# martenlienen/generative-turbulence

Hardware: AMD Instinct MI355X
Metric: U-Net fwd+bwd voxels/sec (DDPM training step, 192x64x48x4) (higher is better)
Workload: dtype bf16

## Files before the change

### generative-turbulence_amd/csrc/tdx_codec.hip

```cpp
#include "tdx_codec_elem.h"
#include "tdx_conv3.h"

#define CD_THREADS 256
#define CD_VOX 512
#define CD_VOX_DEC 2048

template <typename T, int F>
__global__ void __launch_bounds__(CD_THREADS)
encode_fwd_kernel(const float* __restrict__ x, const float* __restrict__ wx, const float* __restrict__ bx,
                  const float* __restrict__ c, const float* __restrict__ wc, const float* __restrict__ bc,
                  T* __restrict__ y, int64_t V, int D, int Dtot) {
    const int b = blockIdx.y;
    const int L = Dtot >> 3, rows = CD_THREADS / L;
    const int lc = threadIdx.x % L, r = threadIdx.x / L;
    if (r >= rows) return;
    const EncLane<F> enc(lc, b, D, V, x, wx, bx, c, wc, bc);
    const int64_t v0 = (int64_t)blockIdx.x * CD_VOX, v1 = min(V, v0 + CD_VOX);
    for (int64_t v = v0 + r; v < v1; v += rows) {
        const auto in = enc.load(V, v);
        Vec8<T> o;
#pragma unroll
        for (int j = 0; j < 8; ++j) o.v[j] = enc.eval(j, in);
        o.store(y + ((int64_t)b * V + v) * Dtot + lc * 8);
    }
}

template <typename T, int F>
__global__ void __launch_bounds__(CD_THREADS)
encode_bwd_kernel(const T* __restrict__ dy, const float* __restrict__ x, const float* __restrict__ c,
                  const float* __restrict__ wc, float* __restrict__ dwx, float* __restrict__ dbx,
                  float* __restrict__ dwc, float* __restrict__ dbc, float* __restrict__ dc, int B, int64_t V, int D,
                  int Dtot, int64_t slab_stride) {
    dwx += blockIdx.x * slab_stride; dbx += blockIdx.x * slab_stride;
    if (dwc) { dwc += blockIdx.x * slab_stride; dbc += blockIdx.x * slab_stride; }
    const int L = Dtot >> 3, rows = CD_THREADS / L;
    const int lc = threadIdx.x % L, r = threadIdx.x / L;
    const bool active = r < rows;
    const bool is_x = lc * 8 < D;
    const int ch0 = is_x ? lc * 8 : lc * 8 - D;
    float s[8 * F + 8];
#pragma unroll
    for (int j = 0; j < 8 * F + 8; ++j) s[j] = 0.f;
    float wr[8][F];
    if (!is_x) {
#pragma unroll
        for (int j = 0; j < 8; ++j)
#pragma unroll
            for (int k = 0; k < F; ++k) wr[j][k] = wc[(ch0 + j) * F + k];
    }
    const int Lc = (Dtot - D) >> 3;
    const int64_t v0 = (int64_t)blockIdx.x * CD_VOX, v1 = min(V, v0 + CD_VOX);
    for (int64_t vb = v0; vb < v1; vb += rows) {
        const int64_t v = vb + r;
        const bool ok = active && v < v1;
        float dcl[F];
#pragma unroll
        for (int k = 0; k < F; ++k) dcl[k] = 0.f;
        for (int b0 = 0; b0 < B; b0 += 3) {
            Raw8<T> graw[3];
            float in[3][F];
#pragma unroll
            for (int u = 0; u < 3; ++u) {
                const int b = min(b0 + u, B - 1);
                const bool okb = ok && b0 + u < B;
                graw[u].load(dy + ((int64_t)b * V + (okb ? v : v0)) * Dtot + lc * 8);
                const float* src = is_x ? x + (int64_t)b * F * V : c;
#pragma unroll
                for (int k = 0; k < F; ++k) in[u][k] = src[(int64_t)k * V + (okb ? v : v0)];
            }
            __builtin_amdgcn_sched_barrier(0);
#pragma unroll
            for (int u = 0; u < 3; ++u) {
                const bool okb = ok && b0 + u < B;
                Vec8<T> g = graw[u].get();
#pragma unroll
                for (int j = 0; j < 8; ++j) g.v[j] = okb ? g.v[j] : 0.f;
#pragma unroll
                for (int j = 0; j < 8; ++j) {
#pragma unroll
                    for (int k = 0; k < F; ++k) s[j * F + k] += g.v[j] * in[u][k];
                    s[8 * F + j] += g.v[j];
                }
                if (!is_x) {
#pragma unroll
                    for (int k = 0; k < F; ++k)
#pragma unroll
                        for (int j = 0; j < 8; ++j) dcl[k] += wr[j][k] * g.v[j];
                }
            }
        }
        if (dc != nullptr && Lc > 0) {
#pragma unroll
            for (int k = 0; k < F; ++k) {
                float t = is_x ? 0.f : dcl[k];
                for (int o = 1; o < L; o <<= 1) t += __shfl_xor(t, o, 64);
                if (ok && lc == 0) dc[(int64_t)k * V + v] = t;
            }
        }
    }
    __shared__ float red[CD_THREADS][8 * F + 8 + 1];
    const int tid = threadIdx.x;
#pragma unroll
    for (int j = 0; j < 8 * F + 8; ++j) red[tid][j] = active ? s[j] : 0.f;
    __syncthreads();
    constexpr int N = 8 * F + 8;
    for (int o = tid; o < L * N; o += CD_THREADS) {
        const int l = o / N, j = o - l * N;
        float t = 0.f;
        for (int q = 0; q < rows; ++q) t += red[q * L + l][j];
        const bool lx = l * 8 < D;
        const int c0 = lx ? l * 8 : l * 8 - D;
        float* dw = lx ? dwx : dwc;
        float* db = lx ? dbx : dbc;
        if (j < 8 * F) atomicAdd(&dw[(c0 + j / F) * F + (j % F)], t);
        else atomicAdd(&db[c0 + (j - 8 * F)], t);
    }
}

static bool pow2(int v) { return v > 0 && (v & (v - 1)) == 0; }
static hipError_t codec_zero(float* p, size_t n, hipStream_t st) {
    return tdx_zero_async(p, n * sizeof(float), st) == TDX_OK ? hipSuccess : hipErrorUnknown;
}
static float* det_slabs(int64_t floats) {
    char* arena = (char*)tdx_scratch_ptr();
    if (!arena || (int64_t)tdx_scratch_bytes() < 256 + floats * (int64_t)sizeof(float)) return nullptr;
    return reinterpret_cast<float*>(arena + 256);
}

extern "C" int tdx_encode_fwd(const float* x, int Fx, const float* wx, const float* bx, const float* c, int Fc,
                              const float* wc, const float* bc, void* y, int B, int64_t V, int D, int dtype,
                              void* stream) {
    TDX_CHECK_ARG(x && wx && bx && y && B > 0 && V > 0 && D > 0);
    TDX_CHECK_ARG(c == nullptr || (wc && bc));
    const int Dtot = c ? 2 * D : D;
    if ((D % 8) || !pow2(Dtot / 8) || Dtot / 8 > 64 || Fx != 4 || (c && Fc != 4)) return TDX_ESHAPE;
    dim3 grid(ceil_div(V, CD_VOX), B);
    TDX_DISPATCH_DTYPE(dtype, hipLaunchKernelGGL((encode_fwd_kernel<T, 4>), grid, dim3(CD_THREADS), 0, as_stream(stream),
                                                 x, wx, bx, c, wc, bc, (T*)y, V, D, Dtot));
    return tdx_launch_status();
}

extern "C" int tdx_encode_bwd(const void* dy, const float* x, int Fx, const float* c, int Fc, const float* wc,
                              float* dwx, float* dbx, float* dwc, float* dbc, float* dc, int B, int64_t V, int D,
                              int dtype, void* stream) {
    TDX_CHECK_ARG(dy && x && dwx && dbx && B > 0 && V > 0 && D > 0);
    TDX_CHECK_ARG(c == nullptr || (wc && dwc && dbc));
    const int Dtot = c ? 2 * D : D;
    if ((D % 8) || !pow2(Dtot / 8) || Dtot / 8 > 64 || Fx != 4 || (c && Fc != 4)) return TDX_ESHAPE;
    hipStream_t st = as_stream(stream);
    dim3 grid(ceil_div(V, CD_VOX));
    if (tdx_deterministic()) {
        const int64_t slab = 10 * (int64_t)D;
        float* slabs = det_slabs((int64_t)grid.x * slab);
        if (!slabs) return TDX_EINVAL;
        int e0 = tdx_zero_async(slabs, (size_t)grid.x * slab * sizeof(float), st);
        if (e0 != TDX_OK) return e0;
        TDX_DISPATCH_DTYPE(dtype, hipLaunchKernelGGL((encode_bwd_kernel<T, 4>), grid, dim3(CD_THREADS), 0, st, (const T*)dy, x, c, wc,
                                                     slabs, slabs + 4 * D, c ? slabs + 5 * D : nullptr,
                                                     c ? slabs + 9 * D : nullptr, dc, B, V, D, Dtot, slab));
        int rc = tdx_launch_status();
        if (rc == TDX_OK) rc = ordered_sum_launch(slabs, (int)grid.x, slab, dwx, 1, 4 * D, 4 * D, false, st);
        if (rc == TDX_OK) rc = ordered_sum_launch(slabs + 4 * D, (int)grid.x, slab, dbx, 1, D, D, false, st);
        if (rc == TDX_OK && c) rc = ordered_sum_launch(slabs + 5 * D, (int)grid.x, slab, dwc, 1, 4 * D, 4 * D, false, st);
        if (rc == TDX_OK && c) rc = ordered_sum_launch(slabs + 9 * D, (int)grid.x, slab, dbc, 1, D, D, false, st);
        return rc;
    }
    hipError_t e = codec_zero(dwx, (size_t)D * 4, st);
    if (e == hipSuccess) e = codec_zero(dbx, (size_t)D, st);
    if (e == hipSuccess && c) e = codec_zero(dwc, (size_t)D * 4, st);
    if (e == hipSuccess && c) e = codec_zero(dbc, (size_t)D, st);
    if (e != hipSuccess) return (int)e;
    TDX_DISPATCH_DTYPE(dtype, hipLaunchKernelGGL((encode_bwd_kernel<T, 4>), grid, dim3(CD_THREADS), 0, st, (const T*)dy,
                                                 x, c, wc, dwx, dbx, dwc, dbc, dc, B, V, D, Dtot, (int64_t)0));
    return tdx_launch_status();
}

template <typename T, int F>
__global__ void __launch_bounds__(CD_THREADS)
decode_fwd_kernel(const T* __restrict__ h, const float* __restrict__ w, const float* __restrict__ bias,
                  float* __restrict__ y, int64_t V, int D) {
    const int b = blockIdx.y;
    const int L = D >> 3, rows = CD_THREADS / L;
    const int lc = threadIdx.x % L, r = threadIdx.x / L;
    const DecLane<F> dec(lc, D, w, bias);
    const int64_t v0 = (int64_t)blockIdx.x * CD_VOX_DEC, v1 = min(V, v0 + CD_VOX_DEC);
    for (int64_t vb = v0; vb < v1; vb += rows) {
        const int64_t v = vb + r;
        const bool ok = r < rows && v < v1;
        Vec8<T> a;
#pragma unroll
        for (int j = 0; j < 8; ++j) a.v[j] = 0.f;
        if (ok) a.load(h + ((int64_t)b * V + v) * D + lc * 8);
#pragma unroll
        for (int f = 0; f < F; ++f) {
            const float t = dec.dot(f, a.v, L);
            if (ok && lc == 0) y[((int64_t)b * F + f) * V + v] = t;
        }
    }
}

template <typename T, int F>
__global__ void __launch_bounds__(CD_THREADS)
decode_bwd_kernel(const float* __restrict__ dy, const T* __restrict__ h, const float* __restrict__ w,
                  T* __restrict__ dh, float* __restrict__ dw, float* __restrict__ db, int64_t V, int D, int64_t slab_stride) {
    const int b = blockIdx.y;
    dw += ((int64_t)blockIdx.y * gridDim.x + blockIdx.x) * slab_stride;
    db += ((int64_t)blockIdx.y * gridDim.x + blockIdx.x) * slab_stride;
    const int L = D >> 3, rows = CD_THREADS / L;
    const int lc = threadIdx.x % L, r = threadIdx.x / L;
    const bool active = r < rows;
    float wr[F][8], s[F * 8 + F];
#pragma unroll
    for (int f = 0; f < F; ++f)
#pragma unroll
        for (int j = 0; j < 8; ++j) wr[f][j] = w[f * D + lc * 8 + j];
#pragma unroll
    for (int j = 0; j < F * 8 + F; ++j) s[j] = 0.f;
    const int64_t v0 = (int64_t)blockIdx.x * CD_VOX_DEC, v1 = min(V, v0 + CD_VOX_DEC);
    if (active) {
        for (int64_t v = v0 + r; v < v1; v += rows) {
            float g[F];
#pragma unroll
            for (int f = 0; f < F; ++f) g[f] = dy[((int64_t)b * F + f) * V + v];
            Vec8<T> a, o;
            a.load(h + ((int64_t)b * V + v) * D + lc * 8);
#pragma unroll
            for (int j = 0; j < 8; ++j) {
                float t = 0.f;
#pragma unroll
                for (int f = 0; f < F; ++f) { t += wr[f][j] * g[f]; s[f * 8 + j] += g[f] * a.v[j]; }
                o.v[j] = t;
            }
            if (lc == 0) {
#pragma unroll
                for (int f = 0; f < F; ++f) s[F * 8 + f] += g[f];
            }
            o.store(dh + ((int64_t)b * V + v) * D + lc * 8);
        }
    }
    __shared__ float red[CD_THREADS][F * 8 + F + 1];
    const int tid = threadIdx.x;
    constexpr int N = F * 8 + F;
#pragma unroll
    for (int j = 0; j < N; ++j) red[tid][j] = active ? s[j] : 0.f;
    __syncthreads();
    for (int o = tid; o < L * N; o += CD_THREADS) {
        const int l = o / N, j = o - l * N;
        float t = 0.f;
        for (int q = 0; q < rows; ++q) t += red[q * L + l][j];
        if (j < F * 8) atomicAdd(&dw[(j / 8) * D + l * 8 + (j % 8)], t);
        else if (l == 0) atomicAdd(&db[j - F * 8], t);
    }
}

extern "C" int tdx_decode_fwd(const void* h, const float* w, const float* bias, float* y, int B, int64_t V, int D, int F,
                              int dtype, void* stream) {
    TDX_CHECK_ARG(h && w && bias && y && B > 0 && V > 0 && D > 0);
    if ((D % 8) || !pow2(D / 8) || D / 8 > 64 || F != 4) return TDX_ESHAPE;
    dim3 grid(ceil_div(V, CD_VOX_DEC), B);
    TDX_DISPATCH_DTYPE(dtype, hipLaunchKernelGGL((decode_fwd_kernel<T, 4>), grid, dim3(CD_THREADS), 0, as_stream(stream),
                                                 (const T*)h, w, bias, y, V, D));
    return tdx_launch_status();
}

extern "C" int tdx_decode_bwd(const float* dy, const void* h, const float* w, void* dh, float* dw, float* db, int B,
                              int64_t V, int D, int F, int dtype, void* stream) {
    TDX_CHECK_ARG(dy && h && w && dh && dw && db && B > 0 && V > 0 && D > 0);
    if ((D % 8) || !pow2(D / 8) || D / 8 > 64 || F != 4) return TDX_ESHAPE;
    hipStream_t st = as_stream(stream);
    dim3 grid(ceil_div(V, CD_VOX_DEC), B);
    if (tdx_deterministic()) {
        const int64_t slab = (int64_t)F * D + F, nblk = (int64_t)grid.x * grid.y;
        float* slabs = det_slabs(nblk * slab);
        if (!slabs) return TDX_EINVAL;
        int e0 = tdx_zero_async(slabs, (size_t)nblk * slab * sizeof(float), st);
        if (e0 != TDX_OK) return e0;
        TDX_DISPATCH_DTYPE(dtype, hipLaunchKernelGGL((decode_bwd_kernel<T, 4>), grid, dim3(CD_THREADS), 0, st, dy, (const T*)h, w,
                                                     (T*)dh, slabs, slabs + (int64_t)F * D, V, D, slab));
        int rc = tdx_launch_status();
        if (rc == TDX_OK) rc = ordered_sum_launch(slabs, (int)nblk, slab, dw, 1, F * D, F * D, false, st);
        if (rc == TDX_OK) rc = ordered_sum_launch(slabs + (int64_t)F * D, (int)nblk, slab, db, 1, F, F, false, st);
        return rc;
    }
    hipError_t e = codec_zero(dw, (size_t)F * D, st);
    if (e == hipSuccess) e = codec_zero(db, (size_t)F, st);
    if (e != hipSuccess) return (int)e;
    TDX_DISPATCH_DTYPE(dtype, hipLaunchKernelGGL((decode_bwd_kernel<T, 4>), grid, dim3(CD_THREADS), 0, st, dy,
// ... 4 lines not shown
```

### generative-turbulence_amd/csrc/tdx_codec_elem.h

```cpp
#pragma once
#include "tdx_common.h"

template <typename T> __device__ __forceinline__ float round_as(float a);
template <> __device__ __forceinline__ float round_as<float>(float a) { return a; }
template <> __device__ __forceinline__ float round_as<bf16>(float a) { return __uint_as_float(pack_bf16x2(a, 0.f) << 16); }
template <> __device__ __forceinline__ float round_as<f16>(float a) { return (float)(_Float16)a; }

template <int F>
struct EncLane {
    struct In { float v[F]; };
    const float* src;
    float w[8][F], bias[8];
    __device__ __forceinline__ EncLane(int lc, int b, int D, int64_t V, const float* __restrict__ x, const float* __restrict__ wx,
                                       const float* __restrict__ bx, const float* __restrict__ c, const float* __restrict__ wc,
                                       const float* __restrict__ bc) {
        const bool is_x = lc * 8 < D;
        const int ch0 = is_x ? lc * 8 : lc * 8 - D;
        const float* wp = is_x ? wx : wc;
        const float* bp = is_x ? bx : bc;
        src = is_x ? x + (int64_t)b * F * V : c;
#pragma unroll
        for (int j = 0; j < 8; ++j) {
            bias[j] = bp[ch0 + j];
#pragma unroll
            for (int k = 0; k < F; ++k) w[j][k] = wp[(ch0 + j) * F + k];
        }
    }
    __device__ __forceinline__ In load(int64_t V, int64_t v) const {
        In in;
#pragma unroll
        for (int k = 0; k < F; ++k) in.v[k] = src[(int64_t)k * V + v];
        return in;
    }
    __device__ __forceinline__ float eval(int j, const In& in) const {
        float a = bias[j];
#pragma unroll
        for (int k = 0; k < F; ++k) a = __builtin_fmaf(w[j][k], in.v[k], a);
        return a;
    }
};

template <int F>
struct DecLane {
    float w[F][8], bias[F];
    __device__ __forceinline__ DecLane(int lc, int C, const float* __restrict__ wp, const float* __restrict__ bp) {
#pragma unroll
        for (int f = 0; f < F; ++f) {
            bias[f] = bp[f];
#pragma unroll
            for (int j = 0; j < 8; ++j) w[f][j] = wp[f * C + lc * 8 + j];
        }
    }
    __device__ __forceinline__ float dot(int f, const float (&h)[8], int L) const {
        float t = 0.f;
#pragma unroll
        for (int j = 0; j < 8; ++j) t = __builtin_fmaf(w[f][j], h[j], t);
        for (int q = 1; q < L; q <<= 1) t += __shfl_xor(t, q, 64);
        return t + bias[f];
    }
};
```

### generative-turbulence_amd/csrc/tdx_conv3.h

```cpp
#pragma once
#include "tdx_common.h"

struct Conv3Geom {
    int B;
    int Xi, Yi, Zi;
    int Xo, Yo, Zo;
    int off;
};

bool conv3_mfma_supported(int C1, int C2, int Cout);
bool conv3_mfma_f32_supported(int C1, int C2, int Cout);
static inline int conv3_layout_kc(int dtype, int K, int N) {
    if (dtype == 1 || dtype == 3) return conv3_mfma_supported(K, 0, N) ? 16 : 0;
    return conv3_mfma_f32_supported(K, 0, N) ? 8 : 0;
}
static inline bool conv3_uses_mfma_layout(int dtype, int K, int N) { return (dtype == 1 || dtype == 3) && conv3_mfma_supported(K, 0, N); }
bool conv3_mfma_split_supported(int C1, int C2, int Cout);

struct Conv3Ext {
    int ld1, ld2;
    const void* init;
    bool init_shared;
};

struct Conv3Call {
    const void* x1; int C1;
    const void* x2; int C2;
    const void* wp;
    const float* bias;
    void* y;
    int B, X, Y, Z, N;
    bool zero_pad;
    double* gn_acc;
    void* d1; int D1; void* d2;
    const void* a1; const void* a2;
    hipStream_t st;
    int fmt;
    const Conv3Ext* ext;
    const int* slabs_beyond;
    bool hf() const { return fmt == TDX_F16; }
    Conv3Geom geom() const { return Conv3Geom{B, X, Y, Z, X, Y, Z, 0}; }
};

struct SmallGeom {
    int B;
    int Ev[3];
    int Es[3];
    int off;
    int clamp;
    int nbg;
    int xs;
    int gx;
    int Ix, Iy, Iz;
    int K, N;
    int per_split;
    int nsplit;
};
struct Conv3SmallPlan {
    SmallGeom g;
    size_t lds;
    int mtw;
};

struct Conv3Route {
    int fmt, family, status;
    int ring_depth;
    Conv3SmallPlan small;
};
Conv3Route conv3_route(int dtype, int impl, int C1, int C2, int N, int B, int X, int Y, int Z, bool data_gradient);

int conv3_mfma_launch(const Conv3Call& c);
int conv3_mfma_split_launch(const Conv3Call& c);
int conv3_mfma_f32_launch(const Conv3Call& c);
int conv3_direct_launch(const Conv3Call& c);
int conv3_fold_launch(const Conv3Call& c);

int conv3_ring_depth(int C1, int C2, int N, int B, int X, int Y, int Z, bool data_gradient);
int conv3_ring_launch(const Conv3Call& c, int depth);

bool conv3_small_plan(Conv3SmallPlan& p, int C1, int C2, int N, int B, int X, int Y, int Z, bool data_gradient, bool split);
int conv3_small_launch(const Conv3Call& c, const Conv3SmallPlan& p);

struct Conv3WgradCall {
    const void* x1; int C1;
    const void* x2; int C2;
    const void* dy;
    float* dwp;
    float* dbias;
    int B, X, Y, Z, Cout;
    hipStream_t st;
    float* slabs; int max_slabs; int* nslab;
    bool hf;
};
bool tdx_deterministic();
static inline float* conv3_wgrad_merge(const Conv3WgradCall& c, int& nsplit, int64_t& slab_stride) {
    if (tdx_deterministic() && c.slabs != nullptr && nsplit > c.max_slabs) nsplit = c.max_slabs > 0 ? c.max_slabs : 1;
    const bool use_slabs = c.slabs != nullptr && nsplit <= c.max_slabs;
    slab_stride = use_slabs ? (int64_t)27 * (c.C1 + c.C2) * c.Cout : 0;
    if (c.nslab) *c.nslab = use_slabs ? nsplit : 0;
    return use_slabs ? c.slabs : c.dwp;
}
bool conv3_wgrad_mfma_supported(int C1, int C2, int Cout);
bool conv3_wgrad_mfma_split_supported(int C1, int C2, int Cout);
bool conv3_wgrad_mfma_f32_supported(int C1, int C2, int Cout);
int conv3_wgrad_mfma_launch(const Conv3WgradCall& c);
int conv3_wgrad_small_launch(const Conv3WgradCall& c);
int conv3_wgrad_ring_launch(const Conv3WgradCall& c);
int conv3_wgrad_mfma_split_launch(const Conv3WgradCall& c);
int conv3_wgrad_split_ring_launch(const Conv3WgradCall& c);
int conv3_wgrad_mfma_f32_launch(const Conv3WgradCall& c);
int conv3_wgrad_direct_launch(const Conv3WgradCall& c, int dtype);
int conv3_unpack_wgrad_launch(const Conv3WgradCall& c, float* dw, float* dbw, float* dbias, bool many);
int tdx_persistent_cus();
int ordered_sum_launch(const float* slabs, int nslab, int64_t stride, float* dst, int rows, int cols, int64_t ld, bool add,
                       hipStream_t st);
size_t bias_grad_ordered_scratch_floats(int C);
int bias_grad_ordered_launch(const void* dy, int64_t nvox, int C, int dtype, float* dbias, float* part, size_t part_floats,
                             hipStream_t st);
void* tdx_scratch_ptr();
size_t tdx_scratch_bytes();

size_t conv3_shell_buffer_bytes(int B, int X, int Y, int Z, int N);
int conv3_shell_launch(const void* dy, const void* wb, void* d1, int D1, void* d2, int B, int X, int Y, int Z, int K, int N,
                       int mode, hipStream_t st, void* sbuf = nullptr);

#define TDX_GN_REPLICAS 32
int gn_finalize_launch(double* acc, float* stats, int B, int C, int G, int64_t V, float eps, int replicas,
                       hipStream_t st);
int gn_stats_launch(const void* x, float* stats, int B, int64_t V, int C, int G, float eps, int dtype, void* workspace,
                    bool clean, hipStream_t stream);
```

### generative-turbulence_amd/csrc/tdx_conv3_entry.hip

```cpp
#include "tdx_common.h"
#include "tdx_conv3.h"
#include <stdlib.h>
#include <algorithm>

int tdx_persistent_cus() {
    const char* env = getenv("TDX_PERSISTENT_CUS");
    int n = env ? atoi(env) : 256;
    n = n < 8 ? 8 : (n > 256 ? 256 : n);
    return n & ~7;
}
static void* g_scratch = nullptr;
static size_t g_scratch_bytes = 0;
void* tdx_scratch_ptr() { return g_scratch; }
size_t tdx_scratch_bytes() { return g_scratch_bytes; }
extern "C" int tdx_set_scratch(void* ptr, size_t bytes) {
    if (ptr != nullptr && bytes < 64) return TDX_EINVAL;
    g_scratch = ptr;
    g_scratch_bytes = ptr ? bytes : 0;
    return TDX_OK;
}

Conv3Route conv3_route(int dtype, int impl, int C1, int C2, int N, int B, int X, int Y, int Z, bool data_gradient) {
    Conv3Route r;
    r.fmt = dtype; r.family = TDX_KERNEL_DIRECT; r.status = TDX_OK; r.ring_depth = 0;
    impl &= 0xff;
    auto small_or_brick = [&](bool split) {
        r.family = conv3_small_plan(r.small, C1, C2, N, B, X, Y, Z, data_gradient, split) ? TDX_KERNEL_SMALL : TDX_KERNEL_BRICK;
    };
    if (dtype == TDX_F32 && impl == TDX_CONV_SPLIT && conv3_mfma_split_supported(C1 + C2, 0, N)) {
        r.fmt = TDX_F32_SPLIT;
        if (!conv3_mfma_split_supported(C1, C2, N)) { r.family = TDX_KERNEL_BRICK; r.status = TDX_ESHAPE; return r; }
        small_or_brick(true);
    } else if (dtype == TDX_F32 && impl != TDX_CONV_DIRECT && conv3_mfma_f32_supported(C1, C2, N)) {
        r.family = TDX_KERNEL_BRICK;
    } else {
        const bool ok = tdx_is_h16(dtype) && conv3_mfma_supported(C1, C2, N);
        const bool asked = impl == TDX_CONV_MFMA && (tdx_is_h16(dtype) || !data_gradient);
        if (!ok) { r.status = asked ? TDX_ESHAPE : TDX_OK; return r; }
        if (!asked && impl != TDX_CONV_AUTO) return r;
        small_or_brick(false);
        if (r.family == TDX_KERNEL_BRICK && (r.ring_depth = conv3_ring_depth(C1, C2, N, B, X, Y, Z, data_gradient)) != 0)
            r.family = TDX_KERNEL_RING;
    }
    return r;
}

static int conv3_launch(const Conv3Call& c, const Conv3Route& r) {
    switch (r.family) {
        case TDX_KERNEL_SMALL: return conv3_small_launch(c, r.small);
        case TDX_KERNEL_RING: return conv3_ring_launch(c, r.ring_depth);
        case TDX_KERNEL_BRICK:
            if (c.fmt == TDX_F32_SPLIT) return conv3_mfma_split_launch(c);
            return c.fmt == TDX_F32 ? conv3_mfma_f32_launch(c) : conv3_mfma_launch(c);
        default: return conv3_direct_launch(c);
    }
}

static Conv3Call conv3_fwd_call(const void* x1, int C1, const void* x2, int C2, const void* wf, const float* bias, void* y, int B,
                                int X, int Y, int Z, int Cout, int fmt, void* stream) {
    Conv3Call c = {};
    c.x1 = x1; c.C1 = C1; c.x2 = x2; c.C2 = C2; c.wp = wf; c.bias = bias; c.y = y;
    c.B = B; c.X = X; c.Y = Y; c.Z = Z; c.N = Cout;
    c.st = as_stream(stream); c.fmt = fmt;
    return c;
}

extern "C" int tdx_conv3_fwd(const void* x1, int C1, const void* x2, int C2, const void* wf, const float* bias,
                             void* y, int B, int X, int Y, int Z, int Cout, int dtype, int impl, void* stream) {
    TDX_CHECK_ARG(x1 && wf && y && B > 0 && X > 0 && Y > 0 && Z > 0 && C1 > 0 && C2 >= 0 && Cout > 0);
    TDX_CHECK_ARG(C2 == 0 || x2);
    const Conv3Route r = conv3_route(dtype, impl, C1, C2, Cout, B, X, Y, Z, false);
    if (r.status != TDX_OK) return r.status;
    return conv3_launch(conv3_fwd_call(x1, C1, x2, C2, wf, bias, y, B, X, Y, Z, Cout, r.fmt, stream), r);
}

extern "C" int tdx_conv3_fwd_kernel(int C1, int C2, int Cout, int B, int X, int Y, int Z, int dtype, int impl) {
    return conv3_route(dtype, impl, C1, C2, Cout, B, X, Y, Z, false).family;
}

extern "C" int tdx_conv3_fwd_gn(const void* x1, int C1, const void* x2, int C2, const void* wf, const float* bias,
                                void* y, float* stats, int G, float eps, void* gn_workspace, int B, int X, int Y, int Z,
                                int Cout, int dtype, int impl, void* stream) {
    TDX_CHECK_ARG(x1 && wf && y && stats && gn_workspace && B > 0 && X > 0 && Y > 0 && Z > 0 && C1 > 0 && C2 >= 0);
    TDX_CHECK_ARG(Cout > 0 && G > 0 && (Cout % G) == 0 && (C2 == 0 || x2));
    const bool clean = (impl & TDX_WS_CLEAN) != 0;
    const Conv3Route r = conv3_route(dtype, impl, C1, C2, Cout, B, X, Y, Z, false);
    if (r.status != TDX_OK) return r.status;
    Conv3Call c = conv3_fwd_call(x1, C1, x2, C2, wf, bias, y, B, X, Y, Z, Cout, r.fmt, stream);
    const int64_t V = (int64_t)X * Y * Z;
    if (r.family == TDX_KERNEL_DIRECT || r.family == TDX_KERNEL_SMALL || tdx_deterministic()) {
        int rc = conv3_launch(c, r);
        if (rc != TDX_OK) return rc;
        if (r.family == TDX_KERNEL_DIRECT && !tdx_deterministic())
            return tdx_gn_stats(y, stats, B, V, Cout, G, eps, dtype, gn_workspace, stream);
        return gn_stats_launch(y, stats, B, V, Cout, G, eps, dtype, gn_workspace, clean, c.st);
    }
    c.gn_acc = (double*)gn_workspace;
    if (!clean) {
        int e = tdx_zero_async(c.gn_acc, (size_t)TDX_GN_REPLICAS * B * Cout * 2 * sizeof(double), c.st);
        if (e != TDX_OK) return e;
    }
    int rc = conv3_launch(c, r);
    if (rc != TDX_OK) return rc;
    return gn_finalize_launch(c.gn_acc, stats, B, Cout, G, V, eps, TDX_GN_REPLICAS, c.st);
}

extern "C" int tdx_conv3_fwd_partial(const void* x1, int C1, int ld1, const void* wf, const float* bias,
                                     const void* init, int init_shared, void* y, float* stats, int G, float eps,
                                     void* gn_workspace, int B, int X, int Y, int Z, int Cout, int dtype, int impl,
                                     void* stream) {
    TDX_CHECK_ARG(x1 && wf && y && B > 0 && X > 0 && Y > 0 && Z > 0 && C1 > 0 && Cout > 0 && ld1 >= C1 && (ld1 % 8) == 0);
    TDX_CHECK_ARG(stats == nullptr || (gn_workspace && G > 0 && (Cout % G) == 0));
    const bool clean = (impl & TDX_WS_CLEAN) != 0;
    if (!tdx_is_h16(dtype)) return TDX_EDTYPE;
    if (!conv3_mfma_supported(C1, 0, Cout)) return TDX_ESHAPE;
    const bool det = tdx_deterministic();
    const Conv3Ext ext = {ld1, 0, init, init_shared != 0};
    Conv3Call c = conv3_fwd_call(x1, C1, nullptr, 0, wf, bias, y, B, X, Y, Z, Cout, dtype, stream);
    c.ext = &ext;
    c.gn_acc = (stats && !det) ? (double*)gn_workspace : nullptr;
    if (c.gn_acc && !clean) {
        int e = tdx_zero_async(c.gn_acc, (size_t)TDX_GN_REPLICAS * B * Cout * 2 * sizeof(double), c.st);
        if (e != TDX_OK) return e;
    }
    int rc = conv3_mfma_launch(c);
    if (rc != TDX_OK || !stats) return rc;
    if (det) return gn_stats_launch(y, stats, B, (int64_t)X * Y * Z, Cout, G, eps, dtype, gn_workspace, clean, c.st);
    return gn_finalize_launch(c.gn_acc, stats, B, Cout, G, (int64_t)X * Y * Z, eps, TDX_GN_REPLICAS, c.st);
}

extern "C" size_t tdx_conv3_bwd_data_workspace_bytes(int B, int X, int Y, int Z, int Cin, int dtype, int impl) {
    (void)impl;
    const size_t padded = (size_t)B * (X + 2) * (Y + 2) * (Z + 2) * Cin * (tdx_is_h16(dtype) ? 2 : 4);
    const size_t shell = conv3_shell_buffer_bytes(B, X, Y, Z, Cin);
    return (padded > shell ? padded : shell) + 256;
}

static int conv3_bwd_data_impl(const void* dy, const void* wb, void* dx1, int C1, void* dx2, int C2, const void* add1,
                               const void* add2, int B, int X, int Y, int Z, int Cout, int dtype, int impl,
                               void* workspace, void* stream) {
    TDX_CHECK_ARG(dy && wb && dx1 && workspace && B > 0 && X > 0 && Y > 0 && Z > 0 && C1 > 0 && C2 >= 0 && Cout > 0);
    TDX_CHECK_ARG(C2 == 0 || dx2);
    const int Cin = C1 + C2;
    if ((C1 % 8) || (C2 % 8) || (Cout % 8)) return TDX_ESHAPE;
    const Conv3Route r = conv3_route(dtype, impl, Cout, 0, Cin, B, X, Y, Z, true);
    if (r.status != TDX_OK) return r.status;
    Conv3Call c = {};
    c.x1 = dy; c.C1 = Cout; c.wp = wb;
    c.B = B; c.X = X; c.Y = Y; c.Z = Z; c.N = Cin;
    c.zero_pad = true;
    c.d1 = dx1; c.D1 = C1; c.d2 = dx2; c.a1 = add1; c.a2 = add2;
    c.st = as_stream(stream); c.fmt = r.fmt;
    if (r.family == TDX_KERNEL_DIRECT) c.y = workspace;
    int rc = conv3_launch(c, r);
    if (rc != TDX_OK || r.family == TDX_KERNEL_SMALL) return rc;
    if (r.family == TDX_KERNEL_DIRECT) return conv3_fold_launch(c);
    const int shell_mode = r.fmt == TDX_F16 ? 3 : (r.fmt == TDX_F32_SPLIT ? 2 : (r.fmt == TDX_F32 ? 1 : 0));
    return conv3_shell_launch(dy, wb, dx1, C1, dx2, B, X, Y, Z, Cout, Cin, shell_mode, c.st, workspace);
}

extern "C" int tdx_conv3_bwd_data(const void* dy, const void* wb, void* dx1, int C1, void* dx2, int C2,
                                  int accumulate, int B, int X, int Y, int Z, int Cout, int dtype, int impl,
                                  void* workspace, void* stream) {
    return conv3_bwd_data_impl(dy, wb, dx1, C1, dx2, C2, accumulate ? dx1 : nullptr, accumulate ? dx2 : nullptr, B, X, Y, Z,
                               Cout, dtype, impl, workspace, stream);
}

extern "C" int tdx_conv3_bwd_data_add(const void* dy, const void* wb, void* dx1, int C1, void* dx2, int C2,
                                      const void* add1, const void* add2, int B, int X, int Y, int Z, int Cout, int dtype,
                                      int impl, void* workspace, void* stream) {
    return conv3_bwd_data_impl(dy, wb, dx1, C1, dx2, C2, add1, add2, B, X, Y, Z, Cout, dtype, impl, workspace, stream);
}

#define W3_MAX_SLABS 8
static int w3_slab_capacity(int Cin, int Cout) {
    const int64_t c = ((int64_t)1 << 19) / ((int64_t)Cin * Cout);
    return (int)(c < W3_MAX_SLABS ? W3_MAX_SLABS : (c > 512 ? 512 : c));
}
extern "C" size_t tdx_conv3_bwd_weight_workspace_bytes(int Cin, int Cout, int impl) {
    (void)impl;
    return (size_t)(1 + w3_slab_capacity(Cin, Cout)) * 27 * Cin * Cout * sizeof(float) + (size_t)Cout * sizeof(float) + 512;
}

struct Conv3WgradRoute {
    int (*launch)(const Conv3WgradCall&);
    bool f32;
    int status;
};
static Conv3WgradRoute conv3_wgrad_route(int dtype, int impl, int C1, int C2, int Cout) {
    if (dtype == TDX_F32 && impl == TDX_CONV_SPLIT && conv3_wgrad_mfma_split_supported(C1, C2, Cout))
        return {conv3_wgrad_mfma_split_launch, true, TDX_OK};
    if (dtype == TDX_F32 && impl != TDX_CONV_DIRECT && conv3_wgrad_mfma_f32_supported(C1, C2, Cout))
        return {conv3_wgrad_mfma_f32_launch, true, TDX_OK};
    if (impl == TDX_CONV_MFMA || (impl == TDX_CONV_AUTO && tdx_is_h16(dtype) && conv3_wgrad_mfma_supported(C1, C2, Cout))) {
        if (!tdx_is_h16(dtype)) return {nullptr, false, TDX_EDTYPE};
        if (!conv3_wgrad_mfma_supported(C1, C2, Cout)) return {nullptr, false, TDX_ESHAPE};
        return {conv3_wgrad_mfma_launch, false, TDX_OK};
    }
    return {nullptr, false, TDX_OK};
}

extern "C" int tdx_conv3_bwd_weight(const void* x1, int C1, const void* x2, int C2, const void* dy, float* dw,
                                    float* dbias, int B, int X, int Y, int Z, int Cout, int dtype, int impl,
                                    void* workspace, void* stream) {
    TDX_CHECK_ARG(x1 && dy && dw && workspace && B > 0 && X > 0 && Y > 0 && Z > 0 && C1 > 0 && C2 >= 0 && Cout > 0);
    TDX_CHECK_ARG(C2 == 0 || x2);
    const int Cin = C1 + C2;
    if ((C1 % 8) || (C2 % 8) || (Cout % 8)) return TDX_ESHAPE;
    hipStream_t st = as_stream(stream);
    const bool clean = (impl & TDX_WS_CLEAN) != 0;
    float* dwp = (float*)workspace;
    float* dbw = dwp + (size_t)27 * Cin * Cout;
    if (!clean) {
        int e = tdx_zero_async(dwp, ((size_t)27 * Cin * Cout + Cout) * sizeof(float), st);
        if (e != TDX_OK) return e;
    }
    const Conv3WgradRoute r = conv3_wgrad_route(dtype, impl & 0xff, C1, C2, Cout);
    if (r.status != TDX_OK) return r.status;
    int nslab = 0;
    const bool det = tdx_deterministic();
    float* slab_base = dbw + ((Cout + 63) / 64) * 64;
    auto ordered_bias = [&]() -> int {
        if (!det || !dbias) return TDX_OK;
        return bias_grad_ordered_launch(dy, (int64_t)B * X * Y * Z, Cout, dtype, dbias, slab_base,
                                        (size_t)W3_MAX_SLABS * 27 * Cin * Cout, st);
    };
    Conv3WgradCall c = {x1, C1, x2, C2, dy, dwp, (dbias && !det) ? dbw : nullptr, B, X, Y, Z, Cout, st, slab_base, 0, &nslab,
                        dtype == TDX_F16};
    if (r.launch != nullptr) {
        c.max_slabs = (r.f32 && !det) ? W3_MAX_SLABS : w3_slab_capacity(Cin, Cout);
    } else if (det) {
        c.max_slabs = std::min(w3_slab_capacity(Cin, Cout), 64);
    }
    const int rc = r.launch != nullptr ? r.launch(c) : conv3_wgrad_direct_launch(c, dtype);
    if (rc != TDX_OK) return rc;
    const int rc_unpack = conv3_unpack_wgrad_launch(c, dw, dbw, dbias, r.launch != nullptr && nslab > W3_MAX_SLABS);
    return rc_unpack != TDX_OK ? rc_unpack : ordered_bias();
}
```

### generative-turbulence_amd/csrc/tdx_conv3_mfma.hip

```cpp
#include "tdx_common.h"
#include "tdx_conv3.h"
#include "tdx_mfma.h"
#include <stdlib.h>

#define M3_KC 16

bool conv3_mfma_supported(int C1, int C2, int Cout) {
    return C1 > 0 && (C1 % M3_KC) == 0 && (C2 % M3_KC) == 0 && (Cout % 32) == 0;
}

struct ConvView {
    int B;
    int Ei[3];
    int si[3];
    int so[3];
    int r0[3];
    int r1[3];
    int nb[3];
    int off;
    int ws[3];
    int in_batch, out_batch;
    int ld1, ld2;
    int init_batch;
};

struct ConvViews {
    ConvView v[3];
    int start[4];
};

template <int BN>
__device__ __forceinline__ int out_addr(int v, int c) {
    if (BN == 64) return v * 128 + ((c ^ (v & 7)) << 4);
    return v * 64 + ((c ^ ((v >> 1) & 3)) << 4);
}

template <int NT, bool XT, bool ZERO_PAD, bool PERM, bool EXT, bool HF>
__global__ void __launch_bounds__(256, 2)
conv3_mfma_kernel(const bf16* __restrict__ x1, int C1, const bf16* __restrict__ x2, int C2,
                  const bf16* __restrict__ wp, const float* __restrict__ bias, bf16* __restrict__ y, ConvViews gs,
                  int Cout, double* __restrict__ gn_acc, bf16* __restrict__ d1, int D1, bf16* __restrict__ d2,
                  const bf16* __restrict__ a1, const bf16* __restrict__ a2, const bf16* __restrict__ init) {
    typedef H16<HF> H;
    typedef typename H::T HT;
    constexpr int BN = NT * 32;
    constexpr int BX = XT ? 2 : 4, BY = XT ? 16 : 8, BZ = 8;
    constexpr int HX = BX + 2, HY = BY + 2, HZ = BZ + 2;
    constexpr int SZ = XT ? 10 : 12;
    constexpr int NHALO = HX * HY * HZ;
    constexpr int APLANE = HX * HY * SZ * 16 + 64;
    constexpr int BRICK_BYTES = 2 * APLANE;
    constexpr int B_PLANE = 27 * BN * 16 + 64;
    extern __shared__ __attribute__((aligned(16))) unsigned char smem[];
    unsigned char* sA = smem;
    unsigned char* sB = smem + BRICK_BYTES;

    const int tid = threadIdx.x;
    const int lane = tid & 63, wave = tid >> 6;
    const int r = lane & 31, hh = lane >> 5;

    int bid = blockIdx.x;
    bid = xcd_contiguous(bid, (int)gridDim.x);
    const int region = bid >= gs.start[1] ? (bid >= gs.start[2] ? 2 : 1) : 0;
    const ConvView& g = gs.v[region];
    bid -= gs.start[region];
    const int b2 = bid % g.nb[2]; bid /= g.nb[2];
    const int b1 = bid % g.nb[1]; bid /= g.nb[1];
    const int b0 = bid % g.nb[0]; bid /= g.nb[0];
    const int b = bid;
    const int n0 = blockIdx.y * BN;
    const int o0 = g.r0[0] + b0 * BX, o1 = g.r0[1] + b1 * BY, o2 = g.r0[2] + b2 * BZ;
    const int Cin = C1 + C2;

    constexpr int A_PIECES = NHALO * 2;
    constexpr int A_PER_THREAD = (A_PIECES + 255) / 256;
    constexpr int B_PIECES = 27 * BN * 2;
    constexpr int B_PER_THREAD = (B_PIECES + 255) / 256;
    int a_src[A_PER_THREAD];
    int a_dst[A_PER_THREAD];
#pragma unroll
    for (int i = 0; i < A_PER_THREAD; ++i) {
        const int p = tid + i * 256;
        a_dst[i] = -1;
        a_src[i] = -1;
        if (p < A_PIECES) {
            const int hv = ((p >> 3) << 2) + (p & 3), half = (p >> 2) & 1;
            const int hx = hv / (HY * HZ), rem = hv - hx * (HY * HZ);
            const int hy = rem / HZ, hz = rem - hy * HZ;
            a_dst[i] = half * APLANE + ((hx * HY + hy) * SZ + hz) * 16;
            int s0 = o0 + hx - 1 + g.off, s1 = o1 + hy - 1 + g.off, s2 = o2 + hz - 1 + g.off;
            bool ok = true;
            if (ZERO_PAD) {
                ok = s0 >= 0 && s0 < g.Ei[0] && s1 >= 0 && s1 < g.Ei[1] && s2 >= 0 && s2 < g.Ei[2];
            } else {
                s0 = min(max(s0, 0), g.Ei[0] - 1); s1 = min(max(s1, 0), g.Ei[1] - 1); s2 = min(max(s2, 0), g.Ei[2] - 1);
            }
            if (ok) a_src[i] = (s0 * g.si[0] + s1 * g.si[1] + s2 * g.si[2]) * 2 + half;
        }
    }
    const int64_t batch_vox = (int64_t)b * g.in_batch;

    const int b_half = (tid >> 2) & 1;
    const int b_row0 = ((tid >> 3) << 2) + (tid & 3);
    const int b_goff = ((b_row0 / BN) * Cout + (b_row0 % BN)) * 16 + b_half * 8;
    const int b_dst = b_half * B_PLANE + b_row0 * 16;

    uint4 areg[A_PER_THREAD], breg[B_PER_THREAD];
    auto load_slice = [&](int c) {
        const int k0 = c * M3_KC;
        const bf16* xs;
        int Cs, kk;
        if (k0 < C1) { xs = x1; Cs = EXT ? g.ld1 : C1; kk = k0; } else { xs = x2; Cs = EXT ? g.ld2 : C2; kk = k0 - C1; }
        xs += batch_vox * Cs + kk;
#pragma unroll
        for (int i = 0; i < A_PER_THREAD; ++i) {
            areg[i] = make_uint4(0, 0, 0, 0);
            if (a_src[i] >= 0)
                areg[i] = *reinterpret_cast<const uint4*>(xs + (int64_t)(a_src[i] >> 1) * Cs + (a_src[i] & 1) * 8);
        }
        const bf16* wc = wp + (int64_t)c * 27 * Cout * 16 + (int64_t)n0 * 16 + b_goff;
#pragma unroll
        for (int i = 0; i < B_PER_THREAD; ++i) {
            breg[i] = make_uint4(0, 0, 0, 0);
            if (b_row0 + 128 * i < 27 * BN)
                breg[i] = *reinterpret_cast<const uint4*>(wc + (int64_t)i * (128 / BN) * Cout * 16);
        }
    };
    auto store_slice = [&]() {
#pragma unroll
        for (int i = 0; i < A_PER_THREAD; ++i)
            if (a_dst[i] >= 0) *reinterpret_cast<uint4*>(sA + a_dst[i]) = areg[i];
#pragma unroll
        for (int i = 0; i < B_PER_THREAD; ++i)
            if (b_row0 + 128 * i < 27 * BN) *reinterpret_cast<uint4*>(sB + b_dst + i * 2048) = breg[i];
    };

    const int wx = XT ? (wave >> 1) : wave, wy0 = XT ? 8 * (wave & 1) : 0;
    int a_h[2];
#pragma unroll
    for (int mt = 0; mt < 2; ++mt)
        a_h[mt] = ((wx + 1) * HY + (wy0 + 4 * mt + (r & 3) + 1)) * SZ + ((r >> 2) + 1);
    int b_off[NT];
#pragma unroll
    for (int nt = 0; nt < NT; ++nt) b_off[nt] = hh * B_PLANE + (nt * 32 + r) * 16;

    f32x16 acc[NT][2];
#pragma unroll
    for (int nt = 0; nt < NT; ++nt)
#pragma unroll
        for (int mt = 0; mt < 2; ++mt)
#pragma unroll
            for (int i = 0; i < 16; ++i) acc[nt][mt][i] = 0.f;

    const int nchunks = Cin / M3_KC;
    load_slice(0);
    for (int c = 0; c < nchunks; ++c) {
        __syncthreads();
        store_slice();
        __syncthreads();
        if (c + 1 < nchunks) load_slice(c + 1);

        bf16x8 xf[2][2], wf[2][NT];
        auto read_frags = [&](int tap, int buf) {
            const int ex = tap / 9 - 1, ey = (tap / 3) % 3 - 1, ez = tap % 3 - 1;
            const int toff = (ex * HY + ey) * SZ + ez;
            const int wtap = (XT || PERM) ? (ex + 1) * g.ws[0] + (ey + 1) * g.ws[1] + (ez + 1) * g.ws[2] : tap;
#pragma unroll
            for (int mt = 0; mt < 2; ++mt)
                xf[buf][mt] = *reinterpret_cast<const bf16x8*>(sA + hh * APLANE + (a_h[mt] + toff) * 16);
#pragma unroll
            for (int nt = 0; nt < NT; ++nt)
                wf[buf][nt] = *reinterpret_cast<const bf16x8*>(sB + wtap * (BN * 16) + b_off[nt]);
        };
        read_frags(0, 0);
        __builtin_amdgcn_sched_group_barrier(0x100, 2 + NT, 0);
#pragma unroll
        for (int tap = 0; tap < 27; ++tap) {
            if (tap + 1 < 27) read_frags(tap + 1, (tap + 1) & 1);
#pragma unroll
            for (int nt = 0; nt < NT; ++nt)
#pragma unroll
                for (int mt = 0; mt < 2; ++mt)
                    acc[nt][mt] = H::mfma(wf[tap & 1][nt], xf[tap & 1][mt], acc[nt][mt]);
            if (tap + 1 < 27) {
#pragma unroll
                for (int k = 0; k < 2 * NT; ++k) {
                    __builtin_amdgcn_sched_group_barrier(0x008, 1, 0);
                    if (k < 2 + NT) __builtin_amdgcn_sched_group_barrier(0x100, 1, 0);
                }
            } else {
                __builtin_amdgcn_sched_group_barrier(0x008, 2 * NT, 0);
            }
        }
    }

    __syncthreads();
    unsigned char* sO = smem;
#pragma unroll
    for (int nt = 0; nt < NT; ++nt)
#pragma unroll
        for (int j = 0; j < 4; ++j) {
            const int ch = nt * 32 + 8 * j + 4 * hh;
            float bv[4] = {0.f, 0.f, 0.f, 0.f};
            if (bias) {
#pragma unroll
                for (int e = 0; e < 4; ++e) bv[e] = bias[n0 + ch + e];
            }
#pragma unroll
            for (int mt = 0; mt < 2; ++mt) {
                const int v = (wx * BY + wy0 + 4 * mt + (r & 3)) * 8 + (r >> 2);
                const unsigned lo = H::pack2(acc[nt][mt][4 * j] + bv[0], acc[nt][mt][4 * j + 1] + bv[1]);
                const unsigned hi = H::pack2(acc[nt][mt][4 * j + 2] + bv[2], acc[nt][mt][4 * j + 3] + bv[3]);
                *reinterpret_cast<uint2*>(sO + out_addr<BN>(v, ch >> 3) + (ch & 7) * 2) = make_uint2(lo, hi);
            }
        }
    __syncthreads();
    constexpr int CHUNKS = BN / 8;
    float s1[8], s2[8];
#pragma unroll
    for (int e = 0; e < 8; ++e) s1[e] = s2[e] = 0.f;
#pragma unroll
    for (int i = 0; i < CHUNKS; ++i) {
        const int p = tid + i * 256;
        const int v = p / CHUNKS, cidx = p % CHUNKS;
        const int c0 = o0 + (v >> 3) / BY, c1 = o1 + (v >> 3) % BY, c2 = o2 + (v & 7);
        if (c0 < g.r1[0] && c1 < g.r1[1] && c2 < g.r1[2]) {
            uint4 val = *reinterpret_cast<const uint4*>(sO + out_addr<BN>(v, cidx));
            bool direct = false;
            if (ZERO_PAD && d1 != nullptr) {
                const int u0 = c0 + g.off, u1 = c1 + g.off, u2 = c2 + g.off;
                if (u0 >= 0 && u0 < g.Ei[0] && u1 >= 0 && u1 < g.Ei[1] && u2 >= 0 && u2 < g.Ei[2]) {
                    const int64_t u = (int64_t)b * g.in_batch + u0 * g.si[0] + u1 * g.si[1] + u2 * g.si[2];
                    const int n = n0 + cidx * 8;
                    const bool lo = n < D1;
                    bf16* dst = lo ? d1 + u * D1 + n : d2 + u * (Cout - D1) + (n - D1);
                    const bf16* asrc = lo ? (a1 ? a1 + u * D1 + n : nullptr) : (a2 ? a2 + u * (Cout - D1) + (n - D1) : nullptr);
                    if (asrc) {
                        Vec8<HT> va, vb;
                        va.load(reinterpret_cast<const HT*>(&val));
                        vb.load(reinterpret_cast<const HT*>(asrc));
#pragma unroll
                        for (int e = 0; e < 8; ++e) va.v[e] += vb.v[e];
                        va.store(reinterpret_cast<HT*>(dst));
                    } else {
                        *reinterpret_cast<uint4*>(dst) = val;
                    }
                    direct = true;
                }
            }
            if (!direct) {
                const int64_t ov = (int64_t)b * g.out_batch + c0 * g.so[0] + c1 * g.so[1] + c2 * g.so[2];
                if (EXT && init != nullptr) {
                    const int64_t iv = (int64_t)b * g.init_batch + c0 * g.so[0] + c1 * g.so[1] + c2 * g.so[2];
                    Vec8<HT> va, vb;
                    va.load(reinterpret_cast<const HT*>(&val));
                    vb.load(reinterpret_cast<const HT*>(init + iv * Cout + n0 + cidx * 8));
#pragma unroll
                    for (int e = 0; e < 8; ++e) va.v[e] += vb.v[e];
                    va.store(reinterpret_cast<HT*>(&val));
                }
                *reinterpret_cast<uint4*>(y + ov * Cout + n0 + cidx * 8) = val;
            }
            if (gn_acc != nullptr) {
                const unsigned wds[4] = {val.x, val.y, val.z, val.w};
#pragma unroll
                for (int e = 0; e < 4; ++e) {
                    const float lo = H::lo(wds[e]), hi = H::hi(wds[e]);
                    s1[2 * e] += lo; s2[2 * e] += lo * lo;
                    s1[2 * e + 1] += hi; s2[2 * e + 1] += hi * hi;
                }
            }
        }
    }
    if (gn_acc != nullptr) {
        constexpr int NP = 256 / CHUNKS;
        float* red = reinterpret_cast<float*>(smem + 256 * BN * 2);
        const int cidx = tid % CHUNKS, part = tid / CHUNKS;
#pragma unroll
        for (int e = 0; e < 8; ++e) {
            red[(part * BN + cidx * 8 + e) * 2] = s1[e];
            red[(part * BN + cidx * 8 + e) * 2 + 1] = s2[e];
        }
        __syncthreads();
        if (tid < BN * 2) {
            float t = 0.f;
#pragma unroll 8
            for (int pp = 0; pp < NP; ++pp) t += red[pp * BN * 2 + tid];
            const int rep = blockIdx.x & (TDX_GN_REPLICAS - 1);
            atomicAdd(&gn_acc[(((size_t)rep * g.B + b) * Cout + n0) * 2 + tid], (double)t);
        }
    }
}

template <int NT, bool XT, bool ZP, bool PERM, bool EXT, bool HF>
static int launch_view_h(const Conv3Call& c, const ConvViews& v) {
    constexpr int BN = NT * 32;
    constexpr int HXv = (XT ? 2 : 4) + 2, HYv = (XT ? 16 : 8) + 2, SZv = XT ? 10 : 12;
    const size_t lds = (size_t)2 * (HXv * HYv * SZv * 16 + 64) + (size_t)27 * BN * 32 + 128;
    auto kern = conv3_mfma_kernel<NT, XT, ZP, PERM, EXT, HF>;
    static bool attr_set = false;
    if (!attr_set) {
        hipError_t e = hipFuncSetAttribute((const void*)kern, hipFuncAttributeMaxDynamicSharedMemorySize, (int)lds);
        if (e != hipSuccess) return (int)e;
        attr_set = true;
    }
    dim3 grid((unsigned)v.start[3], c.N / BN);
    hipLaunchKernelGGL(kern, grid, dim3(256), lds, c.st, (const bf16*)c.x1, c.C1, (const bf16*)c.x2, c.C2, (const bf16*)c.wp, c.bias,
                       (bf16*)c.y, v, c.N, c.gn_acc, (bf16*)c.d1, c.D1, (bf16*)c.d2, (const bf16*)c.a1, (const bf16*)c.a2,
                       (const bf16*)(EXT ? c.ext->init : nullptr));
    return tdx_launch_status();
}
template <int NT, bool XT, bool ZP, bool PERM, bool EXT = false>
static int launch_view(const Conv3Call& c, const ConvViews& v) {
    return c.hf() ? launch_view_h<NT, XT, ZP, PERM, EXT, true>(c, v) : launch_view_h<NT, XT, ZP, PERM, EXT, false>(c, v);
}

int conv3_mfma_launch(const Conv3Call& c) {
    if (!tdx_is_h16(c.fmt)) return TDX_EINVAL;
    const Conv3Geom g = c.geom();
    const int C1 = c.C1, C2 = c.C2;
    const bool zero_pad = c.zero_pad;
    const Conv3Ext* ext = c.ext;
    const int* slabs_beyond = c.slabs_beyond;
    const int NT = (c.N % 64 == 0) ? 2 : 1;
    if ((int64_t)g.Xi * g.Yi * g.Zi * 2 >= (1ll << 31) || (int64_t)g.Xo * g.Yo * g.Zo >= (1ll << 31)) return TDX_ESHAPE;
    static const bool no_thin = getenv("TDX_CONV3_THIN") && atoi(getenv("TDX_CONV3_THIN")) == 0;

    const int Ei[3] = {g.Xi, g.Yi, g.Zi}, Eo[3] = {g.Xo, g.Yo, g.Zo};
    const int si[3] = {g.Yi * g.Zi, g.Zi, 1}, so[3] = {g.Yo * g.Zo, g.Zo, 1};
    const int bdim[3] = {4, 8, 8};
    static const bool force_thin = getenv("TDX_CONV3_THIN") && atoi(getenv("TDX_CONV3_THIN")) == 2;
    const bool big = force_thin || (int64_t)g.Xo * g.Yo * g.Zo >= 60000;
    int main_end[3];
    bool thin[3];
    for (int a = 0; a < 3; ++a) {
        const int rem = Eo[a] % bdim[a];
        thin[a] = !no_thin && rem >= 1 && rem <= 2 && Eo[a] > bdim[a] && big && ext == nullptr;
        main_end[a] = thin[a] ? Eo[a] - rem : Eo[a];
        if (slabs_beyond != nullptr) {
            if (ext != nullptr || slabs_beyond[a] <= 0 || Eo[a] - slabs_beyond[a] > 2 || Eo[a] < slabs_beyond[a]) return TDX_ESHAPE;
            main_end[a] = slabs_beyond[a];
            thin[a] = main_end[a] < Eo[a];
        }
    }
    auto make_view = [&](const int perm[3], const int lo[3], const int hi[3], bool xt, ConvView& v) -> int {
        v.B = g.B; v.off = g.off;
        v.in_batch = g.Xi * g.Yi * g.Zi; v.out_batch = g.Xo * g.Yo * g.Zo;
        v.ld1 = ext && ext->ld1 ? ext->ld1 : C1;
        v.ld2 = ext && ext->ld2 ? ext->ld2 : C2;
        v.init_batch = ext && ext->init && !ext->init_shared ? v.out_batch : 0;
        const int bl[3] = {xt ? 2 : 4, xt ? 16 : 8, 8};
        int64_t n = g.B;
        for (int k = 0; k < 3; ++k) {
            const int a = perm[k];
            v.Ei[k] = Ei[a]; v.si[k] = si[a]; v.so[k] = so[a];
            v.ws[k] = (a == 0) ? 9 : (a == 1 ? 3 : 1);
            v.r0[k] = lo[a]; v.r1[k] = hi[a];
            v.nb[k] = hi[a] > lo[a] ? ceil_div(hi[a] - lo[a], bl[k]) : 0;
            n *= v.nb[k];
        }
        return (int)n;
    };
    auto launch = [&](const ConvViews& vs, bool xt, bool permuted) -> int {
        if (vs.start[3] == 0) return TDX_OK;
#define M3_GO(NTV, XTV, PV) (zero_pad ? launch_view<NTV, XTV, true, PV>(c, vs) : launch_view<NTV, XTV, false, PV>(c, vs))
        if (ext != nullptr) {
            if (zero_pad || xt || permuted) return TDX_ESHAPE;
            return NT == 2 ? launch_view<2, false, false, false, true>(c, vs) : launch_view<1, false, false, false, true>(c, vs);
        }
        if (NT == 2) return xt ? M3_GO(2, true, false) : (permuted ? M3_GO(2, false, true) : M3_GO(2, false, false));
        return xt ? M3_GO(1, true, false) : (permuted ? M3_GO(1, false, true) : M3_GO(1, false, false));
#undef M3_GO
    };
    const int lo[3] = {0, 0, 0}, hi[3] = {main_end[0], main_end[1], main_end[2]};
    static const bool no_perm = getenv("TDX_CONV3_PERM") && atoi(getenv("TDX_CONV3_PERM")) == 0;
    int best[3] = {0, 1, 2};
    if (!no_perm && ext == nullptr) {
        const int cand[3][3] = {{0, 1, 2}, {1, 0, 2}, {2, 0, 1}};
        int64_t best_n = -1;
        for (int c = 0; c < 3; ++c) {
            const int64_t n = (int64_t)ceil_div(hi[cand[c][0]], 4) * ceil_div(hi[cand[c][1]], 8) * ceil_div(hi[cand[c][2]], 8);
            if (best_n < 0 || n < best_n) {
                best_n = n;
                for (int k = 0; k < 3; ++k) best[k] = cand[c][k];
            }
        }
    }
    ConvViews mainv;
    const int nmain = make_view(best, lo, hi, false, mainv.v[0]);
    mainv.v[1] = mainv.v[2] = mainv.v[0];
    mainv.start[0] = 0; mainv.start[1] = mainv.start[2] = mainv.start[3] = nmain;
    int rc = slabs_beyond ? TDX_OK : launch(mainv, false, !(best[0] == 0 && best[1] == 1 && best[2] == 2));
    if (rc != TDX_OK) return rc;
    if (thin[0] || thin[1] || thin[2]) {
        const int pm[3][3] = {{0, 1, 2}, {1, 0, 2}, {2, 0, 1}};
        const int l[3][3] = {{main_end[0], 0, 0}, {0, main_end[1], 0}, {0, 0, main_end[2]}};
        const int h[3][3] = {{Eo[0], Eo[1], Eo[2]}, {main_end[0], Eo[1], Eo[2]}, {main_end[0], main_end[1], Eo[2]}};
        ConvViews tv;
        int total = 0;
        for (int r = 0; r < 3; ++r) {
            tv.start[r] = total;
            const int n = make_view(pm[r], l[r], h[r], true, tv.v[r]);
            if (thin[r]) total += n;
        }
        tv.start[3] = total;
        for (int r = 2; r >= 0; --r)
            if (!thin[r]) tv.start[r] = tv.start[r + 1];
        if ((rc = launch(tv, true, false)) != TDX_OK) return rc;
    }
    return TDX_OK;
}
```

### generative-turbulence_amd/csrc/tdx_conv3_ring.hip

```cpp
#include "tdx_common.h"
#include "tdx_conv3.h"
#include "tdx_mfma.h"
#include <stdlib.h>
#include <algorithm>

#define RG_HY 10
#define RG_SZ 12
#define RG_SZ4 6
#define RG_WSLOTS 3
#define RG_WAVES 8
#define RG_STEPS 14
#ifndef RG_DEFAULT_LOADERS
#define RG_DEFAULT_LOADERS 1
#endif

struct RingArgs {
    const bf16* x1; const bf16* x2; int C1, C2;
    const bf16* wp; const float* bias; bf16* y;
    int B, X, Y, Z, Cout;
    int nbx, nby, nbz, ntn;
    double* gn_acc;
    bf16* d1; bf16* d2; int D1; const bf16* a1; const bf16* a2;
    const void* zeros;
    unsigned long long* stamps;
};

__device__ __forceinline__ void rg_dma_off(const void* sbase, unsigned voff, unsigned lds) {
    lds = __builtin_amdgcn_readfirstlane(lds);
    unsigned keep;
    asm volatile("s_mov_b32 %0, m0\n\ts_mov_b32 m0, %3\n\ts_nop 0\n\tglobal_load_lds_dwordx4 %1, %2\n\ts_mov_b32 m0, %0"
                 : "=&s"(keep) : "v"(voff), "s"(sbase), "s"(lds) : "memory");
}
#define RG_VMCNT(n) asm volatile("s_waitcnt vmcnt(%0)" ::"n"(n) : "memory")

#ifdef RG_STAMPS
#define RG_NSTAMP 64
#define RG_T()                                                                                        \
    do {                                                                                              \
        if (ord >= RG_STAMP_B0 && ord < RG_STAMP_B0 + 2) {                                            \
            const unsigned long long t_ = __builtin_amdgcn_s_memtime();                               \
            if (lane == 0 && nst < RG_NSTAMP) sStamp[wave * RG_NSTAMP + nst] = t_;                    \
            ++nst;                                                                                    \
        }                                                                                             \
    } while (0)
#else
#define RG_T() do { } while (0)
#endif

template <int BN>
__device__ __forceinline__ int rg_tile_addr(int v, int c) {
    if (BN == 64) return v * 128 + ((c ^ (v & 7)) << 4);
    return v * 64 + ((c ^ ((v >> 1) & 3)) << 4);
}

template <int NT, int LW = 0, bool Z4 = false>
struct RingShape {
    static constexpr int IW = LW ? LW : 8;
    static constexpr int BN = NT * 32;
    static constexpr int MT = 4 / NT;
    static constexpr int XP = Z4 ? MT : MT / 2;
    static constexpr int BX = 8 * XP;
    static constexpr int BZ = Z4 ? 4 : 8;
    static constexpr int HZ = BZ + 2;
    static constexpr int SZ = Z4 ? RG_SZ4 : RG_SZ;
    static constexpr int ENT = Z4 ? (BX + 2) / 2 * RG_HY * RG_SZ
                                  : (BX + 2) * RG_HY * SZ;
    static constexpr int APIECES = (ENT + 63) / 64;
    static constexpr int ABUF = APIECES * 1024;
    static constexpr int BPW = (APIECES + IW - 1) / IW;
    static constexpr int WPIECES = 28 * BN * 16 / 1024;
    static constexpr int WSLOT = WPIECES * 1024;
    static constexpr int WPW = (WPIECES + IW - 1) / IW;
    static constexpr int TILE = 32 * BN * 2;
    static constexpr int CH = BN / 8;
    static constexpr int VPI = 64 / CH;
    static constexpr int NST = MT * (32 / VPI);
    static constexpr size_t LDS = (size_t)2 * ABUF + (size_t)RG_WSLOTS * WSLOT + (size_t)RG_WAVES * TILE + 1024  +
                                  64  + BN * 4  + (size_t)RG_WAVES * BN * 2 * 4 ;
};

template <int NT, bool ZP, int LW, bool HF, bool Z4>
__global__ void __launch_bounds__(512 + 64 * LW, LW ? 3 : 2) conv3_ring_kernel(RingArgs A) {
    typedef RingShape<NT, LW, Z4> S;
    typedef H16<HF> H;
    typedef typename H::T HT;
    constexpr int BN = S::BN, MT = S::MT, XP = S::XP, BPW = S::BPW, WPW = S::WPW, CH = S::CH, VPI = S::VPI, NST = S::NST;
    static_assert(LW > 0 || BPW + WPW < RG_STEPS, "one DMA instruction per K step");
    extern __shared__ __attribute__((aligned(1024))) unsigned char smem[];
    unsigned char* sA = smem;
    unsigned char* sW = sA + 2 * S::ABUF;
    unsigned char* sT = sW + RG_WSLOTS * S::WSLOT;
    unsigned char* sD = sT + RG_WAVES * S::TILE;
    unsigned char* sZ = sD + 1024;
    float* sBias = reinterpret_cast<float*>(sZ + 64);
    float* sRed = sBias + BN;
    const unsigned lds0 = (unsigned)(size_t)(__attribute__((address_space(3))) const void*)smem;
    const unsigned ldsA = lds0, ldsW = lds0 + 2 * S::ABUF, ldsD = ldsW + RG_WSLOTS * S::WSLOT + RG_WAVES * S::TILE;

    const int tid = threadIdx.x, lane = tid & 63;
    const int wave = __builtin_amdgcn_readfirstlane(tid >> 6);
    const int r = lane & 31, hh = lane >> 5;
    const bool loader = LW > 0 && wave >= RG_WAVES;
    const int iw = LW ? wave - RG_WAVES : wave;
#ifdef RG_STAMPS
    unsigned long long* sStamp = reinterpret_cast<unsigned long long*>(NT == 2 ? sRed : sRed + RG_WAVES * BN * 2);
    int nst = 0;
#endif

    const int hw = blockIdx.x, xcd = hw & 7, slot = hw >> 3;
    const int ntile = slot % A.ntn, kx = slot / A.ntn, KX = (int)(gridDim.x >> 3) / A.ntn;
    const int nbricks = A.B * A.nbx * A.nby * A.nbz;
    const int lo = xcd * (nbricks >> 3) + min(xcd, nbricks & 7), hi = lo + (nbricks >> 3) + (xcd < (nbricks & 7) ? 1 : 0);
    const int nmine = hi - lo > kx ? (hi - lo - kx + KX - 1) / KX : 0;
    if (nmine == 0) return;
    const int n0 = ntile * BN;
    const int Cin = A.C1 + A.C2, nun = Cin >> 3;
    const int YZ = A.Y * A.Z, V = A.X * YZ;

    if (tid < BN) sBias[tid] = A.bias ? A.bias[n0 + tid] : 0.f;
    if (tid < 16) reinterpret_cast<unsigned*>(sZ)[tid] = 0u;
    lds_barrier();

    int hxyz[BPW];
#pragma unroll
    for (int i = 0; i < BPW; ++i) {
        const int pi = min(max(iw, 0) * BPW + i, S::APIECES - 1);
        const int e = min(pi * 64 + lane, S::ENT - 1);
        int hx, hy, hz;
        if (Z4) {
            const int xp = e / (RG_HY * RG_SZ), rem = e - xp * (RG_HY * RG_SZ), q = rem % RG_SZ;
            hy = rem / RG_SZ; hx = 2 * xp + q / RG_SZ4; hz = q % RG_SZ4;
        } else {
            hx = e / (RG_HY * S::SZ);
            const int rem = e - hx * (RG_HY * S::SZ);
            hy = rem / S::SZ; hz = min(rem - hy * S::SZ, S::HZ - 1);
        }
        hxyz[i] = hx | (hy << 8) | (hz << 16);
    }
    unsigned wlane[WPW];
#pragma unroll
    for (int j = 0; j < WPW; ++j) {
        const int pj = min(max(iw, 0) * WPW + j, S::WPIECES - 1);
        const int e = pj * 64 + lane;
        wlane[j] = (unsigned)((min(e / BN, 26) * A.Cout + (e % BN)) * 32);
    }

    const int ly = Z4 ? (r & 7) : (r & 3), lz = Z4 ? (r >> 3) : (r >> 2);
    int a_h[MT];
#pragma unroll
    for (int mt = 0; mt < MT; ++mt) {
        const int px = Z4 ? wave * XP + mt : wave * XP + mt / 2, py = Z4 ? ly : 4 * (mt % 2) + ly;
        const int hx = px + 1;
        a_h[mt] = Z4 ? ((hx >> 1) * (RG_HY * RG_SZ) + (py + 1) * RG_SZ + (hx & 1) * RG_SZ4 + (lz + 1)) * 16
                     : ((hx * RG_HY + (py + 1)) * S::SZ + (lz + 1)) * 16;
    }
    int xo[Z4 ? 2 : 1][RG_STEPS];
#pragma unroll
    for (int p = 0; p < RG_STEPS; ++p) {
        const int t = min(2 * p + hh, 26);
        const int dx = t / 9 - 1, dy = (t / 3) % 3 - 1, dz = t % 3 - 1;
        if (Z4) {
            const int step_odd = dx > 0 ? RG_HY * RG_SZ - RG_SZ4 : (dx < 0 ? -RG_SZ4 : 0);
            const int step_even = dx > 0 ? RG_SZ4 : (dx < 0 ? RG_SZ4 - RG_HY * RG_SZ : 0);
            xo[0][p] = (step_odd + dy * RG_SZ + dz) * 16;
            xo[Z4 ? 1 : 0][p] = (step_even + dy * RG_SZ + dz) * 16;
        } else {
            xo[0][p] = ((dx * RG_HY + dy) * S::SZ + dz) * 16;
        }
    }
    int b_off[NT];
#pragma unroll
    for (int nt = 0; nt < NT; ++nt) b_off[nt] = (hh * BN + nt * 32 + r) * 16;

    int vox[BPW];
    int vb_b = 0;
    auto brick_coords = [&](int ord, int& b, int& o0, int& o1, int& o2) {
        int id = lo + kx + KX * ord;
        const int bz = id % A.nbz; id /= A.nbz;
        const int by = id % A.nby; id /= A.nby;
        const int bx = id % A.nbx; id /= A.nbx;
        b = id; o0 = bx * S::BX; o1 = by * 8; o2 = bz * S::BZ;
    };
    auto plan_brick = [&](int ord) {
        int b, o0, o1, o2;
        brick_coords(min(ord, nmine - 1), b, o0, o1, o2);
        vb_b = b;
#pragma unroll
        for (int i = 0; i < BPW; ++i) {
            int s0 = o0 + (hxyz[i] & 0xff) - 1, s1 = o1 + ((hxyz[i] >> 8) & 0xff) - 1, s2 = o2 + ((hxyz[i] >> 16) & 0xff) - 1;
            bool ok = true;
            if (ZP) ok = s0 >= 0 && s0 < A.X && s1 >= 0 && s1 < A.Y && s2 >= 0 && s2 < A.Z;
            else { s0 = min(max(s0, 0), A.X - 1); s1 = min(max(s1, 0), A.Y - 1); s2 = min(max(s2, 0), A.Z - 1); }
            vox[i] = ok ? (s0 * A.Y + s1) * A.Z + s2 : -1;
        }
    };
    auto issue_brick_piece = [&](int c8, int buf, int i) {
        const int k0 = c8 << 3;
        const bf16* xs; int Cs, kk;
        if (k0 < A.C1) { xs = A.x1; Cs = A.C1; kk = k0; } else { xs = A.x2; Cs = A.C2; kk = k0 - A.C1; }
        const bf16* base = xs + ((int64_t)vb_b * V) * Cs + kk;
        const int pi = iw * BPW + i;
        const unsigned dst = pi < S::APIECES ? ldsA + buf * S::ABUF + pi * 1024 : ldsD;
        if (ZP) {
            const bf16* src = vox[i] >= 0 ? base + (int64_t)vox[i] * Cs : reinterpret_cast<const bf16*>(A.zeros);
            lds_dma16(src, dst);
        } else {
            rg_dma_off(base, (unsigned)(vox[i] * Cs) * 2u, dst);
        }
    };
    auto issue_weight_piece = [&](int c8, int wslot, int j) {
        const bf16* base = A.wp + ((int64_t)((c8 >> 1) * 27) * A.Cout + n0) * 16 + (c8 & 1) * 8;
        const int pj = iw * WPW + j;
        const unsigned dst = pj < S::WPIECES ? ldsW + wslot * S::WSLOT + pj * 1024 : ldsD;
        rg_dma_off(base, wlane[j], dst);
    };

    typedef __attribute__((ext_vector_type(2))) float f32x2;
    f32x2 p1[4], p2[4];
#pragma unroll
    for (int e = 0; e < 4; ++e) p1[e] = p2[e] = f32x2{0.f, 0.f};
    auto flush_stats = [&](int b) {
        float s1[8], s2[8];
#pragma unroll
        for (int e = 0; e < 4; ++e) { s1[2 * e] = p1[e].x; s1[2 * e + 1] = p1[e].y; s2[2 * e] = p2[e].x; s2[2 * e + 1] = p2[e].y; }
#pragma unroll
        for (int e = 0; e < 8; ++e) {
#pragma unroll
            for (int o = CH; o < 64; o <<= 1) { s1[e] += __shfl_xor(s1[e], o, 64); s2[e] += __shfl_xor(s2[e], o, 64); }
        }
        if (lane < CH) {
#pragma unroll
            for (int e = 0; e < 8; ++e) {
                sRed[(wave * BN + lane * 8 + e) * 2] = s1[e];
                sRed[(wave * BN + lane * 8 + e) * 2 + 1] = s2[e];
            }
        }
        lds_barrier();
        if (tid < BN * 2) {
            float t = 0.f;
#pragma unroll
            for (int w = 0; w < RG_WAVES; ++w) t += sRed[w * BN * 2 + tid];
            const int rep = blockIdx.x & (TDX_GN_REPLICAS - 1);
            atomicAdd(&A.gn_acc[(((size_t)rep * A.B + b) * A.Cout + n0) * 2 + tid], (double)t);
        }
        lds_barrier();
#pragma unroll
        for (int e = 0; e < 4; ++e) p1[e] = p2[e] = f32x2{0.f, 0.f};
    };

    int qs = 1, qb = 0, ws = 2 % nun, uw = 2;
    int u = 0;
    if (LW == 0 || loader) {
        plan_brick(0);
#pragma unroll
        for (int i = 0; i < BPW; ++i) issue_brick_piece(0, 0, i);
#pragma unroll
        for (int j = 0; j < WPW; ++j) issue_weight_piece(0, 0, j);
#pragma unroll
        for (int j = 0; j < WPW; ++j) issue_weight_piece(1 % nun, 1, j);
        if (qs == nun) { qs = 0; qb = 1; plan_brick(1); }
    }
    if (LW > 0 && loader) {
        for (int ord = 0; ord < nmine; ++ord) {
            for (int c8 = 0; c8 < nun; ++c8, ++u) {
                RG_VMCNT(WPW);
                lds_barrier();
#pragma unroll
                for (int i = 0; i < BPW; ++i) issue_brick_piece(qs, (u + 1) & 1, i);
#pragma unroll
                for (int j = 0; j < WPW; ++j) issue_weight_piece(ws, uw % RG_WSLOTS, j);
                ++uw;
                if (++ws == nun) ws = 0;
                if (++qs == nun) { qs = 0; ++qb; plan_brick(qb); }
            }
#ifndef RG_STAMPS
            if (!ZP && A.gn_acc != nullptr) {
                int b, nb = -1, t0, t1, t2;
                brick_coords(ord, b, t0, t1, t2);
                if (ord + 1 < nmine) brick_coords(ord + 1, nb, t0, t1, t2);
                if (nb != b) { lds_barrier(); lds_barrier(); }
            }
#endif
        }
        RG_VMCNT(0);
        return;
    }
    bool stores_behind = false;

    f32x16 acc[NT][MT];

    for (int ord = 0; ord < nmine; ++ord) {
        int b, o0, o1, o2;
        brick_coords(ord, b, o0, o1, o2);
#pragma unroll
        for (int nt = 0; nt < NT; ++nt)
#pragma unroll
            for (int j = 0; j < 4; ++j) {
                const float4 bv = *reinterpret_cast<const float4*>(sBias + nt * 32 + 8 * j + 4 * hh);
#pragma unroll
                for (int mt = 0; mt < MT; ++mt) {
                    acc[nt][mt][4 * j] = bv.x; acc[nt][mt][4 * j + 1] = bv.y; acc[nt][mt][4 * j + 2] = bv.z; acc[nt][mt][4 * j + 3] = bv.w;
                }
            }

        for (int c8 = 0; c8 < nun; ++c8, ++u) {
            RG_T();
            if (LW == 0) { if (stores_behind) RG_VMCNT(WPW + NST); else RG_VMCNT(WPW); }
            stores_behind = false;
            RG_T();
            lds_barrier();
            RG_T();

            const unsigned char* bufA = sA + (u & 1) * S::ABUF;
            const unsigned char* slotW = sW + (u % RG_WSLOTS) * S::WSLOT;
            const unsigned char* xa[MT];
#pragma unroll
            for (int mt = 0; mt < MT; ++mt) xa[mt] = bufA + a_h[mt];

            bf16x8 xf[3][MT], wf[3][NT];
            auto read_frags = [&](int p, int fb) {
#pragma unroll
                for (int mt = 0; mt < MT; ++mt) {
                    const unsigned char* src = xa[mt] + xo[Z4 ? (mt & 1) : 0][p];
                    if (p == RG_STEPS - 1) src = hh ? sZ : src;
                    xf[fb][mt] = *reinterpret_cast<const bf16x8*>(src);
                }
#pragma unroll
                for (int nt = 0; nt < NT; ++nt) wf[fb][nt] = *reinterpret_cast<const bf16x8*>(slotW + p * (2 * BN * 16) + b_off[nt]);
            };
            read_frags(0, 0);
            read_frags(1, 1);
            __builtin_amdgcn_sched_group_barrier(0x100, 2 * (MT + NT), 0);
#pragma unroll
            for (int p = 0; p < RG_STEPS; ++p) {
#if defined(RG_ABL) && (RG_ABL & 2)
                if (false)
#endif
                if (p + 2 < RG_STEPS) read_frags(p + 2, (p + 2) % 3);
#pragma unroll
                for (int nt = 0; nt < NT; ++nt)
#pragma unroll
                    for (int mt = 0; mt < MT; ++mt)
                        acc[nt][mt] = H::mfma(wf[p % 3][nt], xf[p % 3][mt], acc[nt][mt]);
                if (p + 2 < RG_STEPS) {
#pragma unroll
                    for (int k = 0; k < 4; ++k) {
                        __builtin_amdgcn_sched_group_barrier(0x008, 1, 0);
                        if (k < MT + NT) __builtin_amdgcn_sched_group_barrier(0x100, 1, 0);
                    }
                } else {
                    __builtin_amdgcn_sched_group_barrier(0x008, 4, 0);
                }
#if !defined(RG_ABL) || !(RG_ABL & 1)
                if (LW == 0 && p < BPW) issue_brick_piece(qs, (u + 1) & 1, p);
                if (LW == 0 && p >= BPW && p < BPW + WPW) issue_weight_piece(ws, uw % RG_WSLOTS, p - BPW);
#endif
                if (LW == 0 && p == BPW + WPW) {
                    ++uw;
                    if (++ws == nun) ws = 0;
                    if (++qs == nun) { qs = 0; ++qb; plan_brick(qb); }
                }
            }
        }

        RG_T();
        unsigned char* tile = sT + wave * S::TILE;
        const int last_b = b;
#pragma unroll
        for (int mt = 0; mt < MT; ++mt) {
            const int vw = ly * S::BZ + lz;
#pragma unroll
            for (int nt = 0; nt < NT; ++nt)
#pragma unroll
                for (int j = 0; j < 4; ++j) {
                    const int ch = nt * 32 + 8 * j + 4 * hh;
                    const unsigned lo2 = H::pack2(acc[nt][mt][4 * j], acc[nt][mt][4 * j + 1]);
                    const unsigned hi2 = H::pack2(acc[nt][mt][4 * j + 2], acc[nt][mt][4 * j + 3]);
                    *reinterpret_cast<uint2*>(tile + rg_tile_addr<BN>(vw, ch >> 3) + (ch & 7) * 2) = make_uint2(lo2, hi2);
                }
#pragma unroll
            for (int i = 0; i < 32 / VPI; ++i) {
                const int v = lane / CH + VPI * i, cidx = lane % CH;
                const int c0 = o0 + (Z4 ? wave * XP + mt : wave * XP + mt / 2);
                const int c1 = o1 + (Z4 ? (v >> 2) : 4 * (mt % 2) + (v >> 3)), c2 = o2 + (Z4 ? (v & 3) : (v & 7));
                uint4 val = *reinterpret_cast<const uint4*>(tile + rg_tile_addr<BN>(v, cidx));
                const int64_t ov = (int64_t)b * V + c0 * YZ + c1 * A.Z + c2;
                const int n = n0 + cidx * 8;
                if (ZP) {
                    const bool lo1 = n < A.D1;
                    bf16* dst = lo1 ? A.d1 + ov * A.D1 + n : A.d2 + ov * (A.Cout - A.D1) + (n - A.D1);
                    const bf16* asrc = lo1 ? (A.a1 ? A.a1 + ov * A.D1 + n : nullptr)
                                           : (A.a2 ? A.a2 + ov * (A.Cout - A.D1) + (n - A.D1) : nullptr);
                    if (asrc) {
                        Vec8<HT> va, vb;
                        va.load(reinterpret_cast<const HT*>(&val));
                        vb.load(reinterpret_cast<const HT*>(asrc));
#pragma unroll
                        for (int e = 0; e < 8; ++e) va.v[e] += vb.v[e];
                        va.store(reinterpret_cast<HT*>(dst));
                    } else {
                        *reinterpret_cast<uint4*>(dst) = val;
                    }
                } else {
                    *reinterpret_cast<uint4*>(A.y + ov * A.Cout + n) = val;
                    if (A.gn_acc != nullptr) {
                        const unsigned wds[4] = {val.x, val.y, val.z, val.w};
#pragma unroll
                        for (int e = 0; e < 4; ++e) {
                            const f32x2 lh = {H::lo(wds[e]), H::hi(wds[e])};
                            p1[e] += lh;
                            p2[e] = __builtin_elementwise_fma(lh, lh, p2[e]);
                        }
                    }
                }
            }
        }
        stores_behind = true;
        RG_T();
#ifndef RG_STAMPS
        if (!ZP && A.gn_acc != nullptr) {
            int nb = -1;
            if (ord + 1 < nmine) { int t0, t1, t2; brick_coords(ord + 1, nb, t0, t1, t2); }
            if (nb != last_b) flush_stats(last_b);
        }
#endif
    }
    if (LW == 0) RG_VMCNT(0);
#ifdef RG_STAMPS
    if (lane == 0 && A.stamps != nullptr) {
        unsigned long long* rec = A.stamps + ((size_t)blockIdx.x * RG_WAVES + wave) * (RG_NSTAMP + 1);
        rec[0] = nst;
        for (int i = 0; i < RG_NSTAMP; ++i) rec[1 + i] = sStamp[wave * RG_NSTAMP + i];
    }
#endif
}

static bool ring_z8_supported(int C1, int C2, int Cout, int B, int X, int Y, int Z, int mode);
static bool ring_z4_supported(int C1, int C2, int Cout, int B, int X, int Y, int Z, int mode) {
    const char* env = getenv("TDX_RING_Z4");
    if (env && atoi(env) == 0) return false;
    const int NT = Cout % 64 == 0 ? 2 : 1, bx = NT == 2 ? 16 : 32;
    if (X < bx || Y < 8 || Z < 4 || (X % bx) > 2 || (Y % 8) > 2 || (Z % 4) > 2) return false;
    const int ntn = Cout / (32 * NT);
    if (ntn > tdx_persistent_cus() / 8) return false;
    if ((int64_t)X * Y * Z * 1024 >= (1ll << 31)) return false;
    if (mode == 2) return true;
    if (NT == 1 && std::max(C1, C2) > 32) return false;
    const int64_t nb = (int64_t)B * (X / bx) * (Y / 8) * (Z / 4);
    return nb * ntn >= 192 && (C1 + C2) >= 64;
}
static int ring_brick_depth(int C1, int C2, int Cout, int B, int X, int Y, int Z) {
    const char* env = getenv("TDX_CONV3_RING");
    const int mode = env ? atoi(env) : 1;
    if (mode == 0 || !conv3_mfma_supported(C1, C2, Cout)) return 0;
    const char* z4 = getenv("TDX_RING_Z4");
    if (z4 && atoi(z4) == 2 && ring_z4_supported(C1, C2, Cout, B, X, Y, Z, 2)) return 4;
    if (ring_z8_supported(C1, C2, Cout, B, X, Y, Z, mode)) return 8;
    return ring_z4_supported(C1, C2, Cout, B, X, Y, Z, mode) ? 4 : 0;
}
int conv3_ring_depth(int C1, int C2, int N, int B, int X, int Y, int Z, bool data_gradient) {
    if (data_gradient && (tdx_scratch_ptr() == nullptr || tdx_scratch_bytes() < 16)) return 0;
    return ring_brick_depth(C1, C2, N, B, X, Y, Z);
}
static bool ring_z8_supported(int C1, int C2, int Cout, int B, int X, int Y, int Z, int mode) {
    const int NT = Cout % 64 == 0 ? 2 : 1, bx = NT == 2 ? 8 : 16;
    if (X < bx || Y < 8 || Z < 8 || (X % bx) > 2 || (Y % 8) > 2 || (Z % 8) > 2) return false;
    const char* rag = getenv("TDX_RING_RAGGED");
    if (rag && atoi(rag) == 0 && ((X % bx) || (Y % 8) || (Z % 8))) return false;
    const int ntn = Cout / (32 * NT);
    if (ntn > tdx_persistent_cus() / 8) return false;
    if ((int64_t)X * Y * Z * 1024 >= (1ll << 31)) return false;
    if (mode == 2) return true;
    if (NT == 1 && std::max(C1, C2) > 32) return false;
    const int64_t nb = (int64_t)B * (X / bx) * (Y / 8) * (Z / 8);
    const char* mi = getenv("TDX_RING_MIN_ITEMS");
    return nb * ntn >= (mi ? atoi(mi) : 3 * 256);
}

#ifdef RG_STAMPS
static unsigned long long* rg_stamp_buffer = nullptr;
#endif

template <int NT, bool ZP, int LW, bool HF, bool Z4 = false>
static int ring_go(const RingArgs& a, hipStream_t st) {
    size_t lds = RingShape<NT, LW, Z4>::LDS;
#ifdef RG_STAMPS
    if (NT == 1) lds += (size_t)RG_WAVES * RG_NSTAMP * 8;
#endif
    auto kern = conv3_ring_kernel<NT, ZP, LW, HF, Z4>;
    static bool attr_set = false;
    if (!attr_set) {
        hipError_t e = hipFuncSetAttribute((const void*)kern, hipFuncAttributeMaxDynamicSharedMemorySize, (int)lds);
        if (e != hipSuccess) return (int)e;
        attr_set = true;
    }
    const int px = tdx_persistent_cus() / 8, grid = 8 * (px - px % a.ntn);
    hipLaunchKernelGGL(kern, dim3(grid), dim3(512 + 64 * LW), lds, st, a);
    return tdx_launch_status();
}

int conv3_ring_launch(const Conv3Call& c, int depth) {
    if ((depth != 4 && depth != 8) || !tdx_is_h16(c.fmt)) return TDX_EINVAL;
    if (c.zero_pad && (tdx_scratch_ptr() == nullptr || tdx_scratch_bytes() < 16)) return TDX_EINVAL;
    const int X = c.X, Y = c.Y, Z = c.Z;
    const bool zero_pad = c.zero_pad, hf = c.hf();
    hipStream_t st = c.st;
    const int NT = c.N % 64 == 0 ? 2 : 1;
    const int bxr = (NT == 2 ? 8 : 16) * (depth == 4 ? 2 : 1);
    RingArgs a;
    a.x1 = (const bf16*)c.x1; a.x2 = (const bf16*)c.x2; a.C1 = c.C1; a.C2 = c.C2;
    a.wp = (const bf16*)c.wp; a.bias = c.bias; a.y = (bf16*)c.y;
    a.B = c.B; a.X = X; a.Y = Y; a.Z = Z; a.Cout = c.N;
    a.nbx = X / bxr; a.nby = Y / 8; a.nbz = Z / depth; a.ntn = c.N / (32 * NT);
    a.gn_acc = c.gn_acc;
    a.d1 = (bf16*)c.d1; a.d2 = (bf16*)c.d2; a.D1 = c.D1; a.a1 = (const bf16*)c.a1; a.a2 = (const bf16*)c.a2;
    a.zeros = tdx_scratch_ptr();
    a.stamps = nullptr;
#ifdef RG_STAMPS
    a.stamps = rg_stamp_buffer;
#endif
    const char* env = getenv("TDX_RING_LOADERS");
    const bool lw = env ? atoi(env) != 0 : RG_DEFAULT_LOADERS;
    int rc;
    if (depth == 4) {
#define RG_Z4(NTV) (hf ? (zero_pad ? ring_go<NTV, true, 4, true, true>(a, st) : ring_go<NTV, false, 4, true, true>(a, st)) \
                       : (zero_pad ? ring_go<NTV, true, 4, false, true>(a, st) : ring_go<NTV, false, 4, false, true>(a, st)))
        rc = NT == 2 ? RG_Z4(2) : RG_Z4(1);
#undef RG_Z4
    } else if (hf) {
        if (NT == 2) rc = zero_pad ? ring_go<2, true, 4, true>(a, st) : ring_go<2, false, 4, true>(a, st);
        else rc = zero_pad ? ring_go<1, true, 4, true>(a, st) : ring_go<1, false, 4, true>(a, st);
    } else if (NT == 2) {
        if (lw) rc = zero_pad ? ring_go<2, true, 4, false>(a, st) : ring_go<2, false, 4, false>(a, st);
        else rc = zero_pad ? ring_go<2, true, 0, false>(a, st) : ring_go<2, false, 0, false>(a, st);
    } else {
        if (lw) rc = zero_pad ? ring_go<1, true, 4, false>(a, st) : ring_go<1, false, 4, false>(a, st);
        else rc = zero_pad ? ring_go<1, true, 0, false>(a, st) : ring_go<1, false, 0, false>(a, st);
    }
    if (rc != TDX_OK || ((X % bxr) == 0 && (Y % 8) == 0 && (Z % depth) == 0)) return rc;
    const int beyond[3] = {X - X % bxr, Y - Y % 8, Z - Z % depth};
    Conv3Call rest = c;
    rest.slabs_beyond = beyond;
    return conv3_mfma_launch(rest);
}

extern "C" int tdx_conv3_uses_ring(int C1, int C2, int Cout, int B, int X, int Y, int Z) {
    return ring_brick_depth(C1, C2, Cout, B, X, Y, Z) != 0 ? 1 : 0;
}
extern "C" int tdx_conv3_ring_brick_depth(int C1, int C2, int Cout, int B, int X, int Y, int Z) {
    return ring_brick_depth(C1, C2, Cout, B, X, Y, Z);
}
```

### generative-turbulence_amd/csrc/tdx_conv3_wgrad_ring.hip

```cpp
#include "tdx_conv3_wgrad.h"
#include <stdlib.h>
#include <algorithm>
#include <type_traits>

typedef WgradBrick<4> WR;
#define WR_NSTEPS (WR::NVOX / 16)
#define WR_XPIECES ((WR::NHALO * 4 + 63) / 64)
#define WR_XBUF (WR_XPIECES * 1024)
#define WR_XPW ((WR_XPIECES + 3) / 4)
#define WR_CW 8
#define WR_GBUF(NTN) ((NTN) * WR::GPLANE)
#define WR_GPW(NTN) (4 * (NTN))
#define WR_SLOTS(NTN) ((NTN) == 2 ? 7 : 4)

template <int NTN, bool HF>
__global__ void __launch_bounds__(768, 3)
conv3_wgrad_ring_kernel(const bf16* __restrict__ x1, int C1, const bf16* __restrict__ x2, int C2, const bf16* __restrict__ dy,
                        float* __restrict__ dwp, float* __restrict__ dbias, WgradView gv, int Cout, int nsplit, int n_ci_tiles,
                        int64_t slab_stride, const void* __restrict__ zeros) {
    extern __shared__ __attribute__((aligned(1024))) unsigned char smem[];
    unsigned char* sX = smem;
    unsigned char* sG = smem + 2 * WR_XBUF;
    constexpr int GBUF = WR_GBUF(NTN), GPW = WR_GPW(NTN), SLOTS = WR_SLOTS(NTN);
    const unsigned lds0 = lds_addr(smem);
// ... 78 lines not shown

    auto run = [&](auto odd_c) {
        constexpr bool ODD = decltype(odd_c)::value;
        int it = 0;
        for (int brick = split; brick < nbricks; brick += nsplit, ++it) {
            lds_barrier();
            const unsigned char* bX = sX + (it & 1) * WR_XBUF;
            const unsigned char* bG = sG + (it & 1) * GBUF + b_row;
            auto step_off = [&](int s) { return wgrad_x_step_offset<WR>(s); };
            auto read_a = [&](int s, int t) {
                const unsigned char* ap = bX + a_off[t] + step_off(s);
                return tr_frag(ap, ap + 4 * 64);
            };
            auto read_b = [&](int s, int nt) {
                const unsigned char* bp = bG + nt * WR::GPLANE + s * (16 * 64);
                return tr_frag(bp, bp + 4 * 64);
            };
            bf16x8 A[4], Bq[2][NTN];
#pragma unroll
            for (int t = 0; t < 4; ++t) A[t] = read_a(0, t);
#pragma unroll
            for (int nt = 0; nt < NTN; ++nt) Bq[0][nt] = read_b(0, nt);

            auto step = [&](int s, int cur) {
                const int sn = min(s + 1, WR_NSTEPS - 1), nx = cur ^ 1;
#pragma unroll
                for (int nt = 0; nt < NTN; ++nt) Bq[nx][nt] = read_b(sn, nt);
                __builtin_amdgcn_sched_group_barrier(0x100, 2 * NTN, 0);
                if constexpr (NTN == 2) {
                    const bf16x8 a6 = bias_slot ? ones : A[3];
                    const bf16x8 b6 = bias_slot ? (wave == 7 ? Bq[cur][1] : Bq[cur][0]) : (ODD ? Bq[cur][1] : Bq[cur][0]);
                    if (!ODD) {
                        acc[0] = H16<HF>::mfma(A[0], Bq[cur][0], acc[0]);
                        acc[1] = H16<HF>::mfma(A[0], Bq[cur][1], acc[1]);
                        A[0] = read_a(sn, 0);
                        __builtin_amdgcn_sched_group_barrier(0x008, 2, 0); __builtin_amdgcn_sched_group_barrier(0x100, 2, 0);
                        acc[2] = H16<HF>::mfma(A[1], Bq[cur][0], acc[2]);
                        acc[3] = H16<HF>::mfma(A[1], Bq[cur][1], acc[3]);
                        A[1] = read_a(sn, 1);
                        __builtin_amdgcn_sched_group_barrier(0x008, 2, 0); __builtin_amdgcn_sched_group_barrier(0x100, 2, 0);
                        acc[4] = H16<HF>::mfma(A[2], Bq[cur][0], acc[4]);
                        acc[5] = H16<HF>::mfma(A[2], Bq[cur][1], acc[5]);
                        A[2] = read_a(sn, 2);
                        __builtin_amdgcn_sched_group_barrier(0x008, 2, 0); __builtin_amdgcn_sched_group_barrier(0x100, 2, 0);
                        acc[6] = H16<HF>::mfma(a6, b6, acc[6]);
                        A[3] = read_a(sn, 3);
                        __builtin_amdgcn_sched_group_barrier(0x008, 1, 0); __builtin_amdgcn_sched_group_barrier(0x100, 2, 0);
                    } else {
                        acc[0] = H16<HF>::mfma(A[0], Bq[cur][1], acc[0]);
                        A[0] = read_a(sn, 0);
                        __builtin_amdgcn_sched_group_barrier(0x008, 1, 0); __builtin_amdgcn_sched_group_barrier(0x100, 2, 0);
                        acc[1] = H16<HF>::mfma(A[1], Bq[cur][0], acc[1]);
                        acc[2] = H16<HF>::mfma(A[1], Bq[cur][1], acc[2]);
                        A[1] = read_a(sn, 1);
                        __builtin_amdgcn_sched_group_barrier(0x008, 2, 0); __builtin_amdgcn_sched_group_barrier(0x100, 2, 0);
                        acc[3] = H16<HF>::mfma(A[2], Bq[cur][0], acc[3]);
                        acc[4] = H16<HF>::mfma(A[2], Bq[cur][1], acc[4]);
                        A[2] = read_a(sn, 2);
                        __builtin_amdgcn_sched_group_barrier(0x008, 2, 0); __builtin_amdgcn_sched_group_barrier(0x100, 2, 0);
                        acc[5] = H16<HF>::mfma(A[3], Bq[cur][0], acc[5]);
                        acc[6] = H16<HF>::mfma(a6, b6, acc[6]);
                        A[3] = read_a(sn, 3);
                        __builtin_amdgcn_sched_group_barrier(0x008, 2, 0); __builtin_amdgcn_sched_group_barrier(0x100, 2, 0);
                    }
                } else {
#pragma unroll
                    for (int t = 0; t < 3; ++t) {
                        acc[t] = H16<HF>::mfma(A[t], Bq[cur][0], acc[t]);
                        A[t] = read_a(sn, t);
                        __builtin_amdgcn_sched_group_barrier(0x008, 1, 0); __builtin_amdgcn_sched_group_barrier(0x100, 2, 0);
                    }
                    if (ODD) {
                        acc[3] = H16<HF>::mfma(bias_slot ? ones : A[3], Bq[cur][0], acc[3]);
                        A[3] = read_a(sn, 3);
                        __builtin_amdgcn_sched_group_barrier(0x008, 1, 0); __builtin_amdgcn_sched_group_barrier(0x100, 2, 0);
                    }
                }
            };
#pragma unroll 1
            for (int s2 = 0; s2 < WR_NSTEPS / 2; ++s2) {
                step(2 * s2, 0);
                step(2 * s2 + 1, 1);
            }
        }
    };
    if (NTN == 2 ? odd : (cnt == 4 || bias_slot)) run(std::true_type{}); else run(std::false_type{});

    const int r = lane & 31, hh = lane >> 5;
#pragma unroll
    for (int i = 0; i < SLOTS; ++i) {
        const int T = first + i;
        if (i < cnt) {
            const int ltap = T / NTN, nt = T % NTN;
            const int tap = wgrad_global_tap(gv, ltap);
#pragma unroll
            for (int e = 0; e < 16; ++e) {
                const int ci = ci0 + (e & 3) + 8 * (e >> 2) + 4 * hh;
                if (ci >= Cin) continue;
                float* dst = &dwp[((int64_t)tap * Cin + ci) * Cout + co0 + nt * 32 + r];
                if (slab_stride) dst[(int64_t)split * slab_stride] = acc[i][e];
                else atomicAdd(dst, acc[i][e]);
            }
        } else if (bias_slot && i == SLOTS - 1 && dbias != nullptr && ci0 == 0 && hh == 0) {
            atomicAdd(&dbias[co0 + (NTN == 2 ? (wave - 6) * 32 : 0) + r], acc[i][0]);
        }
    }
}

bool conv3_wgrad_ring_supported(int C1, int C2, int Cout) {
    const char* env = getenv("TDX_WGRAD_RING");
    if (env && atoi(env) == 0) return false;
    return conv3_wgrad_mfma_supported(C1, C2, Cout) && (Cout % 32) == 0 && tdx_scratch_ptr() != nullptr && tdx_scratch_bytes() >= 16;
}

int conv3_wgrad_ring_launch(const Conv3WgradCall& c) {
    const int Cout = c.Cout;
    if (!conv3_wgrad_ring_supported(c.C1, c.C2, Cout)) return TDX_ESHAPE;
    const int Cin = c.C1 + c.C2;
    WgradView g;
    const int nbricks = conv3_wgrad_view(g, c, WR::BX, WR::BY, WR::BZ);
    const int NTN = (Cout % 64) == 0 ? 2 : 1;
    {
        const char* env = getenv("TDX_WGRAD_RING");
        if (NTN == 1 && env && atoi(env) == 2) return TDX_ESHAPE;
    }
    const int n_ci = (Cin + 31) / 32, n_co = Cout / (32 * NTN);
    const int ntiles = n_ci * n_co;
    const int cus = tdx_persistent_cus();
    int nsplit = cus >= 256 ? (256 + ntiles - 1) / ntiles : std::max(cus / ntiles, 1);
    if (nsplit > nbricks) nsplit = nbricks;
    if (nsplit < 1) nsplit = 1;
    if (nbricks < 4 * nsplit) return TDX_ESHAPE;
    const size_t lds = (size_t)2 * WR_XBUF + (size_t)2 * WR_GBUF(NTN);
    int64_t slab_stride;
    float* out = conv3_wgrad_merge(c, nsplit, slab_stride);
    static bool attr_set[2][2] = {{false, false}, {false, false}};
#define WR_GO(NTNV, HFV)                                                                                                          \
    do {                                                                                                                          \
        auto kern = conv3_wgrad_ring_kernel<NTNV, HFV>;                                                                           \
        if (!attr_set[NTNV - 1][HFV]) {                                                                                           \
            hipError_t e = hipFuncSetAttribute((const void*)kern, hipFuncAttributeMaxDynamicSharedMemorySize, (int)lds);          \
            if (e != hipSuccess) return (int)e;                                                                                   \
            attr_set[NTNV - 1][HFV] = true;                                                                                       \
        }                                                                                                                         \
        hipLaunchKernelGGL(kern, dim3((unsigned)(ntiles * nsplit)), dim3(768), lds, c.st, (const bf16*)c.x1, c.C1,                \
                           (const bf16*)c.x2, c.C2, (const bf16*)c.dy, out, c.dbias, g, Cout, nsplit, n_ci, slab_stride,          \
                           tdx_scratch_ptr());                                                                                    \
    } while (0)
    if (NTN == 2) { if (c.hf) WR_GO(2, true); else WR_GO(2, false); }
    else { if (c.hf) WR_GO(1, true); else WR_GO(1, false); }
#undef WR_GO
    return tdx_launch_status();
}
```

### generative-turbulence_amd/turbdiff_amd/_lib.py

```python

from __future__ import annotations

import ctypes as C
import os
import threading
from pathlib import Path

import torch

_HERE = Path(__file__).resolve().parent
LIB_PATH = Path(os.environ.get("TDX_LIB", _HERE / "libtdx_hip.so"))

F32, BF16 = 0, 1
F16 = 3
CONV_AUTO, CONV_DIRECT, CONV_MFMA, CONV_SPLIT = 0, 1, 2, 3
F32_SPLIT = 2
WS_CLEAN = 0x100

_vp, _i, _i64, _u64, _f, _sz = C.c_void_p, C.c_int, C.c_int64, C.c_uint64, C.c_float, C.c_size_t

SIGNATURES = {
    "tdx_version": (_i, []),
    "tdx_arch": (C.c_char_p, []),
    "tdx_set_scratch": (_i, [_vp, _sz]),
    "tdx_ncv_to_nvc": (_i, [_vp, _vp, _i, _i, _i64, _i, _i, _vp]),
    "tdx_nvc_to_ncv": (_i, [_vp, _vp, _i, _i, _i64, _i, _i, _vp]),
    "tdx_cast": (_i, [_vp, _vp, _i64, _i, _i, _vp]),
    "tdx_conv3_pack_weight": (_i, [_vp, _vp, _vp, _i, _i, _i, _vp]),
    "tdx_conv3_pack_weights": (_i, [_vp, _i, _i, _vp]),
    "tdx_transpose_many": (_i, [_vp, _i, _vp]),
    "tdx_conv3_fwd": (_i, [_vp, _i, _vp, _i, _vp, _vp, _vp, _i, _i, _i, _i, _i, _i, _i, _vp]),
    "tdx_conv3_uses_ring": (_i, [_i] * 7),
    "tdx_conv3_ring_brick_depth": (_i, [_i] * 7),
    "tdx_conv3_fwd_kernel": (_i, [_i] * 9),
    "tdx_conv3_fwd_gn": (_i, [_vp, _i, _vp, _i, _vp, _vp, _vp, _vp, _i, _f, _vp, _i, _i, _i, _i, _i, _i, _i, _vp]),
    "tdx_conv3_fwd_partial": (_i, [_vp, _i, _i, _vp, _vp, _vp, _i, _vp, _vp, _i, _f, _vp, _i, _i, _i, _i, _i, _i, _i, _vp]),
    "tdx_conv3_bwd_data_workspace_bytes": (_sz, [_i, _i, _i, _i, _i, _i, _i]),
    "tdx_conv3_bwd_data": (_i, [_vp, _vp, _vp, _i, _vp, _i, _i, _i, _i, _i, _i, _i, _i, _i, _vp, _vp]),
    "tdx_conv3_bwd_data_add": (_i, [_vp, _vp, _vp, _i, _vp, _i, _vp, _vp, _i, _i, _i, _i, _i, _i, _i, _vp, _vp]),
    "tdx_conv3_bwd_weight_workspace_bytes": (_sz, [_i, _i, _i]),
    "tdx_conv3_bwd_weight": (_i, [_vp, _i, _vp, _i, _vp, _vp, _vp, _i, _i, _i, _i, _i, _i, _i, _vp, _vp]),
    "tdx_conv1_fwd": (_i, [_vp, _i, _vp, _i, _vp, _i, _vp, _vp, _vp, _i64, _i, _i, _vp]),
    "tdx_conv1_fwd_gn": (_i, [_vp, _i, _vp, _i, _vp, _i, _vp, _vp, _vp, _vp, _vp, _i, _vp, _i, _i64, _i, _i, _vp]),
    "tdx_conv1_bwd_weight": (_i, [_vp, _i, _vp, _i, _vp, _i, _vp, _i64, _i, _vp]),
    "tdx_conv1_bwd_weight_oc": (_i, [_vp, _i, _vp, _i, _vp, _i, _vp, _i, _i64, _i, _vp]),
    "tdx_encode_fwd": (_i, [_vp, _i, _vp, _vp, _vp, _i, _vp, _vp, _vp, _i, _i64, _i, _i, _vp]),
    "tdx_encode_bwd": (_i, [_vp, _vp, _i, _vp, _i, _vp, _vp, _vp, _vp, _vp, _vp, _i, _i64, _i, _i, _vp]),
    "tdx_decode_fwd": (_i, [_vp, _vp, _vp, _vp, _i, _i64, _i, _i, _i, _vp]),
    "tdx_decode_bwd": (_i, [_vp, _vp, _vp, _vp, _vp, _vp, _i, _i64, _i, _i, _i, _vp]),
    "tdx_gn_workspace_bytes": (_sz, [_i, _i]),
    "tdx_gn_stats": (_i, [_vp, _vp, _i, _i64, _i, _i, _f, _i, _vp, _vp]),
    "tdx_gn_apply": (_i, [_vp, _vp, _vp, _vp, _vp, _vp, _vp, _vp, _i, _i64, _i, _i, _i, _i, _vp]),
    "tdx_gn_apply_decode": (_i, [_vp, _vp, _vp, _vp, _vp, _vp, _vp, _vp, _i, _i64, _i, _i, _i, _i, _vp]),
    "tdx_gn_apply_encoded": (_i, [_vp, _vp, _vp, _vp, _vp, _i, _vp, _vp, _vp, _i, _vp, _vp, _vp, _i, _i64, _i, _i, _i, _vp]),
    "tdx_gn_bwd": (_i, [_vp] * 12 + [_i, _i64, _i, _i, _i, _i, _vp, _vp]),
    "tdx_resize_fwd": (_i, [_vp, _vp] + [_i] * 9 + [_vp]),
    "tdx_resize_bwd": (_i, [_vp, _vp, _vp] + [_i] * 9 + [_vp]),
    "tdx_attn_fwd": (_i, [_vp, _vp, _vp, _i, _i, _i, _i, _i, _vp]),
    "tdx_attn_bwd": (_i, [_vp, _vp, _vp, _vp, _vp, _i, _i, _i, _i, _i, _vp, _vp]),
    "tdx_attn_bwd_workspace_bytes": (_sz, [_i, _i, _i, _i]),
    "tdx_cell_mask": (_i, [_vp, _i64, _vp, _i64, _vp]),
    "tdx_q_sample": (_i, [_vp, _vp, _vp, _vp, _vp, _i, _vp, _i, _vp, _i, _i, _i64, _vp]),
    "tdx_p_sample_step": (_i, [_vp] * 7 + [_i, _vp, _i, _i, _vp, _i, _i, _i64, _vp]),
    "tdx_p_sample_step_rng": (_i, [_vp] * 5 + [_i, _vp, _i, _i, _vp, _i, _i, _i64, _u64, _vp, _vp, _vp]),
    "tdx_p_sample_step_lv": (_i, [_vp] * 8 + [_i, _vp, _i, _i, _vp, _i, _i, _i64, _vp]),
    "tdx_p_sample_step_lv_rng": (_i, [_vp] * 6 + [_i, _vp, _i, _i, _vp, _i, _i, _i64, _u64, _vp, _vp, _vp]),
    "tdx_ddim_step": (_i, [_vp] * 7 + [_i, _vp, _vp, _vp, _i, _i, _vp, _i, _i, _i64, _vp]),
    "tdx_ddim_step_rng": (_i, [_vp] * 5 + [_i, _vp, _vp, _vp, _i, _i, _vp, _i, _i, _i64, _u64, _vp, _vp, _vp]),
    "tdx_masked_loss": (_i, [_vp, _vp, _vp, _i64, _i, _vp, _vp, _i, _i, _i64, _vp, _vp]),
    "tdx_masked_loss_dyn": (_i, [_vp, _vp, _vp, _vp, _i, _vp, _vp, _i, _i, _i64, _vp, _vp]),
    "tdx_masked_loss_workspace_bytes": (_sz, []),
    "tdx_elbo_loss": (_i, [_vp] * 5 + [_i64, _vp, _vp, _vp, _i, _i, _i, _i, C.c_double, _vp, _vp, _i, _i, _i64, _vp, _vp]),
    "tdx_elbo_loss_dyn": (_i, [_vp] * 5 + [_vp, _vp, _vp, _vp, _i, _i, _i, _i, C.c_double, _vp, _vp, _i, _i, _i64, _vp, _vp]),
    "tdx_elbo_loss_workspace_bytes": (_sz, []),
    "tdx_grid_embed": (_i, [_vp, _i, _vp, _i, _vp, _i, _vp, _i, _vp, _vp, _vp, _vp, _vp, _vp, _vp, _i, _i64, _i64, _vp]),
    "tdx_grid_select": (_i, [_vp, _vp, _vp, _vp, _vp, _i, _vp, _i, _vp, _i, _vp, _i, _i, _i64, _i64, _vp]),
    "tdx_cell_embed_fwd": (_i, [_vp, _vp, _vp, _i, _i, _i64, _vp]),
    "tdx_cell_embed_bwd_workspace_bytes": (_sz, [_i, _i]),
    "tdx_cell_embed_bwd": (_i, [_vp, _vp, _vp, _i, _i, _i, _i64, _vp, _vp]),
    "tdx_tke_energy": (_i, [_vp, _vp, _i, _i64, _vp]),
    "tdx_tke_sphere": (_i, [_vp, _vp, _vp, _vp, _vp, _i, _i, _i, _i, _i, _i, _vp]),
    "tdx_fd": (_i, [_vp, _vp, _i, _i, _i, _i, _f, _f, _f, _f, _i, _vp]),
    "tdx_ot_features": (_i, [_vp, _vp, _vp, _vp, _vp, _vp, _i, _i64, _i, _i, _i, _f, _f, _f, _vp]),
    "tdx_ot_workspace_bytes": (_sz, [_i, _i]),
    "tdx_ot_auction": (_i, [_vp, _vp, _i64, _vp, _vp, _i, _vp, _i, _i, _i, C.c_double, _i, _i64, _vp, _i, _i, _vp, _vp, _vp]),
    "tdx_randn": (_i, [_vp, _i64, _u64, _u64, _vp, _vp]),
    "tdx_randn_batched": (_i, [_vp, _i, _i64, _u64, _vp, _vp, _vp]),
    "tdx_convg_apply": (_i, [_vp, _vp, _vp, _vp] + [_i] * 16 + [_vp]),
    "tdx_convg_fold_clamp": (_i, [_vp, _vp, _i, _i, _i, _i, _i, _i, _i, _vp]),
    "tdx_convg_bwd_weight": (_i, [_vp, _vp, _vp, _vp] + [_i] * 15 + [_vp]),
    "tdx_convg_apply_fused": (_i, [_vp, _vp, _vp, _vp] + [_i] * 13 + [_vp, _i, _vp]),
    "tdx_convg_fold_fused": (_i, [_vp] * 6 + [_i] * 7 + [_vp]),
    "tdx_film_supported": (_i, [_i, _i]),
    "tdx_film_fwd": (_i, [_vp, _i, _i, _vp, _i, _vp]),
    "tdx_film_bwd_workspace_bytes": (_sz, [_i, _i, _vp, _i]),
    "tdx_film_bwd": (_i, [_vp, _i, _i, _vp, _i, _vp, _vp, _vp]),
    "tdx_opt_chunk_elems": (_i64, []),
    "tdx_grad_norm": (_i, [_vp, _vp, _vp, _i, _f, _vp, _vp, _vp]),
    "tdx_radam_step": (_i, [_vp, _vp, _vp, _i, _vp, _i64, _f, _f, _f, _f, _i, _vp]),
    "tdx_signal_host": (_i, [_vp, _vp, C.c_uint32, _vp]),
    "tdx_stage_scaled": (_i, [_vp, _i, _f, _vp]),
    "tdx_grad_norm_scaled": (_i, [_vp, _vp, _vp, _i, _f, _f, _vp, _vp, _vp]),
    "tdx_radam_step_scaled": (_i, [_vp, _vp, _vp, _i, _vp, _i64, _f, _f, _f, _f, _i, _vp]),
}

FILM_MAX_LAYERS = 32


class FilmLayer(C.Structure):
    _fields_ = [("weight", _vp), ("bias", _vp), ("out", _vp), ("channels", _i)]


class PackJob(C.Structure):
    _fields_ = [("w", _vp), ("wf", _vp), ("wb", _vp), ("Cin", _i), ("Cout", _i)]


class TransposeJob(C.Structure):
    _fields_ = [("src", _vp), ("dst", _vp), ("rows", _i), ("cols", _i)]


class StageItem(C.Structure):
    _fields_ = [("src", _vp), ("dst", _vp), ("n", _i64)]


class FilmGrad(C.Structure):
    _fields_ = [("weight", _vp), ("grad_out", _vp), ("grad_weight", _vp), ("grad_bias", _vp), ("channels", _i)]


_lib = None


def load() -> C.CDLL:
    global _lib
    if _lib is None:
        if not LIB_PATH.exists():
            raise RuntimeError(
                f"{LIB_PATH} not found: the HIP kernels have not been built. "
                "Run `python -c 'import __graft_entry__ as g; g.build()'` (or `make -C generative-turbulence_amd/csrc`)."
            )
        lib = C.CDLL(str(LIB_PATH))
        lax = "TDX_LIB" in os.environ and os.environ.get("TDX_LIB_LAX") == "1"
        for name, (res, args) in SIGNATURES.items():
            if lax and not hasattr(lib, name):
                continue
            fn = getattr(lib, name)
            fn.restype = res
            fn.argtypes = args
        _lib = lib
    return _lib


_SCRATCH: "OrderedDict" = None
_ACTIVE = None
SCRATCH_BYTES = int(os.environ.get("TDX_SCRATCH_MB", "96")) << 20
SCRATCH_SMALL_BYTES = 4096
SCRATCH_MAX_ARENAS = int(os.environ.get("TDX_SCRATCH_MAX_ARENAS", "6"))
ARENA_USERS = {"tdx_conv3_fwd", "tdx_conv3_fwd_gn", "tdx_conv3_fwd_partial", "tdx_conv3_bwd_data", "tdx_conv3_bwd_data_add",
               "tdx_conv3_bwd_weight", "tdx_attn_fwd"}
DET_ARENA_USERS = {"tdx_conv1_bwd_weight", "tdx_conv1_bwd_weight_oc", "tdx_encode_bwd", "tdx_decode_bwd", "tdx_gn_stats"}


def deterministic() -> bool:
    return os.environ.get("TDX_DETERMINISTIC", "0") not in ("", "0")


_LAUNCH_LOCK = threading.RLock()
_SMALL_STREAMS = set()


def declare_zero_block_only(stream) -> None:
    _SMALL_STREAMS.add((stream.device.index, stream.cuda_stream))


def ensure_scratch(device=None) -> None:
    global _SCRATCH, _ACTIVE
    if _SCRATCH is None:
        from collections import OrderedDict

        _SCRATCH = OrderedDict()
    idx = torch.cuda.current_device() if device is None else torch.device(device).index
    idx = torch.cuda.current_device() if idx is None else idx
    key = (idx, stream(idx))
    if _ACTIVE == key:
        return
    if SCRATCH_BYTES <= 0:
        load().tdx_set_scratch(None, 0)
        _ACTIVE = key
# ... 175 lines not shown
```

### generative-turbulence_amd/turbdiff_amd/models/ddpm.py

```python

from __future__ import annotations

import math
import os
from dataclasses import dataclass
from functools import partial

import torch
import torch.nn.functional as F
from torch import nn

from .. import _lib, ops, schedules
from ..sequential import KwargsSequential
from .conditioning import global_conditioning, local_conditioning
from .utils import broadcast_right


@dataclass
class ModelPrediction:
    noise: torch.Tensor
    x_start: torch.Tensor
    mean: torch.Tensor
    log_var: torch.Tensor

# ... 183 lines not shown
        self.extract_features = nn.Sequential(
            nn.Conv3d(in_features, out_features, kernel_size=5, stride=5),
            actfn(),
            nn.Conv3d(out_features, out_features, kernel_size=5, stride=1),
            actfn(),
            nn.Conv3d(out_features, out_features, kernel_size=5, stride=5),
        )

    def forward(self, c_local):
        front = torch.narrow(c_local, dim=-3, start=0, length=50)
        return self.extract_features(front).mean(dim=(-3, -2, -1))




class DenoisingModel(nn.Module):

    def __init__(self, *, in_features: int, out_features: int, c_local_features: int, c_global_features: int,
                 timesteps: int, dim: int, u_net_levels: int, actfn=nn.SiLU, norm_type: str = "instance",
                 with_geometry_embedding: bool = False):
        super().__init__()
        self.in_features = in_features
        self.out_features = out_features
        self.c_local_features = c_local_features
        self.c_global_features = c_global_features
        self.dim = dim
        self.timesteps = timesteps
        self.u_net_levels = u_net_levels
        self.with_geometry_embedding = with_geometry_embedding
        self.compute_dtype = torch.float32
        self.conv_impl = None

        groups_of = {"instance": lambda ch: ch, "layer": lambda ch: 1, "group": lambda ch: 8}
        if norm_type not in groups_of:
            raise RuntimeError(f"Unknown norm type {norm_type}")
        norm_klass = lambda ch: nn.GroupNorm(groups_of[norm_type](ch), ch)

        self.encode_x = nn.Conv3d(in_features, dim, 1)
        c_local_dim = 0
        if c_local_features > 0:
            self.encode_c_local = nn.Conv3d(c_local_features, dim, 1)
            c_local_dim = dim
        c_dim = dim
        self.encode_t = NyquistFrequencyEmbedding(dim, timesteps)
        if c_global_features > 0:
            self.encode_c_global = nn.Linear(c_global_features, dim)
            c_dim += dim
        if with_geometry_embedding and c_local_features > 0:
            self.geometry_embedding = GeometryEmbedding(c_local_features, dim, actfn)
            c_dim += dim
        self.process_c = nn.Sequential(nn.Linear(c_dim, 4 * c_dim), actfn(), nn.Linear(4 * c_dim, c_dim), actfn())

        rb = partial(ResnetBlock, c_dim=c_dim, actfn=actfn, norm_klass=norm_klass)
        self.decode = KwargsSequential(rb(dim, dim), nn.Conv3d(dim, out_features, 1))
        down = [rb(dim + c_local_dim, dim * 2)] + [rb(dim * 2**i, dim * 2 ** (i + 1)) for i in range(1, u_net_levels)]
        up = [rb(2 * dim * 2 ** (i + 1), dim * 2**i) for i in reversed(range(u_net_levels))]
        mid = dim * 2**u_net_levels
        center = KwargsSequential(rb(mid, mid), Residual(PreNorm(norm_klass(mid), Attention(mid))), rb(mid, mid))
        self.u_net = UNet(down, up, center)

    def grad_ready_order(self):
        mods = [self.decode[1], self.decode[0]]
        mods += list(reversed(self.u_net.upsampling_blocks))
        mods += list(reversed(list(self.u_net.center_block)))
        mods += list(reversed(self.u_net.downsampling_blocks))
        mods += [getattr(self, n) for n in ("encode_c_local", "encode_x") if hasattr(self, n)]
        film = {id(p) for m in self.modules() if isinstance(m, ResnetBlock) for p in m.project_onto_scale_shift.parameters()}
        late = []
        for m in mods:
            for p in reversed(list(m.parameters())):
                if id(p) in film:
                    late.append(p)
                else:
                    yield p
        yield from late
        for n in ("geometry_embedding", "encode_c_global", "process_c"):
            if hasattr(self, n):
                yield from reversed(list(getattr(self, n).parameters()))

    def __getstate__(self):
        state = super().__getstate__()
        state.pop("_lists", None)
        return state

    def _static_lists(self):
        hit = self.__dict__.get("_lists")
        if hit is None:
            conv3, conv1, blocks = [], [], []
            for m in self.modules():
                if isinstance(m, Block):
                    conv3.append(m.conv)
                elif isinstance(m, ResnetBlock):
                    blocks.append(m)
                    if not isinstance(m.conv, nn.Identity):
                        conv1.append(m.conv)
                elif isinstance(m, Attention):
                    conv1 += [m.to_qkv, m.to_out]
            hit = self.__dict__["_lists"] = (conv3, conv1, blocks, {})
        return hit

    def prefetch_weights(self, skip_first_conv: bool):
        conv3, conv1, _, plans = self._static_lists()
        first = self.u_net.downsampling_blocks[0].block1.conv if skip_first_conv else None
        key = (bool(skip_first_conv), self.compute_dtype, _lib.pack_code(self.compute_dtype))
        plans[key] = ops.prefetch_weights([m.weight for m in conv3 if m is not first], [m.weight for m in conv1],
                                          self.compute_dtype, plans.get(key))

    def film_table(self, c):
        blocks = self._static_lists()[2]
        films = ops.film_projections(c, [b.project_onto_scale_shift for b in blocks])
        return {id(b): f for b, f in zip(blocks, films)}

    def set_compute_dtype(self, dtype: torch.dtype):
        assert dtype in (torch.float32, torch.bfloat16, torch.float16)
        self.compute_dtype = dtype
        return self

    def conditioning_vector(self, t, C, batch_size):
        parts = [self.encode_t(t)]
        c_global = global_conditioning(C)
        if c_global is not None:
            parts.append(self.encode_c_global(c_global))
        if self.with_geometry_embedding:
            c_local = local_conditioning(C)
            if c_local is not None:
                parts.append(self.geometry_embedding(c_local).expand((batch_size, -1)))
        return self.process_c(parts[0] if len(parts) == 1 else torch.cat(parts, dim=-1))

    def conditioning_table(self, C, timesteps: int):
        if global_conditioning(C) is not None or self.with_geometry_embedding:
            return None
        dev = next(self.parameters()).device
        return self.conditioning_vector(torch.arange(timesteps, device=dev), C, timesteps)

    def encode_local(self, C):
        with _lib.conv_impl_scope(self.conv_impl):
            return self._encode_local(C)

    def _encode_local(self, C):
        c_local = local_conditioning(C)
        if c_local is None:
            return None
        cl = ops.to_nvc(c_local[None].float(), self.compute_dtype)
        enc = ops.conv1(cl, self.encode_c_local.weight, self.encode_c_local.bias)
        first = self.u_net.downsampling_blocks[0]
        n_lead = self.encode_x.out_channels
        if (CACHE_COND_CONV and not torch.is_grad_enabled() and isinstance(first, ResnetBlock) and first.fused()
                and first.block1.conv.in_channels == n_lead + enc.shape[-1]
                and ops.conv3_partial_supported(enc, first.block1.conv.weight, n_lead)):
            enc.first_conv_partial = (n_lead, ops.conv3_shared_tail(enc, first.block1.conv.weight, n_lead))
        return enc


    def compose_first_conv(self, x, c_local):
        first = self.u_net.downsampling_blocks[0]
        D = self.encode_x.out_channels
        if not (COMPOSE_FIRST_CONV and isinstance(first, ResnetBlock) and first.fused() and c_local is not None
                and isinstance(first.conv, nn.Identity) and self.in_features <= 8 and self.c_local_features <= 8
                and first.block1.conv.in_channels == D + self.encode_c_local.out_channels):
            return None
        dev, P = x.device, (16 if c_local.requires_grad else 8)
        eye = getattr(self, "_raw_eye", None)
        if eye is None or eye[0].device != dev or eye[0].shape[0] != P:
            ex = torch.zeros(P, self.in_features, 1, 1, 1, device=dev)
            ec = torch.zeros(P, self.c_local_features, 1, 1, 1, device=dev)
            ex[: self.in_features, :, 0, 0, 0] = torch.eye(self.in_features, device=dev)
            ec[: self.c_local_features, :, 0, 0, 0] = torch.eye(self.c_local_features, device=dev)
            Co_ = first.block1.conv.out_channels
            nx, nc = self.in_features, self.c_local_features
            idx = list(range(nx)) + [nx + nc] * (P - nx) + list(range(nx, nx + nc)) + [nx + nc] * (P - nc)
            eye = self._raw_eye = (ex, ec, torch.zeros(P, device=dev), torch.zeros(Co_, 1, 3, 3, 3, device=dev),
                                   torch.tensor(idx, dtype=torch.long, device=dev))
        if not ops.encode_supported(x, c_local, eye[0]):
            return None
        raw = ops.encode(x, c_local, eye[0], eye[2], eye[1], eye[2], self.compute_dtype)
        W1, b1 = first.block1.conv.weight, first.block1.conv.bias
        frozen = not torch.is_grad_enabled()
        if frozen:
            made_of = (W1, b1, self.encode_x.weight, self.encode_x.bias, self.encode_c_local.weight, self.encode_c_local.bias)
            key = (P,) + tuple((id(p), p._version, p.data_ptr()) for p in made_of)
            hit = getattr(self, "_composed_frozen", None)
            if hit is not None and hit[0] == key:
                return raw, hit[1], hit[2], self.in_features + self.c_local_features
        w_enc = torch.block_diag(self.encode_x.weight.flatten(1), self.encode_c_local.weight.flatten(1))
        b_enc = torch.cat((self.encode_x.bias, self.encode_c_local.bias))
        w8 = torch.einsum("octuv,ck->oktuv", W1, w_enc)
        w_eff = torch.cat((w8, eye[3]), dim=1).index_select(1, eye[4])
        b_eff = b1 + torch.einsum("octuv,c->o", W1, b_enc)
        if frozen:
            self._composed_frozen = (key, w_eff, b_eff)
        return raw, w_eff, b_eff, self.in_features + self.c_local_features

    def forward(self, x: torch.Tensor, t: torch.Tensor, C, encoded_local=None, cond=None):
        with _lib.conv_impl_scope(self.conv_impl):
            return self._forward(x, t, C, encoded_local, cond)

    def _forward(self, x: torch.Tensor, t: torch.Tensor, C, encoded_local=None, cond=None):
        B = x.shape[0]
        c = self.conditioning_vector(t, C, B) if cond is None else cond
        c_local = local_conditioning(C) if self.c_local_features > 0 else None
        first_conv = first_skip = None
        if ops.encode_supported(x, c_local, self.encode_x.weight):
            wc = self.encode_c_local.weight if c_local is not None else None
            bc = self.encode_c_local.bias if c_local is not None else None
            first_conv = self.compose_first_conv(x, c_local)
            if first_conv is not None and DEFER_ENCODE:
                first_skip = ops.encode_deferred(x, c_local, self.encode_x.weight, self.encode_x.bias, wc, bc,
                                                 self.compute_dtype)
                h = first_skip.standin
            else:
                h = ops.encode(x, c_local, self.encode_x.weight, self.encode_x.bias, wc, bc, self.compute_dtype)
        else:
            h = ops.conv1(ops.to_nvc(x, self.compute_dtype), self.encode_x.weight, self.encode_x.bias)
            e = encoded_local if encoded_local is not None else self.encode_local(C)
            if e is not None:
                h = torch.cat((h, e.expand(B, -1, -1, -1, -1)), dim=-1)
        partial = getattr(encoded_local, "first_conv_partial", None) if not torch.is_grad_enabled() else None
        self.prefetch_weights(skip_first_conv=first_conv is not None)
        films = self.film_table(c)
        h = self.u_net(h, c, first_partial=partial, first_conv=first_conv, films=films, first_skip=first_skip)
        last = self.decode[0]
        if (FUSE_DECODE and isinstance(last, ResnetBlock) and last.fused() and isinstance(last.conv, nn.Identity)
                and self.decode[1].bias is not None and ops.decode_fused_supported(last.dim_out, self.decode[1].weight)):
            return last(h, c, films=films, decode_wb=(self.decode[1].weight, self.decode[1].bias))
        h = last(h, c, films=films)
        if ops.decode_supported(h, self.decode[1].weight):
            return ops.decode(h, self.decode[1].weight, self.decode[1].bias)
        y = ops.conv1(h, self.decode[1].weight, self.decode[1].bias)
        return ops.to_ncv(y, torch.float32)




def linear_beta_schedule(timesteps):
    return schedules.betas_for("linear", timesteps)


def log_linear_beta_schedule(timesteps):
    return schedules.betas_for("log-linear", timesteps)


def log_snr_linear_beta_schedule(timesteps, snr_1=1e3, snr_T=1e-5):
    assert (snr_1, snr_T) == (1e3, 1e-5), "only the reference's default SNR end points are tabulated"
    return schedules.betas_for("log-snr-linear", timesteps)


def cosine_beta_schedule(timesteps, s=0.008):
    assert s == 0.008
    return schedules.betas_for("cosine", timesteps)


def sigmoid_beta_schedule(timesteps, start=-3, end=3, tau=1, clamp_min=1e-5):
    assert (start, end, tau) == (-3, 3, 1)
    return schedules.betas_for("sigmoid", timesteps)


def normal_kl(mean1, logvar1, mean2, logvar2):
    return 0.5 * (logvar2 - logvar1 - 1.0 + torch.exp(logvar1 - logvar2) + (mean1 - mean2) ** 2 * torch.exp(-logvar2))


def normal_log_lk(x, mean, log_var):
    return -0.5 * (log_var + math.log(2 * math.pi) + (x - mean) ** 2 * torch.exp(-log_var))


def batch_mean(x: torch.Tensor):
    return x.flatten(1).mean(dim=1)




GRAPH_SAMPLER = os.environ.get("TDX_GRAPH_SAMPLER", "1") != "0"
MAX_GRAPH_SAMPLERS = 3


class GaussianDiffusion(nn.Module):

    def __init__(self, model, *, timesteps: int = 1000, loss_type: str = "l2", beta_schedule: str = "sigmoid",
                 clip_denoised: bool = False, noise_bcs: bool = False, learned_variances: bool = False,
                 elbo_weight: float | None = None, detach_elbo_mean: bool = True):
        super().__init__()
        self.model = model
        self.clip_denoised = clip_denoised
        self.noise_bcs = noise_bcs
        self.learned_variances = learned_variances
        self.elbo_weight = elbo_weight
        self.detach_elbo_mean = detach_elbo_mean
        self.num_timesteps = timesteps
        self.beta_schedule = beta_schedule
        self.loss_type = loss_type
        if loss_type not in ("l1", "l2"):
            raise ValueError(f"invalid loss type {loss_type}")
        tables = schedules.diffusion_tables(beta_schedule, timesteps)
        for name, tab in tables.items():
            self.register_buffer(name, tab, persistent=False)
        self.register_buffer("step_tables", schedules.pack_step_tables(tables), persistent=False)
        self._mask_cache = None
        self._graph_samplers = None

    def graph_samplers(self):
        cache = self.__dict__.get("_graph_samplers")
        if cache is None:
            from collections import OrderedDict

            cache = self.__dict__["_graph_samplers"] = OrderedDict()
        return cache

    def __getstate__(self):
        state = super().__getstate__()
        state["_graph_samplers"] = None
        state["_mask_cache"] = None
        return state

    def domain_mask(self, cell_idx: torch.Tensor, V: int):
        c = self._mask_cache
        if c is None or c[0] is not cell_idx or c[1] != cell_idx._version or c[2] != V:
            c = self._mask_cache = (cell_idx, cell_idx._version, V, ops.cell_mask(cell_idx, V), int(cell_idx.numel()))
        return c[3], c[4]

    @property
    def loss_fn(self):
        return F.l1_loss if self.loss_type == "l1" else F.mse_loss

    def predict_start_from_noise(self, x_t, t, noise):
        return (broadcast_right(self.sqrt_recip_alphas_cumprod[t], x_t) * x_t
                - broadcast_right(self.sqrt_recipm1_alphas_cumprod[t], x_t) * noise)

    def predict_noise_from_start(self, x_t, t, x0):
        return ((broadcast_right(self.sqrt_recip_alphas_cumprod[t], x_t) * x_t - x0)
                / broadcast_right(self.sqrt_recipm1_alphas_cumprod[t], x_t))

    def q_posterior(self, x_start, x_t, t):
        mean = (broadcast_right(self.posterior_mean_coef1[t], x_t) * x_start
                + broadcast_right(self.posterior_mean_coef2[t], x_t) * x_t)
        return mean, broadcast_right(self.posterior_log_var[t], x_t)

    def q_sample(self, x_start, t, noise):
        return ops.q_sample(x_start, noise, self.sqrt_alphas_cumprod, self.sqrt_one_minus_alphas_cumprod, t)

    def _outside_keep(self, mask, inside_vals, outside_vals):
        m = mask.view(inside_vals.shape[-3:]).bool()
        return torch.where(m, inside_vals, outside_vals)
# ... 252 lines not shown
```

### generative-turbulence_amd/turbdiff_amd/ops.py

```python

from __future__ import annotations

import weakref

import os

import torch
from torch.autograd.function import once_differentiable

from . import _lib as L


def _ws(nbytes: int, device) -> torch.Tensor:
    return torch.empty(max(int(nbytes), 16), dtype=torch.uint8, device=device)


_CLEAN = {}
WS_CLEAN = 0 if os.environ.get("TDX_WS_CLEAN", "1") == "0" else L.WS_CLEAN


def _clean_ws(nbytes: int, device, tag=None) -> torch.Tensor:
    if not WS_CLEAN:
        return _ws(nbytes, device)
    key = (device, L.stream(device.index), int(nbytes), tag)
# ... 65 lines not shown
               Cout, code, impl, L.ptr(ws), st, work=work)
    return gx1, gx2


def _conv3_wgrad_out(wshape, has_bias, dev):
    return (torch.empty(wshape, dtype=torch.float32, device=dev),
            torch.empty(wshape[0], dtype=torch.float32, device=dev) if has_bias else None)


def _conv3_wgrad_ws(Cin, Cout, impl, dev):
    return _clean_ws(L.query("tdx_conv3_bwd_weight_workspace_bytes", Cin, Cout, impl), dev, ("w3", Cin, Cout))


def _conv3_wgrad(x1, C1, x2, C2, gy, gw, gb, grid, Cout, code, impl, ws, st, real=None):
    B, X, Y, Z = grid
    L.call("tdx_conv3_bwd_weight", L.ptr(x1), C1, L.ptr(x2), C2, L.ptr(gy), L.ptr(gw), L.ptr(gb), B, X, Y, Z, Cout, code,
           impl | WS_CLEAN, L.ptr(ws), st, work=54.0 * (real or (C1 + C2)) * Cout * B * X * Y * Z)


def _conv1_fwd(x1, C1, x2, C2, w, ldw, col, bias, add, lead, rows, Cout, code, st):
    y = x1.new_empty((*lead, Cout))
    L.call("tdx_conv1_fwd", L.ptr(x1), C1, L.ptr(x2), C2, L.ptr(w) + 4 * col, ldw, L.ptr(bias), L.ptr(add), L.ptr(y), rows, Cout,
           code, st)
    return y


def _gn_apply(x, stats, gamma, beta, scale, shift, res, B, V, Cc, groups, act, code, st):
    y = torch.empty_like(x)
    L.call("tdx_gn_apply", L.ptr(x), L.ptr(stats), L.ptr(gamma), L.ptr(beta), L.ptr(scale), L.ptr(shift), L.ptr(res), L.ptr(y),
           B, V, Cc, groups, act, code, st)
    return y


def _gn_bwd(x, gy, stats, gamma, beta, scale, shift, dscale, dshift, B, V, Cc, groups, act, code, st, ws=None):
    gx, dgamma, dbeta = torch.empty_like(x), stats.new_empty(Cc), stats.new_empty(Cc)
    if ws is None:
        ws = _gn_ws(B, Cc, x.device)
    L.call("tdx_gn_bwd", L.ptr(x), L.ptr(gy), L.ptr(stats), L.ptr(gamma), L.ptr(beta), L.ptr(scale), L.ptr(shift), L.ptr(gx),
           L.ptr(dgamma), L.ptr(dbeta), L.ptr(dscale), L.ptr(dshift), B, V, Cc, groups, act, code, L.ptr(ws), st)
    return gx, dgamma, dbeta


def _resize_fwd(x, size):
    B, Xi, Yi, Zi, Cc = _grid(x)
    Xo, Yo, Zo = (int(s) for s in size)
    y = torch.empty((B, Xo, Yo, Zo, Cc), dtype=x.dtype, device=x.device)
    L.call("tdx_resize_fwd", L.ptr(x), L.ptr(y), B, Xi, Yi, Zi, Xo, Yo, Zo, Cc, L.dtype_code(x.dtype), L.stream())
    return y, (B, Xi, Yi, Zi, Xo, Yo, Zo, Cc)


def _resize_bwd(gy, add, geom):
    B, Xi, Yi, Zi, Xo, Yo, Zo, Cc = geom
    gx = torch.empty((B, Xi, Yi, Zi, Cc), dtype=gy.dtype, device=gy.device)
    L.call("tdx_resize_bwd", L.ptr(gy), L.ptr(add), L.ptr(gx), B, Xi, Yi, Zi, Xo, Yo, Zo, Cc, L.dtype_code(gy.dtype), L.stream())
    return gx




class _ToNVC(torch.autograd.Function):

    @staticmethod
    def forward(ctx, x, dtype):
        ctx.in_dtype = x.dtype
        return _to_nvc(x.contiguous(), dtype)

    @staticmethod
    @once_differentiable
    def backward(ctx, gy):
        return _to_ncv(gy.contiguous(), ctx.in_dtype), None


class _ToNCV(torch.autograd.Function):

    @staticmethod
    def forward(ctx, x, dtype):
        ctx.in_dtype = x.dtype
        return _to_ncv(x.contiguous(), dtype)

    @staticmethod
    @once_differentiable
    def backward(ctx, gy):
        return _to_nvc(gy.contiguous(), ctx.in_dtype), None


def to_nvc(x: torch.Tensor, dtype: torch.dtype) -> torch.Tensor:
    return _ToNVC.apply(x, dtype)


def to_ncv(x: torch.Tensor, dtype: torch.dtype = torch.float32) -> torch.Tensor:
    return _ToNCV.apply(x, dtype)




class _Encode(torch.autograd.Function):

    @staticmethod
    def forward(ctx, x, c_local, wx, bx, wc, bc, dtype, lazy=None):
        B, Fx, X, Y, Z = x.shape
        V, D = X * Y * Z, wx.shape[0]
        x = x.contiguous().float()
        has_c = c_local is not None
        c = c_local.contiguous().float() if has_c else None
        wx2, bx2 = wx.detach().reshape(D, Fx).contiguous(), bx.detach().contiguous()
        wc2 = wc.detach().reshape(D, -1).contiguous() if has_c else None
        bc2 = bc.detach().contiguous() if has_c else None
        if lazy is not None:
            lazy.extend((x, Fx, wx2, bx2, c, c.shape[0] if has_c else 0, wc2, bc2, D))
            y = torch.empty(1, dtype=dtype, device=x.device).expand(B, X, Y, Z, 2 * D if has_c else D)
        else:
            y = torch.empty((B, X, Y, Z, 2 * D if has_c else D), dtype=dtype, device=x.device)
            L.call("tdx_encode_fwd", L.ptr(x), Fx, L.ptr(wx2), L.ptr(bx2), L.ptr(c), c.shape[0] if has_c else 0, L.ptr(wc2),
                   L.ptr(bc2), L.ptr(y), B, V, D, L.dtype_code(dtype), L.stream())
        ctx.save_for_backward(x, c, wc2)
        ctx.shapes = (tuple(wx.shape), tuple(wc.shape) if has_c else None, tuple(c_local.shape) if has_c else None)
        return y

    @staticmethod
    @once_differentiable
    def backward(ctx, gy):
        x, c, wc2 = ctx.saved_tensors
        wx_shape, wc_shape, c_shape = ctx.shapes
        B, Fx = x.shape[:2]
        V = x[0, 0].numel()
        D = wx_shape[0]
        gy = gy.contiguous()
        dev = gy.device
        dwx = torch.empty(wx_shape, dtype=torch.float32, device=dev)
        dbx = torch.empty(D, dtype=torch.float32, device=dev)
        has_c = c is not None
        dwc = torch.empty(wc_shape, dtype=torch.float32, device=dev) if has_c else None
        dbc = torch.empty(D, dtype=torch.float32, device=dev) if has_c else None
        dc = torch.empty(c_shape, dtype=torch.float32, device=dev) if (has_c and ctx.needs_input_grad[1]) else None
        L.call("tdx_encode_bwd", L.ptr(gy), L.ptr(x), Fx, L.ptr(c), c.shape[0] if has_c else 0, L.ptr(wc2), L.ptr(dwx),
               L.ptr(dbx), L.ptr(dwc), L.ptr(dbc), L.ptr(dc), B, V, D, L.dtype_code(gy.dtype), L.stream())
        return None, dc, dwx, dbx, dwc, dbc, None, None


class DeferredEncoding:

    def __init__(self, standin, operands):
        self.standin, self.operands = standin, tuple(operands)


def encode_deferred(x, c_local, wx, bx, wc, bc, dtype) -> DeferredEncoding:
    ops_ = []
    standin = _Encode.apply(x, c_local, wx, bx, wc, bc, dtype, ops_)
    return DeferredEncoding(standin, ops_)


def encode_supported(x, c_local, wx):
    D = wx.shape[0]
    n = (2 * D if c_local is not None else D) // 8
    return (x.shape[1] == 4 and (c_local is None or c_local.shape[0] == 4) and D % 8 == 0 and n & (n - 1) == 0
            and n <= 64 and not x.requires_grad)


def encode(x, c_local, wx, bx, wc, bc, dtype):
    return _Encode.apply(x, c_local, wx, bx, wc, bc, dtype)


class _Decode(torch.autograd.Function):

    @staticmethod
    def forward(ctx, h, w, bias):
        B, X, Y, Z, D = h.shape
        F = w.shape[0]
        h = h.contiguous()
        w2 = w.detach().reshape(F, D).contiguous()
        y = torch.empty((B, F, X, Y, Z), dtype=torch.float32, device=h.device)
        L.call("tdx_decode_fwd", L.ptr(h), L.ptr(w2), L.ptr(bias.detach().contiguous()), L.ptr(y), B, X * Y * Z, D, F,
               L.dtype_code(h.dtype), L.stream())
        ctx.save_for_backward(h, w2)
        ctx.wshape = tuple(w.shape)
        return y

    @staticmethod
    @once_differentiable
    def backward(ctx, gy):
        h, w2 = ctx.saved_tensors
        B, X, Y, Z, D = h.shape
        F = w2.shape[0]
        gy = gy.contiguous().float()
        dh = torch.empty_like(h)
        dw = torch.empty(ctx.wshape, dtype=torch.float32, device=h.device)
        db = torch.empty(F, dtype=torch.float32, device=h.device)
        L.call("tdx_decode_bwd", L.ptr(gy), L.ptr(h), L.ptr(w2), L.ptr(dh), L.ptr(dw), L.ptr(db), B, X * Y * Z, D, F,
               L.dtype_code(h.dtype), L.stream())
        return dh, dw, db


def decode_supported(h, w):
    n = h.shape[-1] // 8
    return w.shape[0] == 4 and h.shape[-1] % 8 == 0 and n & (n - 1) == 0 and n <= 64


def decode(h, w, bias):
    return _Decode.apply(h, w, bias)


def decode_fused_supported(C: int, w) -> bool:
    n = C // 8
    return (not torch.is_grad_enabled() and w.shape[0] == 4 and w.shape[1] == C and C % 8 == 0 and n & (n - 1) == 0
            and n <= 64)



_pack_cache: dict = {}


def _cached(key, weight):
    hit = _pack_cache.get(key)
    if hit is not None and hit[0]() is weight and hit[1] == weight._version and hit[2] == weight.data_ptr():
        return hit[3], hit[4]
    return None


def _cache_store(key, weight, a, b=None):
    _pack_cache[key] = (weakref.ref(weight), weight._version, weight.data_ptr(), a, b)


def _packed_conv3(weight: torch.Tensor, dtype: torch.dtype):
    code = L.pack_code(dtype)
    key = (id(weight), dtype, code)
    hit = _cached(key, weight)
    if hit is not None:
        return hit
    Cout, Cin = weight.shape[0], weight.shape[1]
    w = weight.detach().contiguous()
    wf = torch.empty(27 * Cin * Cout, dtype=dtype, device=w.device)
    wb = torch.empty(27 * Cin * Cout, dtype=dtype, device=w.device)
    L.call("tdx_conv3_pack_weight", L.ptr(w), L.ptr(wf), L.ptr(wb), Cin, Cout, code, L.stream())
    if len(_pack_cache) > 4096:
        _pack_cache.clear()
    _cache_store(key, weight, wf, wb)
    return wf, wb


def _packed_conv3_cin_slice(weight: torch.Tensor, lo: int, hi: int, dtype: torch.dtype):
    code = L.pack_code(dtype)
    key = (id(weight), dtype, lo, hi, code)
    hit = _cached(key, weight)
    if hit is not None:
        return hit[0]
    Cout, Cin = weight.shape[0], hi - lo
    w = weight.detach()[:, lo:hi].contiguous()
    wf = torch.empty(27 * Cin * Cout, dtype=dtype, device=w.device)
    L.call("tdx_conv3_pack_weight", L.ptr(w), L.ptr(wf), None, Cin, Cout, code, L.stream())
    _cache_store(key, weight, wf)
    return wf


class PackPlan:

    def __init__(self, conv3_weights, conv1_weights, dtype: torch.dtype):
        self.dtype, self.code = dtype, L.pack_code(dtype)
        self.w3, self.w1 = list(conv3_weights), list(conv1_weights)
        for w in self.w3 + self.w1:
            assert w.is_cuda and w.dtype == torch.float32 and w.is_contiguous(), "fp32 contiguous device parameters"
        self.ops3 = [(torch.empty(27 * w.shape[1] * w.shape[0], dtype=dtype, device=w.device),
                      torch.empty(27 * w.shape[1] * w.shape[0], dtype=dtype, device=w.device)) for w in self.w3]
        self.ops1 = [torch.empty((w[0].numel(), w.shape[0]), dtype=torch.float32, device=w.device) for w in self.w1]
        self.tab3 = (L.PackJob * max(len(self.w3), 1))(*[L.PackJob(w.data_ptr(), wf.data_ptr(), wb.data_ptr(), w.shape[1], w.shape[0])
                                                         for w, (wf, wb) in zip(self.w3, self.ops3)])
        self.tab1 = (L.TransposeJob * max(len(self.w1), 1))(*[L.TransposeJob(w.data_ptr(), wt.data_ptr(), w.shape[0], w[0].numel())
                                                              for w, wt in zip(self.w1, self.ops1)])
        self.ptrs = [w.data_ptr() for w in self.w3 + self.w1]
        self.seen3, self.seen1 = [None] * len(self.w3), [None] * len(self.w1)

    def valid_for(self, conv3_weights, conv1_weights, dtype) -> bool:
        ws = list(conv3_weights) + list(conv1_weights)
        return (dtype == self.dtype and L.pack_code(dtype) == self.code and len(ws) == len(self.ptrs)
                and all(a is b for a, b in zip(ws, self.w3 + self.w1)) and all(w.data_ptr() == p for w, p in zip(ws, self.ptrs)))

    def refresh(self) -> None:
        if self.w3 and any(w._version != v for w, v in zip(self.w3, self.seen3)):
            L.call("tdx_conv3_pack_weights", self.tab3, len(self.w3), self.code, L.stream())
            for i, (w, (wf, wb)) in enumerate(zip(self.w3, self.ops3)):
                self.seen3[i] = w._version
                _cache_store((id(w), self.dtype, self.code), w, wf, wb)
        if self.w1 and any(w._version != v for w, v in zip(self.w1, self.seen1)):
            L.call("tdx_transpose_many", self.tab1, len(self.w1), L.stream())
            for i, (w, wt) in enumerate(zip(self.w1, self.ops1)):
                self.seen1[i] = w._version
                _cache_store((id(w), "wt"), w, wt)


def prefetch_weights(conv3_weights, conv1_weights, dtype: torch.dtype, plan: "PackPlan | None" = None) -> "PackPlan | None":
    if plan is None or not plan.valid_for(conv3_weights, conv1_weights, dtype):
        plan = PackPlan(conv3_weights, conv1_weights, dtype)
    plan.refresh()
    if len(_pack_cache) > 4096:
        _pack_cache.clear()
    return plan


def conv3_partial_supported(x, weight, n_lead: int) -> bool:
    return (x.dtype in L.H16_DTYPES and n_lead % 16 == 0 and weight.shape[0] % 32 == 0 and x.shape[-1] % 8 == 0
            and L.conv_impl() != L.CONV_DIRECT)


def conv3_shared_tail(e, weight, n_lead: int):
    Cin = weight.shape[1]
    B, X, Y, Z, Ce = _grid(e)
    assert B == 1 and Ce == Cin - n_lead
    wf = _packed_conv3_cin_slice(weight, n_lead, Cin, e.dtype)
    return _conv3_fwd(e.contiguous(), Ce, None, 0, wf, None, (1, X, Y, Z), weight.shape[0], L.dtype_code(e.dtype), L.conv_impl(),
                      L.stream(), timed=False)


class _Conv3(torch.autograd.Function):
    @staticmethod
    def forward(ctx, x1, x2, weight, bias, gn_groups=0, gn_eps=1e-5):
        B, X, Y, Z, C1 = _grid(x1)
        C2 = 0 if x2 is None else x2.shape[-1]
        Cout = weight.shape[0]
        assert weight.shape[1] == C1 + C2 and tuple(weight.shape[2:]) == (3, 3, 3)
        x1 = x1.contiguous()
        x2 = None if x2 is None else x2.contiguous()
        wf, wb = _packed_conv3(weight, x1.dtype)
        ctx.save_for_backward(x1, x2, wb)
        ctx.has_bias = bias is not None
        ctx.wshape = tuple(weight.shape)
        impl = ctx.impl = L.conv_impl()
        out = _conv3_fwd(x1, C1, x2, C2, wf, bias, (B, X, Y, Z), Cout, L.dtype_code(x1.dtype), impl, L.stream(),
                         gn=(gn_groups, gn_eps) if gn_groups else None)
        if gn_groups:
            ctx.mark_non_differentiable(out[1])
        return out

    @staticmethod
    @once_differentiable
    def backward(ctx, gy, _gstats=None):
        x1, x2, wb = ctx.saved_tensors
        B, X, Y, Z, C1 = _grid(x1)
        C2 = 0 if x2 is None else x2.shape[-1]
        Cout, Cin = ctx.wshape[0], ctx.wshape[1]
        gy = gy.contiguous()
        grid, code, impl, st, dev = (B, X, Y, Z), L.dtype_code(gy.dtype), ctx.impl, L.stream(), gy.device
        gx1 = gx2 = gw = gb = None
        if ctx.needs_input_grad[0] or (x2 is not None and ctx.needs_input_grad[1]):
            gx1, gx2 = _conv3_bwd_data(gy, wb, x1, C1, x2, C2, grid, Cout, code, impl, st)
        if ctx.needs_input_grad[2]:
            gw, gb = _conv3_wgrad_out(ctx.wshape, ctx.has_bias, dev)
            _conv3_wgrad(x1, C1, x2, C2, gy, gw, gb, grid, Cout, code, impl, _conv3_wgrad_ws(Cin, Cout, impl, dev), st)
        return gx1, gx2, gw, gb, None, None


def conv3(x1, weight, bias=None, x2=None):
    return _Conv3.apply(x1, x2, weight, bias)


def conv3_gn_stats(x1, weight, bias, groups, eps=1e-5, x2=None):
    return _Conv3.apply(x1, x2, weight, bias, groups, eps)




def _conv1_wt(weight: torch.Tensor) -> torch.Tensor:
    key = (id(weight), "wt")
    hit = _cached(key, weight)
    if hit is not None:
        return hit[0]
    wt = weight.detach().reshape(weight.shape[0], -1).t().contiguous()
    _cache_store(key, weight, wt)
    return wt


def _conv1_weight_grad(x1, C1, x2, C2, gy, Cout, has_bias, rows, code, st):
    Cin = C1 + C2
    off = (Cout * Cin + 63) // 64 * 64
    buf = torch.zeros(off + (Cout if has_bias else 0), dtype=torch.float32, device=gy.device)
    gw = buf[: Cout * Cin].view(Cout, Cin)
    gb = buf[off:] if has_bias else None
    L.call("tdx_conv1_bwd_weight_oc", L.ptr(x1), C1, L.ptr(gy), Cout, gw.data_ptr(), Cin, L.ptr(gb), 1, rows, code, st)
    if x2 is not None:
        L.call("tdx_conv1_bwd_weight_oc", L.ptr(x2), C2, L.ptr(gy), Cout, gw.data_ptr() + 4 * C1, Cin, None, 1, rows, code, st)
    return gw, gb


class _Conv1(torch.autograd.Function):
    @staticmethod
    def forward(ctx, x1, x2, weight, bias, add):
        C1 = x1.shape[-1]
        C2 = 0 if x2 is None else x2.shape[-1]
        Cout = weight.shape[0]
        w2 = weight.detach().reshape(Cout, -1)
        assert w2.shape[1] == C1 + C2
        x1 = x1.contiguous()
        x2 = None if x2 is None else x2.contiguous()
        add = None if add is None else add.contiguous()
        lead = tuple(x1.shape[:-1])
        y = _conv1_fwd(x1, C1, x2, C2, _conv1_wt(weight), Cout, 0, bias, add, lead, x1.numel() // C1, Cout,
                       L.dtype_code(x1.dtype), L.stream())
        ctx.save_for_backward(x1, x2, w2.contiguous())
        ctx.has_bias = bias is not None
        ctx.has_add = add is not None
        ctx.wshape = tuple(weight.shape)
        return y

    @staticmethod
    @once_differentiable
    def backward(ctx, gy):
        x1, x2, w2 = ctx.saved_tensors
        C1 = x1.shape[-1]
        C2 = 0 if x2 is None else x2.shape[-1]
        Cout, Cin = w2.shape
        gy = gy.contiguous()
        lead, rows = tuple(gy.shape[:-1]), gy.numel() // Cout
        code, st = L.dtype_code(gy.dtype), L.stream()
        gx1 = gx2 = gw = gb = None
        if ctx.needs_input_grad[0]:
            gx1 = _conv1_fwd(gy, Cout, None, 0, w2, Cin, 0, None, None, lead, rows, C1, code, st)
        if x2 is not None and ctx.needs_input_grad[1]:
            gx2 = _conv1_fwd(gy, Cout, None, 0, w2, Cin, C1, None, None, lead, rows, C2, code, st)
        if ctx.needs_input_grad[2]:
            gw, gb = _conv1_weight_grad(x1, C1, x2, C2, gy, Cout, ctx.has_bias, rows, code, st)
            gw = gw.view(ctx.wshape)
        return gx1, gx2, gw, gb, (gy if ctx.has_add else None)


def conv1(x1, weight, bias=None, x2=None, add=None):
    return _Conv1.apply(x1, x2, weight, bias, add)




class _GnFilmSilu(torch.autograd.Function):
    @staticmethod
    def forward(ctx, x, gamma, beta, scale, shift, res, groups, act, eps, stats=None):
        B, X, Y, Z, Cc = _grid(x)
        V = X * Y * Z
        x = x.contiguous()
        res = None if res is None else res.contiguous()
        code, st = L.dtype_code(x.dtype), L.stream()
        gamma, beta = gamma.detach().contiguous(), beta.detach().contiguous()
        if scale is not None:
            scale = scale.detach().reshape(B, Cc).float().contiguous()
            shift = shift.detach().reshape(B, Cc).float().contiguous()
        if stats is None:
            stats = torch.empty((B, groups, 2), dtype=torch.float32, device=x.device)
            L.call("tdx_gn_stats", L.ptr(x), L.ptr(stats), B, V, Cc, groups, float(eps), code, L.ptr(_gn_ws(B, Cc, x.device)), st)
        y = _gn_apply(x, stats, gamma, beta, scale, shift, res, B, V, Cc, groups, int(act), code, st)
        ctx.save_for_backward(x, stats, gamma, beta, scale, shift)
        ctx.cfg = (groups, int(act), res is not None)
        return y

    @staticmethod
    @once_differentiable
    def backward(ctx, gy):
        x, stats, gamma, beta, scale, shift = ctx.saved_tensors
        groups, act, has_res = ctx.cfg
        B, X, Y, Z, Cc = _grid(x)
        gy = gy.contiguous()
        dscale = dshift = None
        if scale is not None:
            dscale, dshift = torch.empty_like(scale), torch.empty_like(shift)
        gx, dgamma, dbeta = _gn_bwd(x, gy, stats, gamma, beta, scale, shift, dscale, dshift, B, X * Y * Z, Cc, groups, act,
                                    L.dtype_code(x.dtype), L.stream())
        return gx, dgamma, dbeta, dscale, dshift, (gy if has_res else None), None, None, None, None


def gn_film_silu(x, gamma, beta, groups, scale=None, shift=None, res=None, act=True, eps=1e-5, stats=None):
    return _GnFilmSilu.apply(x, gamma, beta, scale, shift, res, groups, act, eps, stats)




class _Resize(torch.autograd.Function):
    @staticmethod
    def forward(ctx, x, size):
        y, ctx.geom = _resize_fwd(x.contiguous(), size)
        return y

    @staticmethod
    @once_differentiable
    def backward(ctx, gy):
        return _resize_bwd(gy.contiguous(), None, ctx.geom), None


def resize(x, size):
    return _Resize.apply(x, tuple(size))


class _SkipAndResize(torch.autograd.Function):

    @staticmethod
    def forward(ctx, x, size):
        x = x.contiguous()
        y, ctx.geom = _resize_fwd(x, size)
        ctx.set_materialize_grads(False)
        return x.view_as(x), y

    @staticmethod
    @once_differentiable
    def backward(ctx, g_skip, gy):
        if gy is None:
            return g_skip, None
        return _resize_bwd(gy.contiguous(), None if g_skip is None else g_skip.contiguous(), ctx.geom), None
# ... 585 lines not shown
```

### include/tdx.h

```cpp
#ifndef TDX_H
#define TDX_H

#include <stddef.h>
#include <stdint.h>

#ifdef __cplusplus
extern "C" {
#endif

#define TDX_F32 0
#define TDX_BF16 1

#define TDX_OK 0
#define TDX_EINVAL (-1)
#define TDX_ESHAPE (-2)
#define TDX_EDTYPE (-3)

#define TDX_CONV_AUTO 0
#define TDX_CONV_DIRECT 1
#define TDX_CONV_MFMA 2
#define TDX_CONV_SPLIT 3
#define TDX_F32_SPLIT 2
#define TDX_F16 3
#define TDX_WS_CLEAN 0x100

int tdx_version(void);
int tdx_set_scratch(void* ptr, size_t bytes);
const char* tdx_arch(void);

int tdx_ncv_to_nvc(const void* x, void* y, int B, int C, int64_t V, int dtype_in, int dtype_out, void* stream);
int tdx_nvc_to_ncv(const void* x, void* y, int B, int C, int64_t V, int dtype_in, int dtype_out, void* stream);
int tdx_cast(const void* x, void* y, int64_t n, int dtype_in, int dtype_out, void* stream);

int tdx_conv3_pack_weight(const float* w, void* wf, void* wb, int Cin, int Cout, int dtype, void* stream);
typedef struct {
    const float* w;
    void* wf;
    void* wb;
    int Cin, Cout;
} TdxPackJob;
int tdx_conv3_pack_weights(const TdxPackJob* jobs, int n, int dtype, void* stream);
typedef struct {
    const float* src;
    float* dst;
    int rows, cols;
} TdxTransposeJob;
int tdx_transpose_many(const TdxTransposeJob* jobs, int n, void* stream);

int tdx_conv3_fwd(const void* x1, int C1, const void* x2, int C2, const void* wf, const float* bias, void* y,
                  int B, int X, int Y, int Z, int Cout, int dtype, int impl, void* stream);

int tdx_conv3_uses_ring(int C1, int C2, int Cout, int B, int X, int Y, int Z);
int tdx_conv3_ring_brick_depth(int C1, int C2, int Cout, int B, int X, int Y, int Z);
#define TDX_KERNEL_DIRECT 0
#define TDX_KERNEL_BRICK 1
#define TDX_KERNEL_SMALL 2
#define TDX_KERNEL_RING 3
int tdx_conv3_fwd_kernel(int C1, int C2, int Cout, int B, int X, int Y, int Z, int dtype, int impl);

int tdx_conv3_fwd_gn(const void* x1, int C1, const void* x2, int C2, const void* wf, const float* bias, void* y,
                     float* stats, int G, float eps, void* gn_workspace, int B, int X, int Y, int Z, int Cout,
                     int dtype, int impl, void* stream);

int tdx_conv3_fwd_partial(const void* x1, int C1, int ld1, const void* wf, const float* bias, const void* init,
                          int init_shared, void* y, float* stats, int G, float eps, void* gn_workspace, int B, int X,
                          int Y, int Z, int Cout, int dtype, int impl, void* stream);

size_t tdx_conv3_bwd_data_workspace_bytes(int B, int X, int Y, int Z, int Cin, int dtype, int impl);
int tdx_conv3_bwd_data(const void* dy, const void* wb, void* dx1, int C1, void* dx2, int C2, int accumulate,
                       int B, int X, int Y, int Z, int Cout, int dtype, int impl, void* workspace, void* stream);

int tdx_conv3_bwd_data_add(const void* dy, const void* wb, void* dx1, int C1, void* dx2, int C2, const void* add1,
                           const void* add2, int B, int X, int Y, int Z, int Cout, int dtype, int impl,
                           void* workspace, void* stream);

size_t tdx_conv3_bwd_weight_workspace_bytes(int Cin, int Cout, int impl);
int tdx_conv3_bwd_weight(const void* x1, int C1, const void* x2, int C2, const void* dy, float* dw, float* dbias,
                         int B, int X, int Y, int Z, int Cout, int dtype, int impl, void* workspace, void* stream);

int tdx_conv1_fwd(const void* x1, int C1, const void* x2, int C2, const float* w, int ldw, const float* bias,
                  const void* add, void* y, int64_t rows, int Cout, int dtype, void* stream);
int tdx_conv1_fwd_gn(const void* x1, int C1, const void* x2, int C2, const float* w, int ldw, const float* bias,
                     const void* h, const float* stats, const float* gamma, const float* beta, int groups, void* y,
                     int B, int64_t V, int Cout, int dtype, void* stream);
int tdx_conv1_bwd_weight(const void* x, int Cin, const void* dy, int Cout, float* dw, int ldw, float* dbias,
                         int64_t rows, int dtype, void* stream);
int tdx_conv1_bwd_weight_oc(const void* x, int Cin, const void* dy, int Cout, float* dw, int ldw, float* dbias,
                            int accumulate, int64_t rows, int dtype, void* stream);

int tdx_encode_fwd(const float* x, int Fx, const float* wx, const float* bx, const float* c, int Fc, const float* wc,
                   const float* bc, void* y, int B, int64_t V, int D, int dtype, void* stream);
int tdx_encode_bwd(const void* dy, const float* x, int Fx, const float* c, int Fc, const float* wc, float* dwx,
                   float* dbx, float* dwc, float* dbc, float* dc, int B, int64_t V, int D, int dtype, void* stream);
int tdx_decode_fwd(const void* h, const float* w, const float* bias, float* y, int B, int64_t V, int D, int F, int dtype,
                   void* stream);
int tdx_decode_bwd(const float* dy, const void* h, const float* w, void* dh, float* dw, float* db, int B, int64_t V, int D,
                   int F, int dtype, void* stream);

size_t tdx_gn_workspace_bytes(int B, int C);
int tdx_gn_stats(const void* x, float* stats, int B, int64_t V, int C, int G, float eps, int dtype, void* workspace,
                 void* stream);
int tdx_gn_apply(const void* x, const float* stats, const float* gamma, const float* beta, const float* scale,
                 const float* shift, const void* res, void* y, int B, int64_t V, int C, int G, int act, int dtype,
                 void* stream);
int tdx_gn_apply_encoded(const void* x, const float* stats, const float* gamma, const float* beta, const float* x_raw, int Fx,
                         const float* wx, const float* bx, const float* c_raw, int Fc, const float* wc, const float* bc,
                         void* y, int B, int64_t V, int D, int G, int dtype, void* stream);
int tdx_gn_apply_decode(const void* x, const float* stats, const float* gamma, const float* beta, const void* res,
                        const float* w, const float* bias, float* out, int B, int64_t V, int C, int G, int F, int dtype,
                        void* stream);
int tdx_gn_bwd(const void* x, const void* dy, const float* stats, const float* gamma, const float* beta,
               const float* scale, const float* shift, void* dx, float* dgamma, float* dbeta, float* dscale,
               float* dshift, int B, int64_t V, int C, int G, int act, int dtype, void* workspace, void* stream);

int tdx_resize_fwd(const void* x, void* y, int B, int Xi, int Yi, int Zi, int Xo, int Yo, int Zo, int C, int dtype,
                   void* stream);
int tdx_resize_bwd(const void* dy, const void* add, void* dx, int B, int Xi, int Yi, int Zi, int Xo, int Yo, int Zo, int C,
                   int dtype, void* stream);

int tdx_attn_fwd(const void* qkv, void* out, float* lse, int B, int N, int H, int D, int dtype, void* stream);
int tdx_attn_bwd(const void* qkv, const void* out, const float* lse, const void* dout, void* dqkv, int B, int N, int H,
                 int D, int dtype, void* workspace, void* stream);
size_t tdx_attn_bwd_workspace_bytes(int B, int N, int H, int D);


int tdx_cell_mask(const int64_t* cell_idx, int64_t n_cells, uint8_t* mask, int64_t V, void* stream);

int tdx_q_sample(const float* x0, const float* noise, const float* sqrt_ac, const float* sqrt_1mac, const int64_t* t,
                 int t_stride, const uint8_t* mask, int keep_bcs, float* out, int B, int F, int64_t V, void* stream);

int tdx_p_sample_step(const float* x_t, const float* eps, const float* z, const float* z2, const float* x_bcs,
                      const uint8_t* mask, const float* sched, int T, const int64_t* t, int noise_bcs, int clip,
                      float* out, int B, int F, int64_t V, void* stream);

int tdx_p_sample_step_rng(const float* x_t, const float* eps, const float* x_bcs, const uint8_t* mask, const float* sched,
                          int T, int64_t* t, int noise_bcs, int clip, float* out, int B, int F, int64_t V, uint64_t seed,
                          const uint64_t* stream_ids, uint64_t* offset_dev, void* stream);

int tdx_p_sample_step_lv(const float* x_t, const float* model_out, const float* z, const float* z2, const float* x_bcs,
                         const uint8_t* mask, const float* sched, const float* posterior_log_var, int T, const int64_t* t,
                         int noise_bcs, int clip, float* out, int B, int F, int64_t V, void* stream);

int tdx_p_sample_step_lv_rng(const float* x_t, const float* model_out, const float* x_bcs, const uint8_t* mask,
                             const float* sched, const float* posterior_log_var, int T, int64_t* t, int noise_bcs, int clip,
                             float* out, int B, int F, int64_t V, uint64_t seed, const uint64_t* stream_ids,
                             uint64_t* offset_dev, void* stream);

int tdx_ddim_step(const float* x_t, const float* eps, const float* z, const float* z2, const float* x_bcs,
                  const uint8_t* mask, const float* tab, int S, const int64_t* k, const int64_t* tau, const int64_t* t,
                  int noise_bcs, int clip, float* out, int B, int F, int64_t V, void* stream);

int tdx_ddim_step_rng(const float* x_t, const float* eps, const float* x_bcs, const uint8_t* mask, const float* tab, int S,
                      int64_t* k, const int64_t* tau, int64_t* t, int noise_bcs, int clip, float* out, int B, int F,
                      int64_t V, uint64_t seed, const uint64_t* stream_ids, uint64_t* offset_dev, void* stream);

int tdx_masked_loss(const float* eps_hat, const float* noise, const uint8_t* mask, int64_t n_cells, int l1,
                    float* loss, float* grad, int B, int F, int64_t V, void* workspace, void* stream);
int tdx_masked_loss_dyn(const float* eps_hat, const float* noise, const unsigned char* mask, const int64_t* n_cells_dev,
                        int l1, float* loss, float* grad, int B, int F, int64_t V, void* workspace, void* stream);
size_t tdx_masked_loss_workspace_bytes(void);

int tdx_elbo_loss(const float* out, const float* noise, const float* x_start, const float* x_t, const uint8_t* mask,
                  int64_t n_cells, const int64_t* t, const float* sched, const float* posterior_log_var, int T, int l1,
                  int clip, int detach_mean, double elbo_weight, float* loss, float* grad, int B, int F, int64_t V,
                  void* workspace, void* stream);
int tdx_elbo_loss_dyn(const float* out, const float* noise, const float* x_start, const float* x_t, const uint8_t* mask,
                      const int64_t* n_cells_dev, const int64_t* t, const float* sched, const float* posterior_log_var,
                      int T, int l1, int clip, int detach_mean, double elbo_weight, float* loss, float* grad, int B, int F,
                      int64_t V, void* workspace, void* stream);
size_t tdx_elbo_loss_workspace_bytes(void);

int tdx_grid_embed(const float* s0, int d0, const float* s1, int d1, const float* s2, int d2, const float* s3, int d3,
                   const int32_t* cell_of, const int32_t* ovr_of, const float* ovr_val, const uint32_t* ovr_mask,
                   const float* shift, const float* scale, float* x, int B, int64_t n_cells, int64_t V, void* stream);
int tdx_grid_select(const float* x, const int64_t* cell_idx, const float* mean, const float* std, float* o0, int d0,
                    float* o1, int d1, float* o2, int d2, float* o3, int d3, int B, int64_t n_cells, int64_t V,
                    void* stream);
int tdx_cell_embed_fwd(const uint8_t* types, const float* table, float* out, int n_types, int D, int64_t V, void* stream);
size_t tdx_cell_embed_bwd_workspace_bytes(int n_types, int D);
int tdx_cell_embed_bwd(const uint8_t* types, const float* dC, float* dtable, int accumulate, int n_types, int D, int64_t V,
                       void* workspace, void* stream);

int tdx_tke_energy(const float* u, float* tke, int B, int64_t V, void* stream);
int tdx_tke_sphere(const float* fft, const float* p, const float* w, const float* k, float* E, int B, int X, int Y, int Z,
                   int N, int K, void* stream);

#define TDX_FD_CURL 0
#define TDX_FD_DIVERGENCE 1
#define TDX_FD_ENSTROPHY 2
int tdx_fd(const float* u, float* out, int B, int X, int Y, int Z, float two_hx, float two_hy, float two_hz, float dv,
           int mode, void* stream);
int tdx_ot_features(const float* u_grid, const float* u_cells, const float* p_cells, const int64_t* unpadded_idx,
                    const float* scale, float* out, int S, int64_t n_cells, int X, int Y, int Z, float two_hx, float two_hy,
                    float two_hz, void* stream);

#define TDX_OT_OK 0
#define TDX_OT_ROUND_CAP 1
#define TDX_OT_BID_CAP 2
#define TDX_OT_BAD_JOB 3
#define TDX_OT_NONFINITE 4
size_t tdx_ot_workspace_bytes(int max_n, int slots);
int tdx_ot_auction(const float* fa, const float* fb, int64_t n_cells, const int* idx, const int* offsets, int K,
                   const int* jobs, int J, int Sa, int Sb, double rel_eps, int max_rounds, int64_t max_bids,
                   void* workspace, int max_n, int slots, double* out, int* status, void* stream);

int tdx_randn(float* out, int64_t n, uint64_t seed, uint64_t stream_id, uint64_t* offset_dev, void* stream);
int tdx_randn_batched(float* out, int B, int64_t n, uint64_t seed, const uint64_t* stream_ids, uint64_t* offset_dev,
                      void* stream);

#define TDX_SIGNAL_STRIDE 64
int tdx_signal_host(uint32_t* host_flag, const uint32_t* gen_dev, uint32_t k, void* stream);
// ... 80 lines not shown
```

Baseline: 166.9 million.

## Add 8-channel first-conv path with packed encode, ring conv, and wgrad kernel

When x and c_local both have 4 features, the composed first convolution now packs the raw inputs into 8 channels per voxel instead of padding to 16. A dedicated pair-encode kernel, an 8-wide weight layout in the MFMA/ring forward kernels, and a new c8 weight-gradient kernel serve this shape. This halves the input bytes read by the first conv's forward and wgrad and drops the wasted zero-padded half of each K chunk. In exchange it adds new specialized code paths gated by shape and an environment switch, with some risk of reduced MFMA efficiency at K=8.

```diff
diff --git a/generative-turbulence_amd/csrc/tdx_codec.hip b/generative-turbulence_amd/csrc/tdx_codec.hip
--- a/generative-turbulence_amd/csrc/tdx_codec.hip
+++ b/generative-turbulence_amd/csrc/tdx_codec.hip
@@ -22,6 +22,23 @@
 #pragma unroll
         for (int j = 0; j < 8; ++j) o.v[j] = enc.eval(j, in);
         o.store(y + ((int64_t)b * V + v) * Dtot + lc * 8);
+    }
+}
+
+template <typename T, int F>
+__global__ void __launch_bounds__(CD_THREADS)
+encode_pair_fwd_kernel(const float* __restrict__ x, const float* __restrict__ wx, const float* __restrict__ bx,
+                       const float* __restrict__ c, const float* __restrict__ wc, const float* __restrict__ bc,
+                       T* __restrict__ y, int64_t V) {
+    const int b = blockIdx.y;
+    const EncPairLane<F> enc(b, V, x, wx, bx, c, wc, bc);
+    const int64_t v0 = (int64_t)blockIdx.x * CD_VOX, v1 = min(V, v0 + CD_VOX);
+    for (int64_t v = v0 + threadIdx.x; v < v1; v += CD_THREADS) {
+        const auto in = enc.load(V, v);
+        Vec8<T> o;
+#pragma unroll
+        for (int j = 0; j < 8; ++j) o.v[j] = enc.eval(j, in);
+        o.store(y + ((int64_t)b * V + v) * 8);
     }
 }
 
@@ -133,6 +150,12 @@
     TDX_CHECK_ARG(x && wx && bx && y && B > 0 && V > 0 && D > 0);
     TDX_CHECK_ARG(c == nullptr || (wc && bc));
     const int Dtot = c ? 2 * D : D;
+    if (c && D == 4 && Fx == 4 && Fc == 4) {
+        dim3 grid(ceil_div(V, CD_VOX), B);
+        TDX_DISPATCH_DTYPE(dtype, hipLaunchKernelGGL((encode_pair_fwd_kernel<T, 4>), grid, dim3(CD_THREADS), 0, as_stream(stream),
+                                                     x, wx, bx, c, wc, bc, (T*)y, V));
+        return tdx_launch_status();
+    }
     if ((D % 8) || !pow2(Dtot / 8) || Dtot / 8 > 64 || Fx != 4 || (c && Fc != 4)) return TDX_ESHAPE;
     dim3 grid(ceil_div(V, CD_VOX), B);
     TDX_DISPATCH_DTYPE(dtype, hipLaunchKernelGGL((encode_fwd_kernel<T, 4>), grid, dim3(CD_THREADS), 0, as_stream(stream),
diff --git a/generative-turbulence_amd/csrc/tdx_codec_elem.h b/generative-turbulence_amd/csrc/tdx_codec_elem.h
--- a/generative-turbulence_amd/csrc/tdx_codec_elem.h
+++ b/generative-turbulence_amd/csrc/tdx_codec_elem.h
@@ -41,6 +41,39 @@
 };
 
 template <int F>
+struct EncPairLane {
+    struct In { float v[2][F]; };
+    const float* src[2];
+    float w[8][F], bias[8];
+    __device__ __forceinline__ EncPairLane(int b, int64_t V, const float* __restrict__ x, const float* __restrict__ wx,
+                                           const float* __restrict__ bx, const float* __restrict__ c, const float* __restrict__ wc,
+                                           const float* __restrict__ bc) {
+        src[0] = x + (int64_t)b * F * V;
+        src[1] = c;
+#pragma unroll
+        for (int j = 0; j < 8; ++j) {
+            bias[j] = j < 4 ? bx[j] : bc[j - 4];
+#pragma unroll
+            for (int k = 0; k < F; ++k) w[j][k] = j < 4 ? wx[j * F + k] : wc[(j - 4) * F + k];
+        }
+    }
+    __device__ __forceinline__ In load(int64_t V, int64_t v) const {
+        In in;
+#pragma unroll
+        for (int h = 0; h < 2; ++h)
+#pragma unroll
+            for (int k = 0; k < F; ++k) in.v[h][k] = src[h][(int64_t)k * V + v];
+        return in;
+    }
+    __device__ __forceinline__ float eval(int j, const In& in) const {
+        float a = bias[j];
+#pragma unroll
+        for (int k = 0; k < F; ++k) a = __builtin_fmaf(w[j][k], in.v[j >> 2][k], a);
+        return a;
+    }
+};
+
+template <int F>
 struct DecLane {
     float w[F][8], bias[F];
     __device__ __forceinline__ DecLane(int lc, int C, const float* __restrict__ wp, const float* __restrict__ bp) {
diff --git a/generative-turbulence_amd/csrc/tdx_conv3.h b/generative-turbulence_amd/csrc/tdx_conv3.h
--- a/generative-turbulence_amd/csrc/tdx_conv3.h
+++ b/generative-turbulence_amd/csrc/tdx_conv3.h
@@ -10,8 +10,9 @@
 
 bool conv3_mfma_supported(int C1, int C2, int Cout);
 bool conv3_mfma_f32_supported(int C1, int C2, int Cout);
+static inline bool conv3_c8_shape(int C1, int C2, int N) { return C1 == 8 && C2 == 0 && N > 0 && (N % 32) == 0; }
 static inline int conv3_layout_kc(int dtype, int K, int N) {
-    if (dtype == 1 || dtype == 3) return conv3_mfma_supported(K, 0, N) ? 16 : 0;
+    if (dtype == 1 || dtype == 3) return conv3_mfma_supported(K, 0, N) ? 16 : (conv3_c8_shape(K, 0, N) ? 8 : 0);
     return conv3_mfma_f32_supported(K, 0, N) ? 8 : 0;
 }
 static inline bool conv3_uses_mfma_layout(int dtype, int K, int N) { return (dtype == 1 || dtype == 3) && conv3_mfma_supported(K, 0, N); }
@@ -106,6 +107,9 @@
 int conv3_wgrad_mfma_launch(const Conv3WgradCall& c);
 int conv3_wgrad_small_launch(const Conv3WgradCall& c);
 int conv3_wgrad_ring_launch(const Conv3WgradCall& c);
+bool conv3_wgrad_c8_supported(int Cout, int B, int X, int Y, int Z);
+int conv3_wgrad_c8_launch(const Conv3WgradCall& c);
+bool conv3_c8_route(int dtype, int impl, int Cout, int B, int X, int Y, int Z);
 int conv3_wgrad_mfma_split_launch(const Conv3WgradCall& c);
 int conv3_wgrad_split_ring_launch(const Conv3WgradCall& c);
 int conv3_wgrad_mfma_f32_launch(const Conv3WgradCall& c);
diff --git a/generative-turbulence_amd/csrc/tdx_conv3_entry.hip b/generative-turbulence_amd/csrc/tdx_conv3_entry.hip
--- a/generative-turbulence_amd/csrc/tdx_conv3_entry.hip
+++ b/generative-turbulence_amd/csrc/tdx_conv3_entry.hip
@@ -36,6 +36,11 @@
     } else {
         const bool ok = tdx_is_h16(dtype) && conv3_mfma_supported(C1, C2, N);
         const bool asked = impl == TDX_CONV_MFMA && (tdx_is_h16(dtype) || !data_gradient);
+        if (!ok && !data_gradient && tdx_is_h16(dtype) && conv3_c8_shape(C1, C2, N) && (asked || impl == TDX_CONV_AUTO) &&
+            (r.ring_depth = conv3_ring_depth(C1, C2, N, B, X, Y, Z, false)) != 0) {
+            r.family = TDX_KERNEL_RING;
+            return r;
+        }
         if (!ok) { r.status = asked ? TDX_ESHAPE : TDX_OK; return r; }
         if (!asked && impl != TDX_CONV_AUTO) return r;
         small_or_brick(false);
@@ -187,6 +192,19 @@
     bool f32;
     int status;
 };
+static bool c8_enabled() {
+    const char* env = getenv("TDX_CONV3_C8");
+    return !(env && atoi(env) == 0);
+}
+bool conv3_c8_route(int dtype, int impl, int Cout, int B, int X, int Y, int Z) {
+    if (!c8_enabled() || !tdx_is_h16(dtype) || B <= 0 || X <= 0 || Y <= 0 || Z <= 0 || !conv3_c8_shape(8, 0, Cout)) return false;
+    return conv3_route(dtype, impl, 8, 0, Cout, B, X, Y, Z, false).family == TDX_KERNEL_RING &&
+           conv3_wgrad_c8_supported(Cout, B, X, Y, Z);
+}
+extern "C" int tdx_conv3_c8_route(int Cout, int B, int X, int Y, int Z, int dtype, int impl) {
+    return conv3_c8_route(dtype, impl, Cout, B, X, Y, Z) ? 1 : 0;
+}
+
 static Conv3WgradRoute conv3_wgrad_route(int dtype, int impl, int C1, int C2, int Cout) {
     if (dtype == TDX_F32 && impl == TDX_CONV_SPLIT && conv3_wgrad_mfma_split_supported(C1, C2, Cout))
         return {conv3_wgrad_mfma_split_launch, true, TDX_OK};
@@ -215,7 +233,10 @@
         int e = tdx_zero_async(dwp, ((size_t)27 * Cin * Cout + Cout) * sizeof(float), st);
         if (e != TDX_OK) return e;
     }
-    const Conv3WgradRoute r = conv3_wgrad_route(dtype, impl & 0xff, C1, C2, Cout);
+    Conv3WgradRoute r = conv3_wgrad_route(dtype, impl & 0xff, C1, C2, Cout);
+    const bool c8 = tdx_is_h16(dtype) && conv3_c8_shape(C1, C2, Cout) && ((impl & 0xff) == TDX_CONV_AUTO || (impl & 0xff) == TDX_CONV_MFMA) &&
+                    conv3_wgrad_c8_supported(Cout, B, X, Y, Z);
+    if (c8) r = {conv3_wgrad_c8_launch, false, TDX_OK};
     if (r.status != TDX_OK) return r.status;
     int nslab = 0;
     const bool det = tdx_deterministic();
diff --git a/generative-turbulence_amd/csrc/tdx_conv3_mfma.hip b/generative-turbulence_amd/csrc/tdx_conv3_mfma.hip
--- a/generative-turbulence_amd/csrc/tdx_conv3_mfma.hip
+++ b/generative-turbulence_amd/csrc/tdx_conv3_mfma.hip
@@ -35,7 +35,7 @@
     return v * 64 + ((c ^ ((v >> 1) & 3)) << 4);
 }
 
-template <int NT, bool XT, bool ZERO_PAD, bool PERM, bool EXT, bool HF>
+template <int NT, bool XT, bool ZERO_PAD, bool PERM, bool EXT, bool HF, bool C8 = false>
 __global__ void __launch_bounds__(256, 2)
 conv3_mfma_kernel(const bf16* __restrict__ x1, int C1, const bf16* __restrict__ x2, int C2,
                   const bf16* __restrict__ wp, const float* __restrict__ bias, bf16* __restrict__ y, ConvViews gs,
@@ -95,14 +95,15 @@
             } else {
                 s0 = min(max(s0, 0), g.Ei[0] - 1); s1 = min(max(s1, 0), g.Ei[1] - 1); s2 = min(max(s2, 0), g.Ei[2] - 1);
             }
-            if (ok) a_src[i] = (s0 * g.si[0] + s1 * g.si[1] + s2 * g.si[2]) * 2 + half;
+            if (ok && !(C8 && half)) a_src[i] = (s0 * g.si[0] + s1 * g.si[1] + s2 * g.si[2]) * 2 + half;
         }
     }
     const int64_t batch_vox = (int64_t)b * g.in_batch;
 
     const int b_half = (tid >> 2) & 1;
     const int b_row0 = ((tid >> 3) << 2) + (tid & 3);
-    const int b_goff = ((b_row0 / BN) * Cout + (b_row0 % BN)) * 16 + b_half * 8;
+    const int b_goff = C8 ? ((b_row0 / BN) * Cout + (b_row0 % BN)) * 8
+                          : ((b_row0 / BN) * Cout + (b_row0 % BN)) * 16 + b_half * 8;
     const int b_dst = b_half * B_PLANE + b_row0 * 16;
 
     uint4 areg[A_PER_THREAD], breg[B_PER_THREAD];
@@ -118,12 +119,13 @@
             if (a_src[i] >= 0)
                 areg[i] = *reinterpret_cast<const uint4*>(xs + (int64_t)(a_src[i] >> 1) * Cs + (a_src[i] & 1) * 8);
         }
-        const bf16* wc = wp + (int64_t)c * 27 * Cout * 16 + (int64_t)n0 * 16 + b_goff;
+        constexpr int WK = C8 ? 8 : 16;
+        const bf16* wc = wp + (int64_t)c * 27 * Cout * WK + (int64_t)n0 * WK + b_goff;
 #pragma unroll
         for (int i = 0; i < B_PER_THREAD; ++i) {
             breg[i] = make_uint4(0, 0, 0, 0);
-            if (b_row0 + 128 * i < 27 * BN)
-                breg[i] = *reinterpret_cast<const uint4*>(wc + (int64_t)i * (128 / BN) * Cout * 16);
+            if (b_row0 + 128 * i < 27 * BN && !(C8 && b_half))
+                breg[i] = *reinterpret_cast<const uint4*>(wc + (int64_t)i * (128 / BN) * Cout * WK);
         }
     };
     auto store_slice = [&]() {
@@ -152,7 +154,7 @@
 #pragma unroll
             for (int i = 0; i < 16; ++i) acc[nt][mt][i] = 0.f;
 
-    const int nchunks = Cin / M3_KC;
+    const int nchunks = C8 ? 1 : Cin / M3_KC;
     load_slice(0);
     for (int c = 0; c < nchunks; ++c) {
         __syncthreads();
@@ -292,12 +294,12 @@
     }
 }
 
-template <int NT, bool XT, bool ZP, bool PERM, bool EXT, bool HF>
+template <int NT, bool XT, bool ZP, bool PERM, bool EXT, bool HF, bool C8 = false>
 static int launch_view_h(const Conv3Call& c, const ConvViews& v) {
     constexpr int BN = NT * 32;
     constexpr int HXv = (XT ? 2 : 4) + 2, HYv = (XT ? 16 : 8) + 2, SZv = XT ? 10 : 12;
     const size_t lds = (size_t)2 * (HXv * HYv * SZv * 16 + 64) + (size_t)27 * BN * 32 + 128;
-    auto kern = conv3_mfma_kernel<NT, XT, ZP, PERM, EXT, HF>;
+    auto kern = conv3_mfma_kernel<NT, XT, ZP, PERM, EXT, HF, C8>;
     static bool attr_set = false;
     if (!attr_set) {
         hipError_t e = hipFuncSetAttribute((const void*)kern, hipFuncAttributeMaxDynamicSharedMemorySize, (int)lds);
@@ -324,6 +326,8 @@
     const int* slabs_beyond = c.slabs_beyond;
     const int NT = (c.N % 64 == 0) ? 2 : 1;
     if ((int64_t)g.Xi * g.Yi * g.Zi * 2 >= (1ll << 31) || (int64_t)g.Xo * g.Yo * g.Zo >= (1ll << 31)) return TDX_ESHAPE;
+    const bool c8 = conv3_c8_shape(C1, C2, c.N);
+    if (c8 && (slabs_beyond == nullptr || zero_pad || ext != nullptr)) return TDX_ESHAPE;
     static const bool no_thin = getenv("TDX_CONV3_THIN") && atoi(getenv("TDX_CONV3_THIN")) == 0;
 
     const int Ei[3] = {g.Xi, g.Yi, g.Zi}, Eo[3] = {g.Xo, g.Yo, g.Zo};
@@ -363,6 +367,13 @@
     };
     auto launch = [&](const ConvViews& vs, bool xt, bool permuted) -> int {
         if (vs.start[3] == 0) return TDX_OK;
+        if (c8) {
+            if (!xt) return TDX_ESHAPE;
+            if (NT == 2) return c.hf() ? launch_view_h<2, true, false, false, false, true, true>(c, vs)
+                                       : launch_view_h<2, true, false, false, false, false, true>(c, vs);
+            return c.hf() ? launch_view_h<1, true, false, false, false, true, true>(c, vs)
+                          : launch_view_h<1, true, false, false, false, false, true>(c, vs);
+        }
 #define M3_GO(NTV, XTV, PV) (zero_pad ? launch_view<NTV, XTV, true, PV>(c, vs) : launch_view<NTV, XTV, false, PV>(c, vs))
         if (ext != nullptr) {
             if (zero_pad || xt || permuted) return TDX_ESHAPE;
diff --git a/generative-turbulence_amd/csrc/tdx_conv3_ring.hip b/generative-turbulence_amd/csrc/tdx_conv3_ring.hip
--- a/generative-turbulence_amd/csrc/tdx_conv3_ring.hip
+++ b/generative-turbulence_amd/csrc/tdx_conv3_ring.hip
@@ -22,6 +22,7 @@
     double* gn_acc;
     bf16* d1; bf16* d2; int D1; const bf16* a1; const bf16* a2;
     const void* zeros;
+    int wk;
     unsigned long long* stamps;
 };
 
@@ -142,7 +143,7 @@
     for (int j = 0; j < WPW; ++j) {
         const int pj = min(max(iw, 0) * WPW + j, S::WPIECES - 1);
         const int e = pj * 64 + lane;
-        wlane[j] = (unsigned)((min(e / BN, 26) * A.Cout + (e % BN)) * 32);
+        wlane[j] = (unsigned)((min(e / BN, 26) * A.Cout + (e % BN)) * (2 * A.wk));
     }
 
     const int ly = Z4 ? (r & 7) : (r & 3), lz = Z4 ? (r >> 3) : (r >> 2);
@@ -209,7 +210,7 @@
         }
     };
     auto issue_weight_piece = [&](int c8, int wslot, int j) {
-        const bf16* base = A.wp + ((int64_t)((c8 >> 1) * 27) * A.Cout + n0) * 16 + (c8 & 1) * 8;
+        const bf16* base = A.wp + ((int64_t)((c8 >> 1) * 27) * A.Cout + n0) * A.wk + (c8 & 1) * 8;
         const int pj = iw * WPW + j;
         const unsigned dst = pj < S::WPIECES ? ldsW + wslot * S::WSLOT + pj * 1024 : ldsD;
         rg_dma_off(base, wlane[j], dst);
@@ -452,7 +453,7 @@
 static int ring_brick_depth(int C1, int C2, int Cout, int B, int X, int Y, int Z) {
     const char* env = getenv("TDX_CONV3_RING");
     const int mode = env ? atoi(env) : 1;
-    if (mode == 0 || !conv3_mfma_supported(C1, C2, Cout)) return 0;
+    if (mode == 0 || !(conv3_mfma_supported(C1, C2, Cout) || conv3_c8_shape(C1, C2, Cout))) return 0;
     const char* z4 = getenv("TDX_RING_Z4");
     if (z4 && atoi(z4) == 2 && ring_z4_supported(C1, C2, Cout, B, X, Y, Z, 2)) return 4;
     if (ring_z8_supported(C1, C2, Cout, B, X, Y, Z, mode)) return 8;
@@ -515,6 +516,8 @@
     a.gn_acc = c.gn_acc;
     a.d1 = (bf16*)c.d1; a.d2 = (bf16*)c.d2; a.D1 = c.D1; a.a1 = (const bf16*)c.a1; a.a2 = (const bf16*)c.a2;
     a.zeros = tdx_scratch_ptr();
+    a.wk = conv3_c8_shape(c.C1, c.C2, c.N) ? 8 : 16;
+    if (a.wk == 8 && zero_pad) return TDX_ESHAPE;
     a.stamps = nullptr;
 #ifdef RG_STAMPS
     a.stamps = rg_stamp_buffer;
diff --git a/generative-turbulence_amd/csrc/tdx_conv3_wgrad_ring.hip b/generative-turbulence_amd/csrc/tdx_conv3_wgrad_ring.hip
--- a/generative-turbulence_amd/csrc/tdx_conv3_wgrad_ring.hip
+++ b/generative-turbulence_amd/csrc/tdx_conv3_wgrad_ring.hip
@@ -254,3 +254,182 @@
 #undef WR_GO
     return tdx_launch_status();
 }
+
+#define WC_XPIECES ((WR::NHALO + 63) / 64)
+#define WC_XBUF (WC_XPIECES * 1024)
+#define WC_XPW ((WC_XPIECES + 3) / 4)
+#define WC_GROUPS 7
+
+template <int NTN, bool HF>
+__global__ void __launch_bounds__(768)
+conv3_wgrad_c8_kernel(const bf16* __restrict__ x, const bf16* __restrict__ dy, float* __restrict__ dwp, float* __restrict__ dbias,
+                      WgradView gv, int Cout, int nsplit, int64_t slab_stride, const void* __restrict__ zeros) {
+    extern __shared__ __attribute__((aligned(1024))) unsigned char smem[];
+    unsigned char* sX = smem;
+    unsigned char* sG = smem + 2 * WC_XBUF;
+    constexpr int GBUF = WR_GBUF(NTN), GPW = WR_GPW(NTN);
+    const unsigned lds0 = lds_addr(smem);
+
+    const int tid = threadIdx.x, lane = tid & 63;
+    const int wave = __builtin_amdgcn_readfirstlane(tid >> 6);
+    const int tile = blockIdx.x / nsplit, split = blockIdx.x - tile * nsplit;
+    const int co0 = tile * (32 * NTN);
+    const int nbricks = gv.B * gv.nb[0] * gv.nb[1] * gv.nb[2];
+
+    if (wave >= WR_CW) {
+        const int lw = wave - WR_CW;
+        int xh[WC_XPW];
+#pragma unroll
+        for (int i = 0; i < WC_XPW; ++i) {
+            const int hv = min(min(lw * WC_XPW + i, WC_XPIECES - 1) * 64 + lane, WR::NHALO - 1);
+            int hx, hy, hz;
+            WR::halo_coords(hv, hx, hy, hz);
+            xh[i] = hx | (hy << 8) | (hz << 16);
+        }
+        const int g_plane = (lw * GPW) / 16, g_p0 = (lw * GPW) % 16;
+        const int g_e0 = g_p0 * 64 + lane;
+        auto issue = [&](int brick, int buf) {
+            int bx, by, bz;
+            const int bb = wgrad_brick_coords(gv, brick, bx, by, bz);
+#pragma unroll
+            for (int i = 0; i < WC_XPW; ++i) {
+                const int sx = min(max(bx * WR::BX + (xh[i] & 0xff) - 1, 0), gv.E[0] - 1);
+                const int sy = min(max(by * WR::BY + ((xh[i] >> 8) & 0xff) - 1, 0), gv.E[1] - 1);
+                const int sz = min(max(bz * WR::BZ + ((xh[i] >> 16) & 0xff) - 1, 0), gv.E[2] - 1);
+                const int64_t vox = (int64_t)bb * gv.batch + sx * gv.s[0] + sy * gv.s[1] + sz * gv.s[2];
+                lds_dma16(x + vox * 8, lds0 + buf * WC_XBUF + min(lw * WC_XPW + i, WC_XPIECES - 1) * 1024);
+            }
+#pragma unroll
+            for (int j = 0; j < GPW; ++j) {
+                const int e = g_e0 + 64 * j, v = e >> 2, c4 = e & 3;
+                const int vx = bx * WR::BX + (v >> 6), vy = by * WR::BY + ((v >> 3) & 7), vz = bz * WR::BZ + (v & 7);
+                const bool ok = vx < gv.E[0] && vy < gv.E[1] && vz < gv.E[2];
+                const int64_t vox = wgrad_voxel(gv, bb, vx, vy, vz);
+                const bf16* src = ok ? dy + vox * Cout + co0 + g_plane * 32 + c4 * 8 : reinterpret_cast<const bf16*>(zeros);
+                lds_dma16(src, lds0 + 2 * WC_XBUF + buf * GBUF + g_plane * WR::GPLANE + (g_p0 + j) * 1024);
+            }
+        };
+        int brick = split, it = 0;
+        if (brick < nbricks) issue(brick, 0);
+        for (; brick < nbricks; brick += nsplit, ++it) {
+            asm volatile("s_waitcnt vmcnt(0)" ::: "memory");
+            lds_barrier();
+            if (brick + nsplit < nbricks) issue(brick + nsplit, (it + 1) & 1);
+        }
+        asm volatile("s_waitcnt vmcnt(0)" ::: "memory");
+        return;
+    }
+
+    const WgradLane L = wgrad_lane(lane);
+    const int p = lane & 3, gl = (lane >> 4) & 1;
+    const bool bias_wave = wave == WC_GROUPS;
+    const int ltap_lane = min(4 * min(wave, WC_GROUPS - 1) + 2 * gl + (p >> 1), 26);
+    const int a_off = wgrad_x_frag_row<WR>(L, WR::tap_offset(ltap_lane)) * 16 + 8 * (p & 1);
+    const int b_row = (8 * L.kh + L.q) * 64 + L.col_off;
+
+    f32x16 acc[NTN];
+#pragma unroll
+    for (int i = 0; i < NTN; ++i)
+#pragma unroll
+        for (int e = 0; e < 16; ++e) acc[i][e] = 0.f;
+    const bf16x8 ones = H16<HF>::ones();
+
+    int it = 0;
+    for (int brick = split; brick < nbricks; brick += nsplit, ++it) {
+        lds_barrier();
+        const unsigned char* bX = sX + (it & 1) * WC_XBUF + a_off;
+        const unsigned char* bG = sG + (it & 1) * GBUF + b_row;
+        auto read_a = [&](int s) {
+            const unsigned char* ap = bX + (wgrad_x_step_offset<WR>(s) >> 2);
+            return tr_frag(ap, ap + 4 * 16);
+        };
+        auto read_b = [&](int s, int nt) {
+            const unsigned char* bp = bG + nt * WR::GPLANE + s * (16 * 64);
+            return tr_frag(bp, bp + 4 * 64);
+        };
+        bf16x8 A[2], Bq[2][NTN];
+        A[0] = read_a(0);
+#pragma unroll
+        for (int nt = 0; nt < NTN; ++nt) Bq[0][nt] = read_b(0, nt);
+        auto step = [&](int s, int cur) {
+            const int sn = min(s + 1, WR_NSTEPS - 1), nx = cur ^ 1;
+            A[nx] = read_a(sn);
+#pragma unroll
+            for (int nt = 0; nt < NTN; ++nt) Bq[nx][nt] = read_b(sn, nt);
+            const bf16x8 a = bias_wave ? ones : A[cur];
+#pragma unroll
+            for (int nt = 0; nt < NTN; ++nt) acc[nt] = H16<HF>::mfma(a, Bq[cur][nt], acc[nt]);
+        };
+#pragma unroll 1
+        for (int s2 = 0; s2 < WR_NSTEPS / 2; ++s2) {
+            step(2 * s2, 0);
+            step(2 * s2 + 1, 1);
+        }
+    }
+
+    const int r = lane & 31, hh = lane >> 5;
+#pragma unroll
+    for (int nt = 0; nt < NTN; ++nt) {
+        if (!bias_wave) {
+#pragma unroll
+            for (int e = 0; e < 16; ++e) {
+                const int ltap = 4 * wave + (e >> 2), ci = (e & 3) + 4 * hh;
+                if (ltap > 26) continue;
+                const int tap = wgrad_global_tap(gv, ltap);
+                float* dst = &dwp[((int64_t)tap * 8 + ci) * Cout + co0 + nt * 32 + r];
+                if (slab_stride) dst[(int64_t)split * slab_stride] = acc[nt][e];
+                else atomicAdd(dst, acc[nt][e]);
+            }
+        } else if (dbias != nullptr && hh == 0) {
+            atomicAdd(&dbias[co0 + nt * 32 + r], acc[nt][0]);
+        }
+    }
+}
+
+static int wgrad_c8_nsplit(int Cout, int nbricks) {
+    const int NTN = (Cout % 64) == 0 ? 2 : 1, ntiles = Cout / (32 * NTN);
+    const int cus = tdx_persistent_cus();
+    int nsplit = cus >= 256 ? (256 + ntiles - 1) / ntiles : std::max(cus / ntiles, 1);
+    if (nsplit > nbricks) nsplit = nbricks;
+    return nsplit < 1 ? 1 : nsplit;
+}
+
+bool conv3_wgrad_c8_supported(int Cout, int B, int X, int Y, int Z) {
+    const char* env = getenv("TDX_WGRAD_RING");
+    if (env && atoi(env) == 0) return false;
+    if (Cout <= 0 || (Cout % 32) || B <= 0 || X <= 0 || Y <= 0 || Z <= 0) return false;
+    if (tdx_scratch_ptr() == nullptr || tdx_scratch_bytes() < 16) return false;
+    Conv3WgradCall c = {};
+    c.B = B; c.X = X; c.Y = Y; c.Z = Z;
+    WgradView g;
+    const int nbricks = conv3_wgrad_view(g, c, WR::BX, WR::BY, WR::BZ);
+    return nbricks >= 4 * wgrad_c8_nsplit(Cout, nbricks);
+}
+
+int conv3_wgrad_c8_launch(const Conv3WgradCall& c) {
+    const int Cout = c.Cout;
+    if (!conv3_c8_shape(c.C1, c.C2, Cout) || !conv3_wgrad_c8_supported(Cout, c.B, c.X, c.Y, c.Z)) return TDX_ESHAPE;
+    WgradView g;
+    const int nbricks = conv3_wgrad_view(g, c, WR::BX, WR::BY, WR::BZ);
+    const int NTN = (Cout % 64) == 0 ? 2 : 1, ntiles = Cout / (32 * NTN);
+    int nsplit = wgrad_c8_nsplit(Cout, nbricks);
+    const size_t lds = (size_t)2 * WC_XBUF + (size_t)2 * WR_GBUF(NTN);
+    int64_t slab_stride;
+    float* out = conv3_wgrad_merge(c, nsplit, slab_stride);
+    static bool attr_set[2][2] = {{false, false}, {false, false}};
+#define WC_GO(NTNV, HFV)                                                                                                          \
+    do {                                                                                                                          \
+        auto kern = conv3_wgrad_c8_kernel<NTNV, HFV>;                                                                             \
+        if (!attr_set[NTNV - 1][HFV]) {                                                                                           \
+            hipError_t e = hipFuncSetAttribute((const void*)kern, hipFuncAttributeMaxDynamicSharedMemorySize, (int)lds);          \
+            if (e != hipSuccess) return (int)e;                                                                                   \
+            attr_set[NTNV - 1][HFV] = true;                                                                                       \
+        }                                                                                                                         \
+        hipLaunchKernelGGL(kern, dim3((unsigned)(ntiles * nsplit)), dim3(768), lds, c.st, (const bf16*)c.x1, (const bf16*)c.dy,   \
+                           out, c.dbias, g, Cout, nsplit, slab_stride, tdx_scratch_ptr());                                        \
+    } while (0)
+    if (NTN == 2) { if (c.hf) WC_GO(2, true); else WC_GO(2, false); }
+    else { if (c.hf) WC_GO(1, true); else WC_GO(1, false); }
+#undef WC_GO
+    return tdx_launch_status();
+}
diff --git a/generative-turbulence_amd/turbdiff_amd/_lib.py b/generative-turbulence_amd/turbdiff_amd/_lib.py
--- a/generative-turbulence_amd/turbdiff_amd/_lib.py
+++ b/generative-turbulence_amd/turbdiff_amd/_lib.py
@@ -33,6 +33,7 @@
     "tdx_conv3_uses_ring": (_i, [_i] * 7),
     "tdx_conv3_ring_brick_depth": (_i, [_i] * 7),
     "tdx_conv3_fwd_kernel": (_i, [_i] * 9),
+    "tdx_conv3_c8_route": (_i, [_i] * 7),
     "tdx_conv3_fwd_gn": (_i, [_vp, _i, _vp, _i, _vp, _vp, _vp, _vp, _i, _f, _vp, _i, _i, _i, _i, _i, _i, _i, _vp]),
     "tdx_conv3_fwd_partial": (_i, [_vp, _i, _i, _vp, _vp, _vp, _i, _vp, _vp, _i, _f, _vp, _i, _i, _i, _i, _i, _i, _i, _vp]),
     "tdx_conv3_bwd_data_workspace_bytes": (_sz, [_i, _i, _i, _i, _i, _i, _i]),
diff --git a/generative-turbulence_amd/turbdiff_amd/models/ddpm.py b/generative-turbulence_amd/turbdiff_amd/models/ddpm.py
--- a/generative-turbulence_amd/turbdiff_amd/models/ddpm.py
+++ b/generative-turbulence_amd/turbdiff_amd/models/ddpm.py
@@ -359,16 +359,19 @@
         return enc
 
 
-    def compose_first_conv(self, x, c_local):
+    def first_conv_group_width(self, x, c_local) -> int:
+        if c_local.requires_grad:
+            return 16
         first = self.u_net.downsampling_blocks[0]
-        D = self.encode_x.out_channels
-        if not (COMPOSE_FIRST_CONV and isinstance(first, ResnetBlock) and first.fused() and c_local is not None
-                and isinstance(first.conv, nn.Identity) and self.in_features <= 8 and self.c_local_features <= 8
-                and first.block1.conv.in_channels == D + self.encode_c_local.out_channels):
-            return None
-        dev, P = x.device, (16 if c_local.requires_grad else 8)
+        if (self.compute_dtype in _lib.H16_DTYPES and self.in_features == 4 and self.c_local_features == 4
+                and ops.conv3_c8_route(first.block1.conv.out_channels, (x.shape[0],) + tuple(x.shape[2:]), self.compute_dtype)):
+            return 4
+        return 8
+
+    def _raw_eye_for(self, P, dev):
         eye = getattr(self, "_raw_eye", None)
         if eye is None or eye[0].device != dev or eye[0].shape[0] != P:
+            first = self.u_net.downsampling_blocks[0]
             ex = torch.zeros(P, self.in_features, 1, 1, 1, device=dev)
             ec = torch.zeros(P, self.c_local_features, 1, 1, 1, device=dev)
             ex[: self.in_features, :, 0, 0, 0] = torch.eye(self.in_features, device=dev)
@@ -378,6 +381,28 @@
             idx = list(range(nx)) + [nx + nc] * (P - nx) + list(range(nx, nx + nc)) + [nx + nc] * (P - nc)
             eye = self._raw_eye = (ex, ec, torch.zeros(P, device=dev), torch.zeros(Co_, 1, 3, 3, 3, device=dev),
                                    torch.tensor(idx, dtype=torch.long, device=dev))
+        return eye
+
+    def composed_first_conv_weight(self, P, dev):
+        first = self.u_net.downsampling_blocks[0]
+        eye = self._raw_eye_for(P, dev)
+        W1, b1 = first.block1.conv.weight, first.block1.conv.bias
+        w_enc = torch.block_diag(self.encode_x.weight.flatten(1), self.encode_c_local.weight.flatten(1))
+        b_enc = torch.cat((self.encode_x.bias, self.encode_c_local.bias))
+        w8 = torch.einsum("octuv,ck->oktuv", W1, w_enc)
+        w_eff = torch.cat((w8, eye[3]), dim=1).index_select(1, eye[4])
+        b_eff = b1 + torch.einsum("octuv,c->o", W1, b_enc)
+        return w_eff, b_eff
+
+    def compose_first_conv(self, x, c_local):
+        first = self.u_net.downsampling_blocks[0]
+        D = self.encode_x.out_channels
+        if not (COMPOSE_FIRST_CONV and isinstance(first, ResnetBlock) and first.fused() and c_local is not None
+                and isinstance(first.conv, nn.Identity) and self.in_features <= 8 and self.c_local_features <= 8
+                and first.block1.conv.in_channels == D + self.encode_c_local.out_channels):
+            return None
+        dev, P = x.device, self.first_conv_group_width(x, c_local)
+        eye = self._raw_eye_for(P, dev)
         if not ops.encode_supported(x, c_local, eye[0]):
             return None
         raw = ops.encode(x, c_local, eye[0], eye[2], eye[1], eye[2], self.compute_dtype)
@@ -389,11 +414,7 @@
             hit = getattr(self, "_composed_frozen", None)
             if hit is not None and hit[0] == key:
                 return raw, hit[1], hit[2], self.in_features + self.c_local_features
-        w_enc = torch.block_diag(self.encode_x.weight.flatten(1), self.encode_c_local.weight.flatten(1))
-        b_enc = torch.cat((self.encode_x.bias, self.encode_c_local.bias))
-        w8 = torch.einsum("octuv,ck->oktuv", W1, w_enc)
-        w_eff = torch.cat((w8, eye[3]), dim=1).index_select(1, eye[4])
-        b_eff = b1 + torch.einsum("octuv,c->o", W1, b_enc)
+        w_eff, b_eff = self.composed_first_conv_weight(P, dev)
         if frozen:
             self._composed_frozen = (key, w_eff, b_eff)
         return raw, w_eff, b_eff, self.in_features + self.c_local_features
diff --git a/generative-turbulence_amd/turbdiff_amd/ops.py b/generative-turbulence_amd/turbdiff_amd/ops.py
--- a/generative-turbulence_amd/turbdiff_amd/ops.py
+++ b/generative-turbulence_amd/turbdiff_amd/ops.py
@@ -241,6 +241,8 @@
 
 def encode_supported(x, c_local, wx):
     D = wx.shape[0]
+    if D == 4 and c_local is not None:
+        return x.shape[1] == 4 and c_local.shape[0] == 4 and not x.requires_grad and not c_local.requires_grad
     n = (2 * D if c_local is not None else D) // 8
     return (x.shape[1] == 4 and (c_local is None or c_local.shape[0] == 4) and D % 8 == 0 and n & (n - 1) == 0
             and n <= 64 and not x.requires_grad)
@@ -435,6 +437,14 @@
             gw, gb = _conv3_wgrad_out(ctx.wshape, ctx.has_bias, dev)
             _conv3_wgrad(x1, C1, x2, C2, gy, gw, gb, grid, Cout, code, impl, _conv3_wgrad_ws(Cin, Cout, impl, dev), st)
         return gx1, gx2, gw, gb, None, None
+
+
+def conv3_c8_route(Cout: int, grid, dtype: torch.dtype) -> bool:
+    if dtype not in L.H16_DTYPES or not hasattr(L.load(), "tdx_conv3_c8_route"):
+        return False
+    with L._LAUNCH_LOCK:
+        L.ensure_scratch()
+        return bool(L.query("tdx_conv3_c8_route", Cout, *grid, L.dtype_code(dtype), L.conv_impl()))
 
 
 def conv3(x1, weight, bias=None, x2=None):
diff --git a/include/tdx.h b/include/tdx.h
--- a/include/tdx.h
+++ b/include/tdx.h
@@ -57,6 +57,7 @@
 #define TDX_KERNEL_SMALL 2
 #define TDX_KERNEL_RING 3
 int tdx_conv3_fwd_kernel(int C1, int C2, int Cout, int B, int X, int Y, int Z, int dtype, int impl);
+int tdx_conv3_c8_route(int Cout, int B, int X, int Y, int Z, int dtype, int impl);
 
 int tdx_conv3_fwd_gn(const void* x1, int C1, const void* x2, int C2, const void* wf, const float* bias, void* y,
                      float* stats, int G, float eps, void* gn_workspace, int B, int X, int Y, int Z, int Cout,
```

Result: no change. 167.5 million (median of 2 runs) (+0.4%).
